# ziniuwan/maed

Measured on AMD Instinct MI355X. Metric: video-clips/sec (BxT frames) train step, higher is better.
Workload: dtype bf16

## Files before the change

### include/maed_hip.h

```cpp
#ifndef MAED_HIP_H
#define MAED_HIP_H

#include <stddef.h>
#include <stdint.h>

#ifdef __cplusplus
extern "C" {
#endif

typedef enum { MAED_F32 = 0, MAED_BF16 = 1,
               MAED_F32X3 = 2, MAED_F32X6 = 3,
               MAED_F32X1 = 4 } maed_dtype;

typedef enum {
    MAED_OK = 0,
    MAED_ERR_ARG = -1,
    MAED_ERR_SHAPE = -2,
    MAED_ERR_ALIGN = -3,
    MAED_ERR_LAUNCH = -4,
    MAED_ERR_UNSUPPORTED = -5
} maed_status;

typedef enum {
    MAED_EPI_STORE = 0,
    MAED_EPI_GELU = 1,
    MAED_EPI_RESID_F32 = 2,
    MAED_EPI_MUL_DGELU = 3,
    MAED_EPI_ATOMIC_F32 = 4,
    MAED_EPI_STORE_F32 = 5,
    MAED_EPI_TANH = 6,
    MAED_EPI_ADD = 7
} maed_epilogue;

typedef enum { MAED_IMPL_AUTO = 0, MAED_IMPL_VALU = 1, MAED_IMPL_MFMA = 2,
               MAED_IMPL_MFMA_GLDS1 = 3, MAED_IMPL_MFMA_GLDS2 = 4,
               MAED_IMPL_MFMA_LONG = 5,
               MAED_IMPL_MFMA_256 = 6,
               MAED_IMPL_X1 = 9,
               MAED_IMPL_MFMA_SK = 10,
               MAED_IMPL_X3 = 7, MAED_IMPL_X6 = 8
} maed_impl;

const char* maed_last_error(void);
int maed_version(void);

typedef enum {
    MAED_OPT_F32_MATMUL = 0,
    MAED_OPT_SIDE_STREAM = 1,
    MAED_OPT_TN_TARGET_WGS = 2,
    MAED_OPT_ABLATE = 3,
    MAED_OPT_GN_BWD_ONEPASS = 4,
    MAED_OPT_F32_BWD_X1 = 5,
    MAED_OPT_ST_FUSED = 6,
    MAED_OPT_CONV3X3_ROWS_WGS = 7,
    MAED_OPT_STEM_WGRAD_WGS = 8,
    MAED_OPT_LBS_FRAMES = 9,
    MAED_OPT_TN_DMA = 10,
    MAED_OPT_X3_PLANES = 11,
    MAED_OPT_X3_PLANES_LN = 12,
    MAED_OPT_SK = 13,
    MAED_OPT_SK_GRID = 14,
    MAED_OPT_TN_SK = 15,
    MAED_OPT_CONV3X3_NARROW_WGS = 16,
    MAED_OPT_CONV3X3_FRAME = 17,
    MAED_OPT_COUNT
} maed_option;
int maed_init(int device);
int maed_device_faults(void);
int maed_device_faults_clear(void);
int maed_set_option(int key, int value);
int maed_get_option(int key);

int maed_layernorm_fwd(const float* x, int64_t x_row_stride, const float* gamma, const float* beta,
                       void* y, int dtype, float* mean, float* rstd,
                       int64_t rows, int C, float eps, void* stream);
int maed_layernorm_bwd(const void* dy, int dtype, const float* x, int64_t x_row_stride,
                       const float* gamma, const float* mean, const float* rstd,
                       const float* dres_in, float* dx_out, void* dx_twin, float* dgamma, float* dbeta,
                       int64_t rows, int C, void* stream);

int maed_gemm_nt(const void* A, int64_t lda, const void* B, int64_t ldb,
                 int64_t M, int64_t N, int64_t K, int dtype, int epilogue,
                 const float* bias, void* out, int64_t ldo, void* out2,
                 const void* aux, int64_t ldaux, int splitk, int impl, void* stream);

int maed_gemm_nt_planes(const void* a_hi, const void* a_lo, int64_t lda, const void* b_hi, const void* b_lo, int64_t ldb, int64_t M, int64_t N, int64_t K,
                        int epilogue, const float* bias, void* out, int64_t ldo, void* out2_bf16, const void* aux, int64_t ldaux, void* out_hi, void* out_lo,
                        int variant, void* stream);
int maed_split_planes(const float* x, void* hi, void* lo, int64_t n, void* stream);

int maed_gemm_tn_wgrad(const void* Y, int64_t ldy, const void* X, int64_t ldx, int64_t M, int N, int K,
                       float* dW, int64_t ldw, float* dbias, int dtype, void* stream);

int maed_transpose_cast(const void* in, int in_dtype, int64_t ldi, int64_t M, int64_t N,
                        void* out_t, int64_t ldt, void* out_c, int64_t ldc, float* colsum,
                        int dtype, void* stream);

int maed_attn_spatial_fwd(const void* qkv, void* o, float* lse, int F, int P, int H, float scale,
                          int dtype, int impl, void* stream);
int maed_attn_spatial_bwd(const void* qkv, const void* o, const void* d_o, const float* lse,
                          void* dqkv, int accumulate, int F, int P, int H, float scale,
                          int dtype, int impl, void* stream);

int maed_attn_temporal_fwd(const void* qkv, void* o, float* lse, int F, int P, int H, int T,
                           float scale, int dtype, void* stream);
int maed_attn_temporal_bwd(const void* qkv, const void* o, const void* d_o, const float* lse,
                           void* dqkv, int accumulate, int F, int P, int H, int T, float scale,
                           int dtype, void* stream);

int maed_st_colmean(const void* x_s, const void* x_t, void* means, float* ws, int F, int P, int C, int dtype, void* stream);
int maed_st_mix_fwd(const void* x_s, const void* x_t, const float* logits, void* mix,
                    int F, int P, int C, int dtype, void* stream);
int maed_st_mix_bwd_reduce(const void* dmix, const void* x_s, const void* x_t, const float* logits,
                           void* dlogits, float* ws, int F, int P, int C, int dtype, void* stream);
int maed_st_mix_bwd_apply(const void* dmix, const float* logits, const void* dmeans, void* dx_s, void* dx_t,
                          int F, int P, int C, int dtype, void* stream);
int maed_st_fused_supported(int P, int C, int dtype);
int maed_st_fused_fwd(const void* x_s, const void* x_t, const void* w_ts, const float* b_ts, void* means, float* logits, void* mix,
                      uint32_t* sync, float* ex, int F, int P, int C, int dtype, void* stream);
int maed_st_fused_bwd(const void* dmix, const void* x_s, const void* x_t, const float* logits, const void* wt_ts, void* dlogits, void* dx_s,
                      void* dx_t, uint32_t* sync, float* ex, int F, int P, int C, int dtype, void* stream);


int maed_embed_add_fwd(const void* patch, int dtype, const float* cls, const float* pos, const float* temp,
                       float* tokens, int F, int P, int C, int T, void* stream);
int maed_embed_add_bwd(const float* dtokens, void* dpatch, int dtype, float* dpos, float* dtemp, int F, int P, int C, int T, void* stream);

int maed_dropout(const float* x, float* y, int64_t n, float p, uint64_t seed, void* stream);
typedef struct { float lr, bias_corr1, bias_corr2, reserved0; uint64_t seed; uint64_t reserved1; } maed_train_state;
int maed_dropout_dev(const float* x, float* y, int64_t n, float p, const maed_train_state* state, uint64_t call_id, void* stream);
int maed_tanh_bwd(const float* dy, const void* y, void* dx, int64_t n, int dtype, void* stream);

typedef struct {
    int F, P, C, H, T, hidden;
    int dtype;
    int impl;
    float eps;
} maed_block_dims;

typedef struct {
    const float *ln1_g, *ln1_b, *ln2_g, *ln2_b;
    const void *w_qkv, *w_ts, *w_proj, *w_fc1, *w_fc2;
    const float *b_qkv, *b_ts, *b_proj, *b_fc1, *b_fc2;
    const void *wt_qkv, *wt_ts, *wt_proj, *wt_fc1, *wt_fc2;
} maed_block_params;

typedef struct {
    float *ln1_g, *ln1_b, *ln2_g, *ln2_b;
    float *w_qkv, *w_ts, *w_proj, *w_fc1, *w_fc2;
    float *b_qkv, *b_ts, *b_proj, *b_fc1, *b_fc2;
} maed_block_grads;

size_t maed_ste_block_saved_bytes(const maed_block_dims* d);
size_t maed_ste_block_scratch_bytes(const maed_block_dims* d);
int maed_ste_block_fwd(const maed_block_dims* d, const maed_block_params* p, const float* x_in,
                       float* x_out, void* saved, void* stream);
size_t maed_ste_block_twin_work_bytes(const maed_block_dims* d);
int maed_ste_block_fwd_twin(const maed_block_dims* d, const maed_block_params* p, const float* x_in, float* x_out, void* saved_bf16, void* work_f32, int work_slot,
                            void* stream);
int maed_ste_block_twin_join(void* stream);
int maed_ste_block_infer(const maed_block_dims* d, const maed_block_params* p, const float* x_in,
                         float* x_out, void* work, void* stream);
int maed_ste_block_bwd(const maed_block_dims* d, const maed_block_params* p, const maed_block_grads* g,
                       const float* x_in, const float* dx_out, float* dx_in, void* saved, void* scratch,
                       const void* dx_out_twin, void* dx_in_twin, void* stream);

int maed_stream_fence(void* from_stream, void* to_stream);

int maed_prof_enable(int on);
int maed_prof_ntags(void);
int maed_prof_collect(double* ms_total_host, int* count_host);
int maed_prof_flops(double* flops_host);
int maed_prof_records(int tag, double* us_host, double* flops_host, double* bytes_host, int cap);

int maed_ktd_chain_fwd(const float* base, const float* w_anc, float* pose, int F, void* stream);

int maed_rot6d_pose_fwd(const float* pose6d, float* rotmat, float* angle_axis, int64_t n_joints, void* stream);

typedef struct {
    const float* v_template;
    const float* shapedirs;
    const float* posedirs;
    const float* J_template;
    const float* J_shapedirs;
    const float* lbs_weights;
    const int32_t* parents;
} maed_smpl_params;
int maed_smpl_lbs_fwd(const maed_smpl_params* sp, const float* betas, const float* rotmat,
                      float* verts, float* joints24, float* scratch_A, float* v_posed, int F, void* stream);
int maed_joint_regress_fwd(const float* Jreg, int J, const float* verts, float* out, int F, void* stream);
int maed_joint_regress_csr_fwd(const int32_t* rowptr, const int32_t* cols, const float* vals, int J, const float* verts, float* out, int F, void* stream);
int maed_smpl_joints_project_fwd(const float* joints24, const float* verts, const int64_t* extra_vertex_ids,
                                 const float* extra9, const int64_t* joint_map, const float* cam,
                                 const float* joints_override, int Jo, float* kp3d, float* kp2d, int F, void* stream);


int maed_smpl_joints_project_bwd(const float* kp3d, const float* cam, const int64_t* joint_map, const float* d_kp3d,
                                 const float* d_kp2d, const float* d_cam_in, int64_t cam_in_stride, float* d_joints24,
                                 float* d_extra21, float* d_extra9, float* d_cam, int F, void* stream);
int maed_smpl_skin_bwd(const maed_smpl_params* sp, const float* A, const float* v_posed, const float* d_verts,
                       const float* d_extra21, const int64_t* extra_vertex_ids, const float* d_extra9, const float* Jextra,
                       float* d_vposed, float* dA, int F, void* stream);
int maed_smpl_skin_bwd_sparse(const maed_smpl_params* sp, const float* A, const float* v_posed, const int32_t* active, int n_active,
                              const float* d_extra21, const int64_t* extra_vertex_ids, const float* d_extra9, const float* Jextra,
                              float* d_vposed_active, float* dA, int F, void* stream);
int maed_smpl_chain_bwd(const maed_smpl_params* sp, const float* betas, const float* rotmat, const float* dA,
                        const float* d_joints24, const float* dpf_dbeta, const float* d_rotmat_in, const float* d_betas_in,
                        int64_t betas_in_stride, float* d_rotmat, float* d_betas, int F, void* stream);
int maed_rot6d_pose_bwd(const float* pose6d, const float* d_rotmat, const float* d_aa, int64_t aa_stride,
                        float* d_pose6d, int64_t n_joints, void* stream);
int maed_ktd_chain_bwd(const float* pose, const float* w_anc, const float* d_pose, const float* d_shape, const float* d_cam,
                       float* d_out, int64_t ld_out, float* d_w_anc, float* d_b_feat, int F, void* stream);
#define MAED_KTD_W_ANC 3420
typedef struct { const float* w[26]; const float* b[26]; float* gw[26]; float* gb[26]; } maed_ktd_ptrs;
int maed_ktd_pack(const maed_ktd_ptrs* t, int hidden, float* w_feat, float* b_feat, float* w_anc, void* stream);
int maed_ktd_unpack_add(const maed_ktd_ptrs* t, int hidden, const float* d_w_feat, const float* d_b_feat, const float* d_w_anc, void* stream);

typedef struct { float w_kp2d, w_kp3d, w_pose, w_shape, w_norm; } maed_loss_weights;
int maed_loss_fwd_bwd(const float* pred_kp2d, const float* gt_kp2d, int M2, const float* pred_kp3d, const float* gt_kp3d,
                      const float* pred_theta, const float* gt_theta, const uint8_t* w_smpl, int M3,
                      const maed_loss_weights* w, float* losses, float* d_kp2d, float* d_kp3d, float* d_theta,
                      double* partials, void* stream);

int maed_loss_accl_fwd_bwd(const float* pred_kp3d, const float* gt_kp3d, int N, int T, float weight, double* loss, float* d_kp3d, void* stream);

typedef struct {
    const float* w;
    float* gw;
    const void* gout;
    int64_t dst_off;
    int64_t dst_t_off;
    int32_t O, I, KHW, fstart;
    int32_t gout_f32;
    int32_t pad_;
} maed_ws_conv;
int maed_weight_std_fwd(const void* conv_table, int n_convs, int n_filters, void* out, int dtype, float* stats, float eps, int transpose_tiles, void* stream);
int maed_weight_std_bwd(const void* conv_table, int n_convs, int n_filters, int dtype, const float* stats, float eps, void* stream);
int maed_groupnorm_fwd(const void* x, const void* residual, const float* gamma, const float* beta, void* y, double* sums,
                       uint8_t* relu_mask, int N, int HW, int C, float eps, int relu, int dtype, int sums_zeroed, void* stream);
int maed_groupnorm_fwd_twin(const void* x, const void* residual, const float* gamma, const float* beta, void* y, double* sums,
                            uint8_t* relu_mask, int N, int HW, int C, float eps, int relu, int sums_zeroed, void* twin_x, void* twin_y, void* stream);
#define MAED_GN_SYNC_WORDS 80
int maed_groupnorm_bwd(const void* x, const uint8_t* relu_mask, const void* dy, const double* sums, const float* gamma, const float* beta,
                       void* dx, void* dres, float* dgamma, float* dbeta, float* ab_scratch, int N, int HW, int C, float eps,
                       int relu, int dtype, int ab_zeroed, uint32_t* frame_sync, void* aux_stream, void* stream);
typedef struct { const float* ab; float* dgamma; float* dbeta; int N; int C; } maed_gn_affine_item;
int maed_gn_affine_grad_batch(const maed_gn_affine_item* items, int count, void* stream);

int maed_maxpool3s2_same_fwd(const void* x, void* y, uint8_t* idx, int N, int H, int W, int C, int dtype, void* stream);
int maed_maxpool3s2_same_bwd(const void* dy, const uint8_t* idx, void* dx, int N, int H, int W, int C, int dtype, void* stream);

int maed_stem_input(const float* x, void* y, int N, int C, int H, int W, int pad_top, int pad_bottom, int pad_left, int pad_right, int c_stride, int dtype,
                    void* stream);

int maed_conv3x3_wgrad_rows64_scratch_floats(int F, int H, int W, int Cin, int Cout);
int maed_conv3x3_wgrad_rows64(const void* dy, const void* x, float* dW, void* scratch, int F, int H, int W, int dtype, void* stream);

int maed_stem7x7s2_supported(int H, int W);
int maed_stem7x7s2_fwd(const void* xp, const void* w, void* wimg, void* y, double* gn_sums, int F, int H, int W, int dtype, void* stream);
int maed_stem7x7s2_wgrad_scratch_floats(int F, int H, int W);
int maed_stem7x7s2_wgrad(const void* dy, const void* xp, float* dW, void* scratch, int F, int H, int W, int dtype, void* stream);

int maed_subsample2_fwd(const void* x, void* y, int F, int H, int W, int C, int dtype, void* stream);
int maed_subsample2_bwd(const void* g, void* dx, int F, int H, int W, int C, int dtype, void* stream);

typedef struct { const float* src; void* dst_c; void* dst_t; int32_t rows, cols, tile0, tiles_n; } maed_wt_entry;
int maed_weight_refresh(const void* table, int n_entries, int n_tiles, int dtype, void* stream);

int maed_adam_step(float* p, const float* g, float* m, float* v, void* shadow_bf16, int64_t n,
                   float lr, float beta1, float beta2, float eps, float weight_decay,
                   float bias_corr1, float bias_corr2, float gscale, void* stream);
int maed_adam_step_dev(float* p, const float* g, float* m, float* v, void* shadow_bf16, int64_t n, const maed_train_state* state,
                       float beta1, float beta2, float eps, float weight_decay, float gscale, void* stream);

#define MAED_COMM_ID_BYTES 128
int maed_comm_load(const char* librccl_path);
int maed_comm_unique_id(void* id128);
int maed_comm_init(int rank, int world, const void* unique_id);
int maed_comm_allreduce_async(void* buf, size_t n, int dtype, void* compute_stream);
int maed_comm_wait(void* compute_stream);
int maed_comm_world(void);
int maed_comm_destroy(void);

int maed_conv3x3_fwd(const void* x, const void* w_taps, const void* zero_page, void* y, int F, int H, int W, int Cin, int Cout,
                     int stride, int pad_top, int pad_left, int Ho, int Wo, const void* add, int w_layout, int dtype, double* gn_sums,
                     void* stream);

int maed_conv1x1_fwd(const void* x, int64_t ldx, const void* w, int64_t ldw, int64_t M, int Cout, int Cin, void* y, int64_t ldy, int hw,
                     double* gn_sums, int dtype, void* stream);

int maed_conv3x3_s2_dgrad(const void* dy, const void* wt_image, const void* zero_page, void* dx, int F, int H, int W, int Cin, int Cout,
                          int pad_top, int pad_left, int Ho, int Wo, int dtype, void* stream);
int maed_conv3x3_s2_tables(void* tapmask, int* rowtab, int F, int H, int W, int pad_top, int pad_left, int Ho, int Wo, void* stream);
int maed_conv3x3_s2_wgrad(const void* dy, const void* x, const void* tapmask, const int* rowtab, const void* zero_page, float* dW, int F, int H, int W,
                          int Cin, int Cout, int Ho, int Wo, int dtype, void* stream);
int maed_conv3x3_tapmask(void* tapmask, int F, int H, int W, void* stream);
int maed_conv3x3_wgrad(const void* dy, const void* x, const void* tapmask, const void* zero_page, float* dW, int F, int H, int W, int Cin,
                       int Cout, int dtype, void* stream);

int maed_eval_pose_errors(const float* pred, const float* target, int N, int J, float* mpjpe, float* pa_mpjpe,
                          float* pred_centred, float* target_centred, void* stream);
int maed_similarity_transform(const float* S1, const float* S2, int N, int J, float* S1_hat, void* stream);
int maed_eval_accel(const float* joints, const float* joints_gt, int N, int J, float* out, void* stream);
int maed_eval_vertex_error(const float* pred_verts, const float* target_verts, int N, int V, float* out, void* stream);

size_t maed_clip_preprocess_workspace(int F, int H, int W);
int maed_clip_preprocess(const uint8_t* src, int64_t src_bytes, const int32_t* frame_i, const float* frame_minv, const int32_t* clip_i,
                         const float* clip_f, int F, int N, int H, int W, const float* norm_host, int has_contrast, int form, float* out,
                         void* workspace, size_t workspace_bytes, void* stream);

#ifdef __cplusplus
}
#endif
#endif
```

### maed_amd/_lib.py

```python
import ctypes as C
import os

HERE = os.path.dirname(os.path.abspath(__file__))
LIB_PATH = os.environ.get("MAED_HIP_LIB") or os.path.join(HERE, "libmaed_hip.so")

F32, BF16 = 0, 1
F32X3, F32X6, F32X1 = 2, 3, 4
EPI_STORE, EPI_GELU, EPI_RESID_F32, EPI_MUL_DGELU, EPI_ATOMIC_F32, EPI_STORE_F32, EPI_TANH, EPI_ADD = range(8)
IMPL_AUTO, IMPL_VALU, IMPL_MFMA = 0, 1, 2
IMPL_MFMA_256 = 6
IMPL_MFMA_LONG = 5
IMPL_MFMA_SK = 10
IMPL_X3, IMPL_X6, IMPL_X1 = 7, 8, 9
(OPT_F32_MATMUL, OPT_SIDE_STREAM, OPT_TN_TARGET_WGS, OPT_ABLATE, OPT_GN_BWD_ONEPASS, OPT_F32_BWD_X1, OPT_ST_FUSED, OPT_CONV3X3_ROWS_WGS, OPT_STEM_WGRAD_WGS,
 OPT_LBS_FRAMES, OPT_TN_DMA, OPT_X3_PLANES, OPT_X3_PLANES_LN, OPT_SK, OPT_SK_GRID, OPT_TN_SK, OPT_CONV3X3_NARROW_WGS, OPT_CONV3X3_FRAME) = range(18)

vp, i64, i32, f32 = C.c_void_p, C.c_int64, C.c_int, C.c_float


class GnAffineItem(C.Structure):
    _fields_ = [("ab", C.c_void_p), ("dgamma", C.c_void_p), ("dbeta", C.c_void_p), ("N", C.c_int), ("C", C.c_int)]


class BlockDims(C.Structure):
    _fields_ = [("F", i32), ("P", i32), ("C", i32), ("H", i32), ("T", i32), ("hidden", i32),
                ("dtype", i32), ("impl", i32), ("eps", f32)]


_PARAM_FIELDS = ["ln1_g", "ln1_b", "ln2_g", "ln2_b", "w_qkv", "w_ts", "w_proj", "w_fc1", "w_fc2",
                 "b_qkv", "b_ts", "b_proj", "b_fc1", "b_fc2", "wt_qkv", "wt_ts", "wt_proj", "wt_fc1", "wt_fc2"]
_GRAD_FIELDS = _PARAM_FIELDS[:14]


class BlockParams(C.Structure):
    _fields_ = [(n, vp) for n in _PARAM_FIELDS]


class BlockGrads(C.Structure):
    _fields_ = [(n, vp) for n in _GRAD_FIELDS]


class SmplParams(C.Structure):
    _fields_ = [(n, vp) for n in ["v_template", "shapedirs", "posedirs", "J_template", "J_shapedirs", "lbs_weights", "parents"]]


class KtdPtrs(C.Structure):
    _fields_ = [("w", vp * 26), ("b", vp * 26), ("gw", vp * 26), ("gb", vp * 26)]


class LossWeights(C.Structure):
    _fields_ = [(n, f32) for n in ["w_kp2d", "w_kp3d", "w_pose", "w_shape", "w_norm"]]


KTD_W_ANC = 3420

SIGNATURES = {
    "maed_last_error": (C.c_char_p, []),
    "maed_version": (i32, []),
    "maed_init": (i32, [i32]),
    "maed_device_faults": (i32, []),
    "maed_device_faults_clear": (i32, []),
    "maed_set_option": (i32, [i32, i32]),
    "maed_get_option": (i32, [i32]),
    "maed_layernorm_fwd": (i32, [vp, i64, vp, vp, vp, i32, vp, vp, i64, i32, f32, vp]),
    "maed_layernorm_bwd": (i32, [vp, i32, vp, i64, vp, vp, vp, vp, vp, vp, vp, vp, i64, i32, vp]),
    "maed_gemm_tn_wgrad": (i32, [vp, i64, vp, i64, i64, i32, i32, vp, i64, vp, i32, vp]),
    "maed_gemm_nt": (i32, [vp, i64, vp, i64, i64, i64, i64, i32, i32, vp, vp, i64, vp, vp, i64, i32, i32, vp]),
    "maed_transpose_cast": (i32, [vp, i32, i64, i64, i64, vp, i64, vp, i64, vp, i32, vp]),
    "maed_attn_spatial_fwd": (i32, [vp, vp, vp, i32, i32, i32, f32, i32, i32, vp]),
    "maed_attn_spatial_bwd": (i32, [vp, vp, vp, vp, vp, i32, i32, i32, i32, f32, i32, i32, vp]),
    "maed_attn_temporal_fwd": (i32, [vp, vp, vp, i32, i32, i32, i32, f32, i32, vp]),
    "maed_attn_temporal_bwd": (i32, [vp, vp, vp, vp, vp, i32, i32, i32, i32, i32, f32, i32, vp]),
    "maed_st_colmean": (i32, [vp, vp, vp, vp, i32, i32, i32, i32, vp]),
    "maed_st_mix_fwd": (i32, [vp, vp, vp, vp, i32, i32, i32, i32, vp]),
    "maed_st_mix_bwd_reduce": (i32, [vp, vp, vp, vp, vp, vp, i32, i32, i32, i32, vp]),
    "maed_st_mix_bwd_apply": (i32, [vp, vp, vp, vp, vp, i32, i32, i32, i32, vp]),
    "maed_st_fused_supported": (i32, [i32, i32, i32]),
    "maed_st_fused_fwd": (i32, [vp, vp, vp, vp, vp, vp, vp, vp, vp, i32, i32, i32, i32, vp]),
    "maed_st_fused_bwd": (i32, [vp, vp, vp, vp, vp, vp, vp, vp, vp, vp, i32, i32, i32, i32, vp]),
    "maed_embed_add_fwd": (i32, [vp, i32, vp, vp, vp, vp, i32, i32, i32, i32, vp]),
    "maed_embed_add_bwd": (i32, [vp, vp, i32, vp, vp, i32, i32, i32, i32, vp]),
    "maed_ste_block_saved_bytes": (C.c_size_t, [C.POINTER(BlockDims)]),
    "maed_ste_block_scratch_bytes": (C.c_size_t, [C.POINTER(BlockDims)]),
    "maed_gemm_nt_planes": (i32, [vp, vp, i64, vp, vp, i64, i64, i64, i64, i32, vp, vp, i64, vp, vp, i64, vp, vp, i32, vp]),
    "maed_split_planes": (i32, [vp, vp, vp, i64, vp]),
    "maed_ste_block_twin_work_bytes": (C.c_size_t, [C.POINTER(BlockDims)]),
    "maed_ste_block_fwd_twin": (i32, [C.POINTER(BlockDims), C.POINTER(BlockParams), vp, vp, vp, vp, i32, vp]),
    "maed_ste_block_twin_join": (i32, [vp]),
    "maed_ste_block_fwd": (i32, [C.POINTER(BlockDims), C.POINTER(BlockParams), vp, vp, vp, vp]),
    "maed_ste_block_infer": (i32, [C.POINTER(BlockDims), C.POINTER(BlockParams), vp, vp, vp, vp]),
    "maed_ste_block_bwd": (i32, [C.POINTER(BlockDims), C.POINTER(BlockParams), C.POINTER(BlockGrads), vp, vp, vp, vp, vp, vp, vp, vp]),
    "maed_loss_accl_fwd_bwd": (i32, [vp, vp, i32, i32, f32, vp, vp, vp]),
    "maed_dropout": (i32, [vp, vp, i64, f32, C.c_uint64, vp]),
    "maed_dropout_dev": (i32, [vp, vp, i64, f32, vp, C.c_uint64, vp]),
    "maed_tanh_bwd": (i32, [vp, vp, vp, i64, i32, vp]),
    "maed_stream_fence": (i32, [vp, vp]),
    "maed_prof_enable": (i32, [i32]),
    "maed_prof_ntags": (i32, []),
    "maed_prof_collect": (i32, [C.POINTER(C.c_double), C.POINTER(i32)]),
    "maed_prof_flops": (i32, [C.POINTER(C.c_double)]),
    "maed_prof_records": (i32, [i32, C.POINTER(C.c_double), C.POINTER(C.c_double), C.POINTER(C.c_double), i32]),
    "maed_ktd_chain_fwd": (i32, [vp, vp, vp, i32, vp]),
    "maed_rot6d_pose_fwd": (i32, [vp, vp, vp, i64, vp]),
    "maed_smpl_lbs_fwd": (i32, [C.POINTER(SmplParams), vp, vp, vp, vp, vp, vp, i32, vp]),
    "maed_joint_regress_fwd": (i32, [vp, i32, vp, vp, i32, vp]),
    "maed_joint_regress_csr_fwd": (i32, [vp, vp, vp, i32, vp, vp, i32, vp]),
    "maed_smpl_joints_project_fwd": (i32, [vp, vp, vp, vp, vp, vp, vp, i32, vp, vp, i32, vp]),
    "maed_smpl_joints_project_bwd": (i32, [vp, vp, vp, vp, vp, vp, i64, vp, vp, vp, vp, i32, vp]),
    "maed_smpl_skin_bwd": (i32, [C.POINTER(SmplParams), vp, vp, vp, vp, vp, vp, vp, vp, vp, i32, vp]),
    "maed_smpl_skin_bwd_sparse": (i32, [C.POINTER(SmplParams), vp, vp, vp, i32, vp, vp, vp, vp, vp, vp, i32, vp]),
    "maed_smpl_chain_bwd": (i32, [C.POINTER(SmplParams), vp, vp, vp, vp, vp, vp, vp, i64, vp, vp, i32, vp]),
    "maed_rot6d_pose_bwd": (i32, [vp, vp, vp, i64, vp, i64, vp]),
    "maed_ktd_chain_bwd": (i32, [vp, vp, vp, vp, vp, vp, i64, vp, vp, i32, vp]),
    "maed_ktd_pack": (i32, [C.POINTER(KtdPtrs), i32, vp, vp, vp, vp]),
    "maed_ktd_unpack_add": (i32, [C.POINTER(KtdPtrs), i32, vp, vp, vp, vp]),
    "maed_loss_fwd_bwd": (i32, [vp, vp, i32, vp, vp, vp, vp, vp, i32, C.POINTER(LossWeights), vp, vp, vp, vp, vp, vp]),
    "maed_weight_std_fwd": (i32, [vp, i32, i32, vp, i32, vp, f32, i32, vp]),
    "maed_weight_std_bwd": (i32, [vp, i32, i32, i32, vp, f32, vp]),
    "maed_groupnorm_fwd": (i32, [vp, vp, vp, vp, vp, vp, vp, i32, i32, i32, f32, i32, i32, i32, vp]),
    "maed_groupnorm_fwd_twin": (i32, [vp, vp, vp, vp, vp, vp, vp, i32, i32, i32, f32, i32, i32, vp, vp, vp]),
    "maed_groupnorm_bwd": (i32, [vp, vp, vp, vp, vp, vp, vp, vp, vp, vp, vp, i32, i32, i32, f32, i32, i32, i32, vp, vp, vp]),
    "maed_gn_affine_grad_batch": (i32, [vp, i32, vp]),
    "maed_comm_load": (i32, [C.c_char_p]),
    "maed_comm_unique_id": (i32, [vp]),
    "maed_comm_init": (i32, [i32, i32, vp]),
    "maed_comm_allreduce_async": (i32, [vp, C.c_size_t, i32, vp]),
    "maed_comm_wait": (i32, [vp]),
    "maed_comm_world": (i32, []),
    "maed_comm_destroy": (i32, []),
    "maed_conv3x3_fwd": (i32, [vp, vp, vp, vp, i32, i32, i32, i32, i32, i32, i32, i32, i32, i32, vp, i32, i32, vp, vp]),
    "maed_conv1x1_fwd": (i32, [vp, i64, vp, i64, i64, i32, i32, vp, i64, i32, vp, i32, vp]),
    "maed_conv3x3_tapmask": (i32, [vp, i32, i32, i32, vp]),
    "maed_conv3x3_s2_dgrad": (i32, [vp, vp, vp, vp, i32, i32, i32, i32, i32, i32, i32, i32, i32, i32, vp]),
    "maed_conv3x3_s2_tables": (i32, [vp, vp, i32, i32, i32, i32, i32, i32, i32, vp]),
    "maed_conv3x3_s2_wgrad": (i32, [vp, vp, vp, vp, vp, vp, i32, i32, i32, i32, i32, i32, i32, i32, vp]),
    "maed_conv3x3_wgrad": (i32, [vp, vp, vp, vp, vp, i32, i32, i32, i32, i32, i32, vp]),
    "maed_eval_pose_errors": (i32, [vp, vp, i32, i32, vp, vp, vp, vp, vp]),
    "maed_similarity_transform": (i32, [vp, vp, i32, i32, vp, vp]),
    "maed_eval_accel": (i32, [vp, vp, i32, i32, vp, vp]),
    "maed_eval_vertex_error": (i32, [vp, vp, i32, i32, vp, vp]),
    "maed_maxpool3s2_same_fwd": (i32, [vp, vp, vp, i32, i32, i32, i32, i32, vp]),
    "maed_maxpool3s2_same_bwd": (i32, [vp, vp, vp, i32, i32, i32, i32, i32, vp]),
    "maed_stem_input": (i32, [vp, vp, i32, i32, i32, i32, i32, i32, i32, i32, i32, i32, vp]),
    "maed_conv3x3_wgrad_rows64_scratch_floats": (i32, [i32, i32, i32, i32, i32]),
    "maed_conv3x3_wgrad_rows64": (i32, [vp, vp, vp, vp, i32, i32, i32, i32, vp]),
    "maed_stem7x7s2_supported": (i32, [i32, i32]),
    "maed_stem7x7s2_fwd": (i32, [vp, vp, vp, vp, vp, i32, i32, i32, i32, vp]),
    "maed_stem7x7s2_wgrad_scratch_floats": (i32, [i32, i32, i32]),
    "maed_stem7x7s2_wgrad": (i32, [vp, vp, vp, vp, i32, i32, i32, i32, vp]),
    "maed_subsample2_fwd": (i32, [vp, vp, i32, i32, i32, i32, i32, vp]),
    "maed_subsample2_bwd": (i32, [vp, vp, i32, i32, i32, i32, i32, vp]),
    "maed_weight_refresh": (i32, [vp, i32, i32, i32, vp]),
    "maed_adam_step": (i32, [vp, vp, vp, vp, vp, i64, f32, f32, f32, f32, f32, f32, f32, f32, vp]),
    "maed_adam_step_dev": (i32, [vp, vp, vp, vp, vp, i64, vp, f32, f32, f32, f32, f32, vp]),
    "maed_clip_preprocess_workspace": (C.c_size_t, [i32, i32, i32]),
    "maed_clip_preprocess": (i32, [vp, i64, vp, vp, vp, vp, i32, i32, i32, i32, C.POINTER(f32), i32, i32, vp, vp, C.c_size_t, vp]),
}

_lib = None
_init_pending = False


class MaedHipError(RuntimeError):
    pass


def lib():
    global _lib, _init_pending
    if _lib is None:
        if not os.path.exists(LIB_PATH):
            raise MaedHipError(f"{LIB_PATH} is missing: build it with `python -m maed_amd.build` "
                               "(hipcc --offload-arch=gfx950).  maed_amd has no non-HIP fallback.")
        handle = C.CDLL(LIB_PATH)
        for name, (res, args) in SIGNATURES.items():
            fn = getattr(handle, name)
            fn.restype, fn.argtypes = res, args
        _lib = handle
        apply_options(handle)
        _init_pending = True
    if _init_pending:
        import torch
        if torch.cuda.is_available() and torch.cuda.is_initialized():
            _init_pending = False
            check(_lib.maed_init(torch.cuda.current_device()), "maed_init")
    return _lib


_OPTIONS = {
    OPT_F32_MATMUL: {"exact": 0, "0": 0, "bf16x3": 1, "1": 1, "bf16x6": 2, "2": 2}[os.environ.get("MAED_F32_MATMUL", "exact")],
    OPT_SIDE_STREAM: int(os.environ.get("MAED_WGRAD_SIDE_STREAM", "1") == "1"),
    OPT_TN_TARGET_WGS: int(os.environ.get("MAED_TN_TARGET_WGS", "0")),
    OPT_ABLATE: int(os.environ.get("MAED_GEMM_ABLATE", "0")),
    OPT_F32_BWD_X1: int(os.environ.get("MAED_F32_BWD", "") == "bf16x1"),
    OPT_ST_FUSED: int(os.environ.get("MAED_ST_FUSED", "1")),
    OPT_GN_BWD_ONEPASS: int(os.environ.get("MAED_GN_BWD_ONEPASS", "1")),
    OPT_CONV3X3_ROWS_WGS: 0 if os.environ.get("MAED_CONV3X3_WGRAD_ROWS", "1") == "0" else int(os.environ.get("MAED_CONV3X3_ROWS_WGS", "256")),
    OPT_STEM_WGRAD_WGS: int(os.environ.get("MAED_STEM_WGS", "512")),
    OPT_LBS_FRAMES: int(os.environ.get("MAED_LBS_FB", "0")),
    OPT_TN_DMA: int(os.environ.get("MAED_TN_DMA", "1")),
    OPT_X3_PLANES: int(os.environ.get("MAED_X3_PLANES", "6")),
    OPT_SK: int(os.environ.get("MAED_SK", "1")),
    OPT_SK_GRID: int(os.environ.get("MAED_SK_GRID", "0")),
    OPT_CONV3X3_FRAME: int(os.environ.get("MAED_CONV3X3_FRAME", "1")),
    OPT_CONV3X3_NARROW_WGS: int(os.environ.get("MAED_CONV3X3_NARROW_WGS", "0")),
    OPT_TN_SK: int(os.environ.get("MAED_TN_SK", "1")),
    OPT_X3_PLANES_LN: int(os.environ.get("MAED_X3_PLANES_LN", "0")),
}


def apply_options(handle):
    for k, v in _OPTIONS.items():
        if handle.maed_set_option(k, v) != 0:
            raise MaedHipError(f"maed_set_option({k}, {v}) failed")


def set_option(key, value):
    _OPTIONS[key] = int(value)
    if _lib is not None:
        check(_lib.maed_set_option(key, int(value)), "set_option")


def get_option(key):
    return _OPTIONS[key]


def check(rc, what=""):
    if rc != 0:
        msg = lib().maed_last_error().decode("utf-8", "replace")
        raise MaedHipError(f"{what or 'libmaed_hip'} failed with status {rc}: {msg}")


def device_faults():
    return 0 if _lib is None else int(_lib.maed_device_faults())


def loaded_path():
    return LIB_PATH if _lib is not None else None
```

### maed_amd/csrc/backbone.hip

```cpp
#include "common.cuh"

struct WsConv {
    const float* w;
    float* gw;
    const void* gout;
    int64_t dst_off;
    int64_t dst_t_off;
    int32_t O, I, KHW, fstart;
    int32_t gout_f32, pad_;
};
#define WS_MAX_CONVS 64

__device__ __forceinline__ int ws_find_conv(const WsConv* __restrict__ tab, int n_convs, int fi) {
    int c = 0;
    for (int i = 1; i < n_convs; ++i) c = (fi >= tab[i].fstart) ? i : c;
    return c;
}

template <typename T>
__global__ __launch_bounds__(256) void ws_fwd_kernel(const WsConv* __restrict__ tab, int n_convs, int n_filters, T* __restrict__ out,
                                                     float* __restrict__ stats , float eps, int skip_transposed) {
    const int fi = blockIdx.x * 4 + (threadIdx.x >> 6), lane = threadIdx.x & 63;
    if (fi >= n_filters) return;
    const WsConv d = tab[ws_find_conv(tab, n_convs, fi)];
    const int K = d.I * d.KHW, o = fi - d.fstart;
    const float* src = d.w + (int64_t)o * K;
    float s = 0.f;
    for (int i = lane; i < K; i += 64) s += src[i];
    const float mean = wave_sum(s) / (float)K;
    float q = 0.f;
    for (int i = lane; i < K; i += 64) { const float c = src[i] - mean; q += c * c; }
    const float inv = 1.f / (sqrtf(wave_sum(q) / (float)K) + eps);
    if (lane == 0) { stats[2 * fi] = mean; stats[2 * fi + 1] = inv; }
    T* dst = out + d.dst_off + (int64_t)o * K;
    T* dst_t = (d.dst_t_off >= 0 && !skip_transposed) ? out + d.dst_t_off + o : nullptr;
    const int KHW = d.KHW, I = d.I;
    for (int ci = lane; ci < I; ci += 64) {
        const float* sp = src + (int64_t)ci * KHW;
        for (int r = 0; r < KHW; ++r) {
            const float v = (sp[r] - mean) * inv;
            stf(dst + (int64_t)r * I + ci, v);
            if (dst_t) stf(dst_t + ((int64_t)r * I + ci) * d.O, v);
        }
    }
}

template <typename T>
__global__ __launch_bounds__(256) void ws_transpose_kernel(const WsConv* __restrict__ tab, int n_convs, T* __restrict__ out) {
    __shared__ T tile[64][66];
    int t = blockIdx.x, c = 0, tk = 0;
    for (; c < n_convs; ++c) {
        const int K = tab[c].I * tab[c].KHW;
        tk = (K + 63) / 64;
        const int nt = tab[c].dst_t_off >= 0 ? ((tab[c].O + 63) / 64) * tk : 0;
        if (t < nt) break;
        t -= nt;
    }
    if (c >= n_convs) return;
    const WsConv d = tab[c];
    const int K = d.I * d.KHW, o0 = (t / tk) * 64, k0 = (t % tk) * 64;
    const T* src = out + d.dst_off;
    T* dst = out + d.dst_t_off;
    const int r = threadIdx.x >> 2, q = (threadIdx.x & 3) * 16;
    constexpr int VE = 16 / (int)sizeof(T);
    if (o0 + r < d.O) {
        const T* sp = src + (int64_t)(o0 + r) * K + k0 + q;
        if (k0 + q + 16 <= K && ((uintptr_t)sp & 15) == 0) {
#pragma unroll
            for (int v = 0; v < 16 / VE; ++v) { const uint4 w = reinterpret_cast<const uint4*>(sp)[v]; T e[VE]; memcpy(e, &w, 16);
#pragma unroll
                for (int j = 0; j < VE; ++j) tile[r][q + v * VE + j] = e[j]; }
        } else {
#pragma unroll
            for (int j = 0; j < 16; ++j) if (k0 + q + j < K) tile[r][q + j] = sp[j];
        }
    }
    __syncthreads();
    if (k0 + r < K) {
        T* dp = dst + (int64_t)(k0 + r) * d.O + o0 + q;
        if (o0 + q + 16 <= d.O && ((uintptr_t)dp & 15) == 0) {
#pragma unroll
            for (int v = 0; v < 16 / VE; ++v) { T e[VE];
#pragma unroll
                for (int j = 0; j < VE; ++j) e[j] = tile[q + v * VE + j][r];
                uint4 w; memcpy(&w, e, 16); reinterpret_cast<uint4*>(dp)[v] = w; }
        } else {
#pragma unroll
            for (int j = 0; j < 16; ++j) if (o0 + q + j < d.O) dp[j] = tile[q + j][r];
        }
    }
}

template <typename T>
__global__ __launch_bounds__(256) void ws_bwd_kernel(const WsConv* __restrict__ tab, int n_convs, int n_filters,
                                                     const float* __restrict__ stats, float eps) {
    const int fi = blockIdx.x * 4 + (threadIdx.x >> 6), lane = threadIdx.x & 63;
    if (fi >= n_filters) return;
    const WsConv d = tab[ws_find_conv(tab, n_convs, fi)];
    if (!d.gout || !d.gw) return;
    const int K = d.I * d.KHW, o = fi - d.fstart;
    const float* src = d.w + (int64_t)o * K;
    const T* g = (const T*)d.gout + (int64_t)o * K;
    const float* g32 = (const float*)d.gout + (int64_t)o * K;
    const bool f32 = d.gout_f32 != 0;
    const float mean = stats[2 * fi], inv = stats[2 * fi + 1];
    const int KHW = d.KHW, I = d.I;
    const float rk = 1.0f / (float)KHW;
    float sg = 0.f, sgw = 0.f;
    for (int i = lane; i < K; i += 64) {
        const int ci = KHW == 1 ? i : (int)(((float)i + 0.5f) * rk), r = i - ci * KHW;
        const float gi = f32 ? g32[(int64_t)r * I + ci] : ldf(g + (int64_t)r * I + ci);
        sg += gi; sgw += gi * (src[i] - mean);
    }
    sg = wave_sum(sg); sgw = wave_sum(sgw);
    const float sigma = 1.f / inv - eps;
    const float c2 = (sigma > 0.f) ? sgw * inv * inv / ((float)K * sigma) : 0.f;
    const float gm = sg / (float)K;
    float* dst = d.gw + (int64_t)o * K;
    for (int i = lane; i < K; i += 64) {
        const int ci = KHW == 1 ? i : (int)(((float)i + 0.5f) * rk), r = i - ci * KHW;
        const float gi = f32 ? g32[(int64_t)r * I + ci] : ldf(g + (int64_t)r * I + ci);
        dst[i] += inv * (gi - gm) - (src[i] - mean) * c2;
    }
}

extern "C" int maed_weight_std_fwd(const void* conv_table, int n_convs, int n_filters, void* out, int dtype, float* stats, float eps,
                                   int filters_aligned64, void* stream) {
    MAED_CHECK_ARG(conv_table && out && stats, MAED_ERR_ARG, "weight_std_fwd: null pointer");
    MAED_CHECK_ARG(n_convs > 0 && n_convs <= WS_MAX_CONVS, MAED_ERR_SHAPE, "weight_std_fwd: n_convs=%d out of range", n_convs);
    if (n_filters <= 0) return MAED_OK;
    const int t_tiles = filters_aligned64;
    MAED_DISPATCH_DTYPE(dtype, T, {
        hipLaunchKernelGGL((ws_fwd_kernel<T>), dim3((n_filters + 3) / 4), dim3(256), 0, (hipStream_t)stream, (const WsConv*)conv_table, n_convs, n_filters, (T*)out, stats, eps,
                           t_tiles > 0 ? 1 : 0);
        if (t_tiles > 0) hipLaunchKernelGGL((ws_transpose_kernel<T>), dim3(t_tiles), dim3(256), 0, (hipStream_t)stream, (const WsConv*)conv_table, n_convs, (T*)out);
    });
    MAED_CHECK_LAUNCH("weight_std_fwd");
    return MAED_OK;
}

extern "C" int maed_weight_std_bwd(const void* conv_table, int n_convs, int n_filters, int dtype, const float* stats, float eps, void* stream) {
    MAED_CHECK_ARG(conv_table && stats, MAED_ERR_ARG, "weight_std_bwd: null pointer");
    MAED_CHECK_ARG(n_convs > 0 && n_convs <= WS_MAX_CONVS, MAED_ERR_SHAPE, "weight_std_bwd: n_convs=%d out of range", n_convs);
    if (n_filters <= 0) return MAED_OK;
    MAED_DISPATCH_DTYPE(dtype, T, hipLaunchKernelGGL((ws_bwd_kernel<T>), dim3((n_filters + 3) / 4), dim3(256), 0, (hipStream_t)stream,
                                                      (const WsConv*)conv_table, n_convs, n_filters, stats, eps));
    MAED_CHECK_LAUNCH("weight_std_bwd");
    return MAED_OK;
}

#define GN_G 32

template <typename T>
__device__ __forceinline__ void gn_load8(const T* p, float (&v)[8]) { ld8(p, v); }

template <typename T>
__global__ __launch_bounds__(256) void gn_stats_kernel(const T* __restrict__ x, double* __restrict__ sums , int HW, int C,
                                                       int rows_per_wg) {
    __shared__ double ls[GN_G][2];
    const int n = blockIdx.y, cbn = C / 8, cb = threadIdx.x % cbn, rsub = threadIdx.x / cbn, rstep = 256 / cbn;
    if (threadIdx.x < GN_G * 2) (&ls[0][0])[threadIdx.x] = 0.0;
    __syncthreads();
    const int r0 = blockIdx.x * rows_per_wg;
    const int r1 = min(HW, r0 + rows_per_wg);
    float s[8], q[8];
#pragma unroll
    for (int j = 0; j < 8; ++j) { s[j] = 0.f; q[j] = 0.f; }
    const T* base = x + ((int64_t)n * HW) * C + cb * 8;
    for (int r = r0 + rsub; r < r1; r += rstep) {
        float v[8];
        gn_load8(base + (int64_t)r * C, v);
#pragma unroll
        for (int j = 0; j < 8; ++j) { s[j] += v[j]; q[j] = fmaf(v[j], v[j], q[j]); }
    }
    const int cpg = C / GN_G;
    if (cpg >= 8) {
        float ss = 0.f, qq = 0.f;
#pragma unroll
        for (int j = 0; j < 8; ++j) { ss += s[j]; qq += q[j]; }
        const int g = cb * 8 / cpg;
        atomicAdd(&ls[g][0], (double)ss); atomicAdd(&ls[g][1], (double)qq);
    } else {
        for (int j0 = 0; j0 < 8; j0 += cpg) {
            float ss = 0.f, qq = 0.f;
            for (int j = j0; j < j0 + cpg; ++j) { ss += s[j]; qq += q[j]; }
            const int g = (cb * 8 + j0) / cpg;
            atomicAdd(&ls[g][0], (double)ss); atomicAdd(&ls[g][1], (double)qq);
        }
    }
    __syncthreads();
    if (threadIdx.x < GN_G * 2) atomicAdd(sums + (int64_t)n * GN_G * 2 + threadIdx.x, (&ls[0][0])[threadIdx.x]);
}


template <typename T, bool RES, bool RELU>
__global__ __launch_bounds__(256) void gn_apply_kernel(const T* __restrict__ x, const T* __restrict__ res, const double* __restrict__ sums,
                                                       const float* __restrict__ gamma, const float* __restrict__ beta, T* __restrict__ y,
                                                       uint8_t* __restrict__ mask, int HW, int C, float eps, int rows_per_wg,
                                                       bf16* __restrict__ twin_x = nullptr, bf16* __restrict__ twin_y = nullptr) {
    __shared__ float lmu[GN_G], lrs[GN_G];
    const int n = blockIdx.y;
    if (threadIdx.x < GN_G) {
        const double cnt = (double)HW * (C / GN_G);
        const double m = sums[((int64_t)n * GN_G + threadIdx.x) * 2] / cnt;
        double var = sums[((int64_t)n * GN_G + threadIdx.x) * 2 + 1] / cnt - m * m;
        if (var < 0.0) var = 0.0;
        lmu[threadIdx.x] = (float)m; lrs[threadIdx.x] = (float)(1.0 / sqrt(var + (double)eps));
    }
    __syncthreads();
    const int cbn = C / 8, cb = threadIdx.x % cbn, rsub = threadIdx.x / cbn, rstep = 256 / cbn, cpg = C / GN_G;
    float a[8], b[8];
    {
        float gg[8], bb[8];
        ld8(gamma + cb * 8, gg); ld8(beta + cb * 8, bb);
#pragma unroll
        for (int j = 0; j < 8; ++j) {
            const int g = (cb * 8 + j) / cpg;
            a[j] = lrs[g] * gg[j]; b[j] = bb[j] - lmu[g] * a[j];
        }
    }
    const int r0 = blockIdx.x * rows_per_wg, r1 = min(HW, r0 + rows_per_wg);
    const int64_t base = ((int64_t)n * HW) * C + cb * 8;
    for (int r = r0 + rsub; r < r1; r += rstep) {
        float v[8], o[8];
        gn_load8(x + base + (int64_t)r * C, v);
        if (twin_x) st8_nt(twin_x + base + (int64_t)r * C, v);
#pragma unroll
        for (int j = 0; j < 8; ++j) o[j] = fmaf(v[j], a[j], b[j]);
        if (RES) { float rr[8]; gn_load8(res + base + (int64_t)r * C, rr);
#pragma unroll
            for (int j = 0; j < 8; ++j) o[j] += rr[j]; }
        if (RELU) {
            if (RES && mask) {
                uint32_t bits = 0;
#pragma unroll
                for (int j = 0; j < 8; ++j) bits |= (o[j] > 0.f ? 1u : 0u) << j;
                mask[((int64_t)n * HW + r) * cbn + cb] = (uint8_t)bits;
            }
#pragma unroll
            for (int j = 0; j < 8; ++j) o[j] = fmaxf(o[j], 0.f); }
        st8(y + base + (int64_t)r * C, o);
        if (twin_y) st8_nt(twin_y + base + (int64_t)r * C, o);
    }
}

template <typename T, bool RELU, bool YMASK>
__global__ __launch_bounds__(256) void gn_bwd_reduce_kernel(const T* __restrict__ x, const uint8_t* __restrict__ mask, const T* __restrict__ dy,
                                                            const double* __restrict__ sums, const float* __restrict__ gamma,
                                                            const float* __restrict__ beta, float* __restrict__ ab ,
                                                            float* __restrict__ dgamma, float* __restrict__ dbeta,
                                                            int HW, int C, float eps, int rows_per_wg, int defer_affine) {
    MAED_DYN_SHARED(float, lpart);
    __shared__ float lmu[GN_G], lrs[GN_G];
    const int n = blockIdx.y;
    if (threadIdx.x < GN_G) {
        const double cnt = (double)HW * (C / GN_G);
        const double m = sums[((int64_t)n * GN_G + threadIdx.x) * 2] / cnt;
        double var = sums[((int64_t)n * GN_G + threadIdx.x) * 2 + 1] / cnt - m * m;
        if (var < 0.0) var = 0.0;
        lmu[threadIdx.x] = (float)m; lrs[threadIdx.x] = (float)(1.0 / sqrt(var + (double)eps));
    }
    __syncthreads();
    const int cbn = C / 8, cb = threadIdx.x % cbn, rsub = threadIdx.x / cbn, rstep = 256 / cbn, cpg = C / GN_G;
    float mu[8], rs[8], sa[8], sb[8], ga[8], be[8];
    if (RELU && !YMASK) { ld8(gamma + cb * 8, ga); ld8(beta + cb * 8, be); }
#pragma unroll
    for (int j = 0; j < 8; ++j) { const int g = (cb * 8 + j) / cpg; mu[j] = lmu[g]; rs[j] = lrs[g]; sa[j] = 0.f; sb[j] = 0.f; }
    const int r0 = blockIdx.x * rows_per_wg, r1 = min(HW, r0 + rows_per_wg);
    const int64_t base = ((int64_t)n * HW) * C + cb * 8;
#define GN_RED_ROW(v_, d_, o_)                                                                                  \
    {                                                                                                           \
        _Pragma("unroll") for (int j = 0; j < 8; ++j) v_[j] = (v_[j] - mu[j]) * rs[j];               \
        if (RELU) {                                                                                             \
            if (YMASK) { _Pragma("unroll") for (int j = 0; j < 8; ++j) d_[j] = ((o_ >> j) & 1u) ? d_[j] : 0.f; }  \
            else { _Pragma("unroll") for (int j = 0; j < 8; ++j) d_[j] = fmaf(v_[j], ga[j], be[j]) > 0.f ? d_[j] : 0.f; } \
        }                                                                                                       \
        _Pragma("unroll") for (int j = 0; j < 8; ++j) { sa[j] += d_[j]; sb[j] = fmaf(d_[j], v_[j], sb[j]); }    \
    }
    int r = r0 + rsub;
    for (; r + 3 * rstep < r1; r += 4 * rstep) {
        float v0[8], v1[8], v2[8], v3[8], d0[8], d1[8], d2[8], d3[8];
        uint32_t o0 = 0, o1 = 0, o2 = 0, o3 = 0;
        const int64_t a0 = base + (int64_t)r * C, a1 = a0 + (int64_t)rstep * C, a2 = a1 + (int64_t)rstep * C, a3 = a2 + (int64_t)rstep * C;
        gn_load8(x + a0, v0); gn_load8(x + a1, v1); gn_load8(x + a2, v2); gn_load8(x + a3, v3);
        gn_load8(dy + a0, d0); gn_load8(dy + a1, d1); gn_load8(dy + a2, d2); gn_load8(dy + a3, d3);
        if (RELU && YMASK) {
            const int64_t m0 = ((int64_t)n * HW + r) * cbn + cb;
            o0 = mask[m0]; o1 = mask[m0 + (int64_t)rstep * cbn]; o2 = mask[m0 + 2 * (int64_t)rstep * cbn]; o3 = mask[m0 + 3 * (int64_t)rstep * cbn];
        }
        GN_RED_ROW(v0, d0, o0) GN_RED_ROW(v1, d1, o1) GN_RED_ROW(v2, d2, o2) GN_RED_ROW(v3, d3, o3)
    }
    for (; r < r1; r += rstep) {
        float v[8], d[8];
        uint32_t o = 0;
        gn_load8(x + base + (int64_t)r * C, v); gn_load8(dy + base + (int64_t)r * C, d);
        if (RELU && YMASK) o = mask[((int64_t)n * HW + r) * cbn + cb];
        GN_RED_ROW(v, d, o)
    }
#undef GN_RED_ROW
    float* mine = lpart + ((size_t)rsub * C + cb * 8) * 2;
#pragma unroll
    for (int j = 0; j < 8; ++j) { mine[2 * j] = sa[j]; mine[2 * j + 1] = sb[j]; }
    __syncthreads();
    for (int i = threadIdx.x; i < 2 * C; i += 256) {
        float t = 0.f;
        for (int k = 0; k < rstep; ++k) t += lpart[(size_t)k * 2 * C + i];
        atomicAdd(ab + (int64_t)n * C * 2 + i, t);
        if (!defer_affine) atomicAdd(((i & 1) ? dgamma : dbeta) + (i >> 1), t);
    }
}

__global__ __launch_bounds__(256) void gn_affine_grad_kernel(const float* __restrict__ ab, float* __restrict__ dgamma, float* __restrict__ dbeta, int N, int C) {
    colsum_add(ab, N, 2 * C, [=](int i) { return ((i & 1) ? dgamma : dbeta) + (i >> 1); });
}

#define GN_BATCH_MAX 64
struct GnAffineBatch {
    maed_gn_affine_item it[GN_BATCH_MAX];
    int first[GN_BATCH_MAX + 1];
    int count;
};
__global__ __launch_bounds__(256) void gn_affine_grad_batch_kernel(GnAffineBatch t) {
    __shared__ float fold[4][64];
    int i = 0;
    while (i + 1 < t.count && (int)blockIdx.x >= t.first[i + 1]) ++i;
    const maed_gn_affine_item it = t.it[i];
    const int cols = 2 * it.C, c = ((int)blockIdx.x - t.first[i]) * 64 + (threadIdx.x & 63), rl = threadIdx.x >> 6;
    float s = 0.f;
    if (c < cols)
        for (int r = rl; r < it.N; r += 4) s += it.ab[(int64_t)r * cols + c];
    fold[rl][threadIdx.x & 63] = s;
    __syncthreads();
    if (rl == 0 && c < cols) {
        atomicAdd(((c & 1) ? it.dgamma : it.dbeta) + (c >> 1), (fold[0][threadIdx.x] + fold[1][threadIdx.x]) + (fold[2][threadIdx.x] + fold[3][threadIdx.x]));
    }
}
extern "C" int maed_gn_affine_grad_batch(const maed_gn_affine_item* items, int count, void* stream) {
    MAED_CHECK_ARG(count >= 0 && (items || count == 0), MAED_ERR_ARG, "gn_affine_grad_batch: null table");
    for (int base = 0; base < count; base += GN_BATCH_MAX) {
        GnAffineBatch t;
        t.count = count - base < GN_BATCH_MAX ? count - base : GN_BATCH_MAX;
        int wg = 0;
        for (int i = 0; i < t.count; ++i) {
            const maed_gn_affine_item& it = items[base + i];
            MAED_CHECK_ARG(it.ab && it.dgamma && it.dbeta && it.N > 0 && it.C > 0, MAED_ERR_ARG, "gn_affine_grad_batch: item %d: null pointer or empty extent", base + i);
            t.it[i] = it; t.first[i] = wg;
            wg += (2 * it.C + 63) / 64;
        }
        t.first[t.count] = wg;
        hipLaunchKernelGGL(gn_affine_grad_batch_kernel, dim3((unsigned)wg), dim3(256), 0, (hipStream_t)stream, t);
    }
    MAED_CHECK_LAUNCH("gn_affine_grad_batch");
    return MAED_OK;
}

template <typename T, bool RES, bool RELU>
__global__ __launch_bounds__(256) void gn_bwd_apply_kernel(const T* __restrict__ x, const uint8_t* __restrict__ mask, const T* __restrict__ dy,
                                                           const double* __restrict__ sums, const float* __restrict__ ab,
                                                           const float* __restrict__ gamma, const float* __restrict__ beta,
                                                           T* __restrict__ dx, T* __restrict__ dres,
                                                           int HW, int C, float eps, int rows_per_wg) {
    __shared__ float lmu[GN_G], lrs[GN_G], lm1[GN_G], lm2[GN_G];
    const int n = blockIdx.y, cpg = C / GN_G;
    if (threadIdx.x < GN_G) {
        const double cnt = (double)HW * cpg;
        const double m = sums[((int64_t)n * GN_G + threadIdx.x) * 2] / cnt;
        double var = sums[((int64_t)n * GN_G + threadIdx.x) * 2 + 1] / cnt - m * m;
        if (var < 0.0) var = 0.0;
        lmu[threadIdx.x] = (float)m; lrs[threadIdx.x] = (float)(1.0 / sqrt(var + (double)eps));
        float m1 = 0.f, m2 = 0.f;
        for (int c = threadIdx.x * cpg; c < (threadIdx.x + 1) * cpg; ++c) {
            m1 = fmaf(gamma[c], ab[((int64_t)n * C + c) * 2], m1);
            m2 = fmaf(gamma[c], ab[((int64_t)n * C + c) * 2 + 1], m2);
        }
        lm1[threadIdx.x] = m1 / (float)cnt; lm2[threadIdx.x] = m2 / (float)cnt;
    }
    __syncthreads();
    const int cbn = C / 8, cb = threadIdx.x % cbn, rsub = threadIdx.x / cbn, rstep = 256 / cbn;
    float mu[8], rs[8], gg[8], be[8], m1[8], m2[8];
    ld8(gamma + cb * 8, gg); ld8(beta + cb * 8, be);
#pragma unroll
    for (int j = 0; j < 8; ++j) { const int g = (cb * 8 + j) / cpg; mu[j] = lmu[g]; rs[j] = lrs[g]; m1[j] = lm1[g]; m2[j] = lm2[g]; }
    const int r0 = blockIdx.x * rows_per_wg, r1 = min(HW, r0 + rows_per_wg);
    const int64_t base = ((int64_t)n * HW) * C + cb * 8;
    for (int r = r0 + rsub; r < r1; r += rstep) {
        float v[8], d[8], o[8];
        gn_load8(x + base + (int64_t)r * C, v); gn_load8(dy + base + (int64_t)r * C, d);
        if (RELU) {
            if (RES) { const uint32_t bits = mask[((int64_t)n * HW + r) * cbn + cb];
#pragma unroll
                for (int j = 0; j < 8; ++j) d[j] = ((bits >> j) & 1u) ? d[j] : 0.f;
            } else {
#pragma unroll
                for (int j = 0; j < 8; ++j) d[j] = fmaf((v[j] - mu[j]) * rs[j], gg[j], be[j]) > 0.f ? d[j] : 0.f;
            }
        }
        if (RES && dres) st8(dres + base + (int64_t)r * C, d);
#pragma unroll
        for (int j = 0; j < 8; ++j) o[j] = rs[j] * (gg[j] * d[j] - m1[j] - (v[j] - mu[j]) * rs[j] * m2[j]);
        st8(dx + base + (int64_t)r * C, o);
    }
}

#define GN1_NT 512
template <typename T> struct GnChunk;
template <> struct GnChunk<bf16> { uint4 v; };
template <> struct GnChunk<float> { float4 a, b; };
__device__ __forceinline__ void gn_chunk_ld(const bf16* p, GnChunk<bf16>& c) { c.v = *reinterpret_cast<const uint4*>(p); }
__device__ __forceinline__ void gn_chunk_ld(const float* p, GnChunk<float>& c) { c.a = *reinterpret_cast<const float4*>(p); c.b = *reinterpret_cast<const float4*>(p + 4); }
__device__ __forceinline__ void gn_chunk_st(bf16* p, const GnChunk<bf16>& c) { *reinterpret_cast<uint4*>(p) = c.v; }
__device__ __forceinline__ void gn_chunk_st(float* p, const GnChunk<float>& c) { *reinterpret_cast<float4*>(p) = c.a; *reinterpret_cast<float4*>(p + 4) = c.b; }
__device__ __forceinline__ void gn_chunk_zero(GnChunk<bf16>& c) { c.v = make_uint4(0u, 0u, 0u, 0u); }
__device__ __forceinline__ void gn_chunk_zero(GnChunk<float>& c) { c.a = make_float4(0.f, 0.f, 0.f, 0.f); c.b = c.a; }
__device__ __forceinline__ void gn_chunk_get(const GnChunk<bf16>& c, float (&o)[8]) {
    o[0] = __uint_as_float(c.v.x << 16); o[1] = __uint_as_float(c.v.x & 0xffff0000u); o[2] = __uint_as_float(c.v.y << 16); o[3] = __uint_as_float(c.v.y & 0xffff0000u);
    o[4] = __uint_as_float(c.v.z << 16); o[5] = __uint_as_float(c.v.z & 0xffff0000u); o[6] = __uint_as_float(c.v.w << 16); o[7] = __uint_as_float(c.v.w & 0xffff0000u);
}
__device__ __forceinline__ void gn_chunk_get(const GnChunk<float>& c, float (&o)[8]) {
    o[0] = c.a.x; o[1] = c.a.y; o[2] = c.a.z; o[3] = c.a.w; o[4] = c.b.x; o[5] = c.b.y; o[6] = c.b.z; o[7] = c.b.w;
}
__device__ __forceinline__ void gn_chunk_put(GnChunk<bf16>& c, const float (&o)[8]) {
    c.v = make_uint4(pack_bf2(o[0], o[1]), pack_bf2(o[2], o[3]), pack_bf2(o[4], o[5]), pack_bf2(o[6], o[7]));
}
__device__ __forceinline__ void gn_chunk_put(GnChunk<float>& c, const float (&o)[8]) {
    c.a = make_float4(o[0], o[1], o[2], o[3]); c.b = make_float4(o[4], o[5], o[6], o[7]);
}
#define GN1_SYNC_WORDS 80
template <typename T, bool RELU, bool YMASK, int GPC, int CH, int NT>
__global__ __launch_bounds__(NT, 4) void gn_bwd_onepass_kernel(const T* __restrict__ x, const uint8_t* __restrict__ mask, const T* __restrict__ dy,
                                                                   const double* __restrict__ sums, const float* __restrict__ gamma, const float* __restrict__ beta,
                                                                   float* ab , T* __restrict__ dx, T* __restrict__ dres,
                                                                   uint32_t* sync , int HW, int C, float eps, int S,
                                                                   int rows_per_wg, int phase, int skew, uint32_t* fault ) {
    MAED_DYN_SHARED(float, lpart);
    __shared__ float lmu[GN_G], lrs[GN_G], lgrp[GN_G * 2], lb[GN_G], lk[GN_G];
    __shared__ int lfail;
    const int n = blockIdx.y, tid = threadIdx.x, cpg = C / GN_G;
    if (tid < GN_G) {
        const double cnt = (double)HW * cpg;
        const double m = sums[((int64_t)n * GN_G + tid) * 2] / cnt;
        double var = sums[((int64_t)n * GN_G + tid) * 2 + 1] / cnt - m * m;
        if (var < 0.0) var = 0.0;
        lmu[tid] = (float)m; lrs[tid] = (float)(1.0 / sqrt(var + (double)eps));
    }
    if (tid < GN_G * 2) lgrp[tid] = 0.f;
    if (tid == 0) lfail = 0;
    __syncthreads();
    const int cbn = C / 8, cb = tid % cbn, rsub = tid / cbn, rstep = NT / cbn;
    constexpr int JS = 8 / GPC;
    const int g0 = cb * 8 / cpg;
    float mu[GPC], rs[GPC];
#pragma unroll
    for (int q = 0; q < GPC; ++q) { mu[q] = lmu[g0 + q]; rs[q] = lrs[g0 + q]; }
    const int r0 = blockIdx.x * rows_per_wg, r1 = min(HW, r0 + rows_per_wg);
    const int64_t base = ((int64_t)n * HW) * C + cb * 8;
    float* const gsum = (float*)(sync + (int64_t)n * GN1_SYNC_WORDS + 16);
#ifndef MAED_HOSTSIM
    if (skew > 0 && (n & 1) && (int)(blockIdx.y * gridDim.x + blockIdx.x) < 512)
        for (int i = 0; i < skew; ++i) __builtin_amdgcn_s_sleep(100);
#endif

    GnChunk<T> xr[CH], dr[CH];
    uint32_t mb[(CH + 3) / 4];
#pragma unroll
    for (int k = 0; k < (CH + 3) / 4; ++k) mb[k] = 0u;
#pragma unroll
    for (int k = 0; k < CH; ++k) {
        const int r = r0 + rsub + k * rstep;
        if (r < r1) {
            gn_chunk_ld(x + base + (int64_t)r * C, xr[k]);
            gn_chunk_ld(dy + base + (int64_t)r * C, dr[k]);
            if (RELU && YMASK) mb[k >> 2] |= (uint32_t)mask[((int64_t)n * HW + r) * cbn + cb] << (8 * (k & 3));
        } else { gn_chunk_zero(xr[k]); gn_chunk_zero(dr[k]); }
    }
    {
        float sa[8], sb[8], ga[8], be[8];
#pragma unroll
        for (int j = 0; j < 8; ++j) { sa[j] = 0.f; sb[j] = 0.f; ga[j] = 0.f; be[j] = 0.f; }
        if (RELU && !YMASK) { ld8(gamma + cb * 8, ga); ld8(beta + cb * 8, be); }
#pragma unroll
        for (int k = 0; k < CH; ++k) {
            if (r0 + rsub + k * rstep >= r1) continue;
            float v[8], d[8];
            gn_chunk_get(xr[k], v); gn_chunk_get(dr[k], d);
            const uint32_t bits = (mb[k >> 2] >> (8 * (k & 3))) & 0xffu;
#pragma unroll
            for (int j = 0; j < 8; ++j) {
                const float xh = (v[j] - mu[j / JS]) * rs[j / JS];
                if (RELU) d[j] = (YMASK ? ((bits >> j) & 1u) != 0u : fmaf(xh, ga[j], be[j]) > 0.f) ? d[j] : 0.f;
                sa[j] += d[j]; sb[j] = fmaf(d[j], xh, sb[j]);
            }
            if (RELU) gn_chunk_put(dr[k], d);
        }
        if (!(RELU && !YMASK)) ld8(gamma + cb * 8, ga);
        if (phase != 2) {
            float* mine = lpart + ((size_t)rsub * C + cb * 8) * 2;
#pragma unroll
            for (int j = 0; j < 8; ++j) { mine[2 * j] = sa[j]; mine[2 * j + 1] = sb[j]; }
#pragma unroll
            for (int q = 0; q < GPC; ++q) {
                float p1 = 0.f, p2 = 0.f;
#pragma unroll
                for (int j = q * JS; j < (q + 1) * JS; ++j) { p1 = fmaf(ga[j], sa[j], p1); p2 = fmaf(ga[j], sb[j], p2); }
                for (int m = cbn; m < 64; m <<= 1) { p1 += __shfl_xor(p1, m, 64); p2 += __shfl_xor(p2, m, 64); }
                if ((tid & 63) < cbn) { atomicAdd(&lgrp[(g0 + q) * 2], p1); atomicAdd(&lgrp[(g0 + q) * 2 + 1], p2); }
            }
        }
    }
    __syncthreads();
    if (phase != 2) {
        if (tid < GN_G * 2 && (S > 1 || phase == 1)) atomicAdd(gsum + tid, lgrp[tid]);
        if (phase == 0 && S > 1) {
            MAED_WAIT_VMCNT0();
            __syncthreads();
            if (tid == 0 && !maed_frame_arrive_and_wait(sync + (int64_t)n * GN1_SYNC_WORDS, (uint32_t)S)) { lfail = 1; maed_report_fault(fault); }
        }
        for (int i = tid; i < 2 * C; i += NT) {
            float t = 0.f;
            for (int k = 0; k < rstep; ++k) t += lpart[(size_t)k * 2 * C + i];
            atomicAdd(ab + (int64_t)n * C * 2 + i, t);
        }
        if (phase == 1) return;
        __syncthreads();
    }
    if (tid < GN_G * 2 && (S > 1 || phase == 2)) lgrp[tid] = maed_coherent_read(gsum + tid);
    __syncthreads();
    if (tid < GN_G) {
        const float cnt = (float)((double)HW * cpg);
        const float poison = lfail ? __uint_as_float(0x7fc00000u) : 0.f;
        lb[tid] = lrs[tid] * (lgrp[2 * tid] / cnt) + poison; lk[tid] = lrs[tid] * (lgrp[2 * tid + 1] / cnt);
    }
    __syncthreads();
    float A[8], B[GPC], K[GPC];
    {
        float gg[8];
        ld8(gamma + cb * 8, gg);
#pragma unroll
        for (int j = 0; j < 8; ++j) A[j] = rs[j / JS] * gg[j];
#pragma unroll
        for (int q = 0; q < GPC; ++q) { B[q] = lb[g0 + q]; K[q] = lk[g0 + q]; }
    }
#pragma unroll
    for (int k = 0; k < CH; ++k) {
        const int r = r0 + rsub + k * rstep;
        if (r >= r1) continue;
        float v[8], d[8], o[8];
        gn_chunk_get(xr[k], v); gn_chunk_get(dr[k], d);
        if (dres) gn_chunk_st(dres + base + (int64_t)r * C, dr[k]);
#pragma unroll
        for (int j = 0; j < 8; ++j) o[j] = fmaf(A[j], d[j], -fmaf((v[j] - mu[j / JS]) * rs[j / JS], K[j / JS], B[j / JS]));
        GnChunk<T> oc;
        gn_chunk_put(oc, o);
        gn_chunk_st(dx + base + (int64_t)r * C, oc);
    }
}

static int gn_check(int C, int HW, const char* who) {
    MAED_CHECK_ARG(C % GN_G == 0 && C % 8 == 0 && C / 8 <= 256 && 256 % (C / 8) == 0, MAED_ERR_SHAPE, "%s: C=%d unsupported (need C%%32==0, C/8 a power of two <= 256)", who, C);
    MAED_CHECK_ARG(HW > 0, MAED_ERR_SHAPE, "%s: HW=%d", who, HW);
    return MAED_OK;
}
static int gn_rows_per_wg(int N, int HW, int C, int target_wgs = 2048) {
    const int tile = 256 / (C / 8);
    int chunks = (target_wgs + N - 1) / N;
    int rows = (HW + chunks - 1) / chunks;
    rows = (rows + tile - 1) / tile * tile;
    return rows < tile ? tile : rows;
}

static int groupnorm_fwd(const void* x, const void* residual, const float* gamma, const float* beta, void* y, double* sums,
                         uint8_t* relu_mask, int N, int HW, int C, float eps, int relu, int dtype, int sums_zeroed, void* twin_x, void* twin_y, void* stream) {
    MAED_CHECK_ARG(x && gamma && beta && y && sums, MAED_ERR_ARG, "groupnorm_fwd: null pointer");
    MAED_PROPAGATE(gn_check(C, HW, "groupnorm_fwd"));
    if (N <= 0) return MAED_OK;
    hipStream_t s = (hipStream_t)stream;
    const int rows = gn_rows_per_wg(N, HW, C);
    dim3 grid((HW + rows - 1) / rows, N);
    if (!sums_zeroed) MAED_HIP(hipMemsetAsync(sums, 0, (size_t)N * GN_G * 2 * sizeof(double), s), "groupnorm_fwd: memset");
    MAED_DISPATCH_DTYPE(dtype, T, {
        if (sums_zeroed != 2)
            hipLaunchKernelGGL((gn_stats_kernel<T>), grid, dim3(256), 0, s, (const T*)x, sums, HW, C, rows);
        if (residual && relu) hipLaunchKernelGGL((gn_apply_kernel<T, true, true>), grid, dim3(256), 0, s, (const T*)x, (const T*)residual, sums, gamma, beta, (T*)y, relu_mask, HW, C, eps, rows, (bf16*)twin_x, (bf16*)twin_y);
        else if (residual) hipLaunchKernelGGL((gn_apply_kernel<T, true, false>), grid, dim3(256), 0, s, (const T*)x, (const T*)residual, sums, gamma, beta, (T*)y, relu_mask, HW, C, eps, rows, (bf16*)twin_x, (bf16*)twin_y);
        else if (relu) hipLaunchKernelGGL((gn_apply_kernel<T, false, true>), grid, dim3(256), 0, s, (const T*)x, (const T*)nullptr, sums, gamma, beta, (T*)y, relu_mask, HW, C, eps, rows, (bf16*)twin_x, (bf16*)twin_y);
        else hipLaunchKernelGGL((gn_apply_kernel<T, false, false>), grid, dim3(256), 0, s, (const T*)x, (const T*)nullptr, sums, gamma, beta, (T*)y, relu_mask, HW, C, eps, rows, (bf16*)twin_x, (bf16*)twin_y);
    });
    MAED_CHECK_LAUNCH("groupnorm_fwd");
    return MAED_OK;
}

extern "C" int maed_groupnorm_fwd(const void* x, const void* residual, const float* gamma, const float* beta, void* y, double* sums,
                                  uint8_t* relu_mask, int N, int HW, int C, float eps, int relu, int dtype, int sums_zeroed, void* stream) {
    return groupnorm_fwd(x, residual, gamma, beta, y, sums, relu_mask, N, HW, C, eps, relu, dtype, sums_zeroed, nullptr, nullptr, stream);
}
extern "C" int maed_groupnorm_fwd_twin(const void* x, const void* residual, const float* gamma, const float* beta, void* y, double* sums,
                                       uint8_t* relu_mask, int N, int HW, int C, float eps, int relu, int sums_zeroed, void* twin_x, void* twin_y, void* stream) {
    MAED_CHECK_ARG(is_aligned(twin_x, 16) && is_aligned(twin_y, 16), MAED_ERR_ALIGN, "groupnorm_fwd_twin: 16-B alignment");
    return groupnorm_fwd(x, residual, gamma, beta, y, sums, relu_mask, N, HW, C, eps, relu, MAED_F32, sums_zeroed, twin_x, twin_y, stream);
}

extern "C" int maed_groupnorm_bwd(const void* x, const uint8_t* relu_mask, const void* dy, const double* sums, const float* gamma, const float* beta,
                                  void* dx, void* dres, float* dgamma, float* dbeta, float* ab_scratch, int N, int HW, int C, float eps,
                                  int relu, int dtype, int ab_zeroed, uint32_t* frame_sync, void* aux_stream, void* stream) {
    MAED_CHECK_ARG(x && dy && sums && gamma && beta && dx && ab_scratch, MAED_ERR_ARG, "groupnorm_bwd: null pointer");
    MAED_CHECK_ARG((dgamma != nullptr) == (dbeta != nullptr), MAED_ERR_ARG, "groupnorm_bwd: dgamma and dbeta go together (both NULL: the caller folds ab_scratch with maed_gn_affine_grad_batch)");
    MAED_CHECK_ARG(!(relu && dres) || relu_mask, MAED_ERR_ARG, "groupnorm_bwd: the forward's relu_mask is needed when a residual was added before the ReLU");
    MAED_PROPAGATE(gn_check(C, HW, "groupnorm_bwd"));
    if (N <= 0) return MAED_OK;
    hipStream_t s = (hipStream_t)stream;
    const int rows = gn_rows_per_wg(N, HW, C);
    dim3 grid((HW + rows - 1) / rows, N);
    const int rrows = gn_rows_per_wg(N, HW, C, 768);
    dim3 rgrid((HW + rrows - 1) / rrows, N);
    if (!ab_zeroed) MAED_HIP(hipMemsetAsync(ab_scratch, 0, (size_t)N * C * 2 * sizeof(float), s), "groupnorm_bwd: memset");
    const size_t lds = (size_t)(256 / (C / 8)) * 2 * C * sizeof(float);
    constexpr int defer = 1;
    const bool ymask = relu && relu_mask;
    const int cpg = C / GN_G, cbn1 = C / 8, ch1 = dtype == MAED_BF16 ? ((relu && !ymask) ? 7 : 8) : 4;
    int S1 = 0, rows1 = 0;
    const int nt1 = maed_opt(MAED_OPT_GN_BWD_ONEPASS) == 2 ? 256 : GN1_NT;
    uint32_t* const fault1 = maed_fault_word();
    bool onepass = frame_sync && maed_opt(MAED_OPT_GN_BWD_ONEPASS) && cpg >= 2 && cbn1 <= nt1 && !maed_fault_seen("groupnorm_bwd");
    if (onepass) {
        const int rstep = nt1 / cbn1, cap = ch1 * rstep;
        S1 = (HW + cap - 1) / cap;
        rows1 = (((HW + S1 - 1) / S1) + rstep - 1) / rstep * rstep;
        onepass = S1 <= 64;
    }
#define GN_RED(RELU_, YM_) hipLaunchKernelGGL((gn_bwd_reduce_kernel<T, RELU_, YM_>), rgrid, dim3(256), lds, s, (const T*)x, relu_mask, (const T*)dy, \
        sums, gamma, beta, ab_scratch, dgamma, dbeta, HW, C, eps, rrows, defer)
#define GN_APP(RES_, RELU_) hipLaunchKernelGGL((gn_bwd_apply_kernel<T, RES_, RELU_>), grid, dim3(256), 0, s, (const T*)x, relu_mask, (const T*)dy, \
        sums, ab_scratch, gamma, beta, (T*)dx, (T*)dres, HW, C, eps, rows)
#define GN_ONE4(RELU_, YM_, GPC_, CH_, PH_, NT_) hipLaunchKernelGGL((gn_bwd_onepass_kernel<T, RELU_, YM_, GPC_, CH_, NT_>), dim3(S1, N), dim3(NT_), lds1, s, (const T*)x, relu_mask, \
        (const T*)dy, sums, gamma, beta, ab_scratch, (T*)dx, (T*)dres, frame_sync, HW, C, eps, (maed_opt(MAED_OPT_GN_BWD_ONEPASS) == 3 ? 1 : S1), rows1, PH_, skew1, fault1)
#define GN_ONE3(RELU_, YM_, GPC_, CH_, PH_) do { if (nt1 == 256) GN_ONE4(RELU_, YM_, GPC_, CH_, PH_, 256); else GN_ONE4(RELU_, YM_, GPC_, CH_, PH_, GN1_NT); } while (0)
#define GN_ONE2(RELU_, YM_, CH_, PH_) do { if (cpg >= 8) GN_ONE3(RELU_, YM_, 1, CH_, PH_); else if (cpg == 4) GN_ONE3(RELU_, YM_, 2, CH_, PH_); else GN_ONE3(RELU_, YM_, 4, CH_, PH_); } while (0)
#define GN_ONE(PH_) do { constexpr int CH_ = sizeof(T) == 2 ? 8 : 4, CHM_ = sizeof(T) == 2 ? 7 : 4; \
        if (!relu) GN_ONE2(false, false, CH_, PH_); else if (ymask) GN_ONE2(true, true, CH_, PH_); else GN_ONE2(true, false, CHM_, PH_); } while (0)
    const size_t lds1 = (size_t)(nt1 / cbn1) * 2 * C * sizeof(float);
    const int opt1 = maed_opt(MAED_OPT_GN_BWD_ONEPASS);
    const int skew1 = (int64_t)S1 * N >= 1536 ? (opt1 >= 10 ? opt1 - 10 : 2) : 0;
    MAED_DISPATCH_DTYPE(dtype, T, {
        if (onepass) {
#ifdef MAED_HOSTSIM
            GN_ONE(1); GN_ONE(2);
#else
            GN_ONE(0);
#endif
        } else if (!relu) GN_RED(false, false); else if (ymask) GN_RED(true, true); else GN_RED(true, false);
        if (defer && dgamma) {
            hipStream_t sa = s;
            if (aux_stream) {
                MAED_PROPAGATE(maed_stream_fence(s, aux_stream));
                sa = (hipStream_t)aux_stream;
            }
            hipLaunchKernelGGL(gn_affine_grad_kernel, dim3((2 * C + 63) / 64, (N + 63) / 64), dim3(256), 0, sa, ab_scratch, dgamma, dbeta, N, C);
        }
        if (onepass) { }
        else if (ymask) GN_APP(true, true); else if (dres) GN_APP(true, false); else if (relu) GN_APP(false, true); else GN_APP(false, false);
    });
#undef GN_RED
#undef GN_APP
#undef GN_ONE
#undef GN_ONE2
#undef GN_ONE3
#undef GN_ONE4
    MAED_CHECK_LAUNCH("groupnorm_bwd");
    return MAED_OK;
}

template <typename T>
__global__ __launch_bounds__(256) void maxpool3s2_fwd_kernel(const T* __restrict__ x, T* __restrict__ y, uint8_t* __restrict__ idx, int N, int H, int W,
                                                             int C, int Ho, int Wo, int top, int left) {
    const int64_t i = (int64_t)blockIdx.x * 256 + threadIdx.x;
    const int cb = C / 8;
    if (i >= (int64_t)N * Ho * Wo * cb) return;
    const int c8 = (int)(i % cb) * 8;
    const int64_t pix = i / cb;
    const int wo = (int)(pix % Wo), ho = (int)((pix / Wo) % Ho), n = (int)(pix / ((int64_t)Wo * Ho));
    float m[8]; int am[8];
#pragma unroll
    for (int j = 0; j < 8; ++j) { m[j] = -INFINITY; am[j] = 0; }
    bool first = true;
    for (int kh = 0; kh < 3; ++kh) {
        const int h = 2 * ho - top + kh;
        if (h < 0 || h >= H) continue;
        for (int kw = 0; kw < 3; ++kw) {
            const int w = 2 * wo - left + kw;
            if (w < 0 || w >= W) continue;
            float v[8];
            ld8(x + (((int64_t)n * H + h) * W + w) * C + c8, v);
#pragma unroll
            for (int j = 0; j < 8; ++j)
                if (first || v[j] > m[j] || v[j] != v[j]) { m[j] = v[j]; am[j] = kh * 3 + kw; }
            first = false;
        }
    }
    st8(y + i * 8, m);
    uint32_t lo = 0, hi = 0;
#pragma unroll
    for (int j = 0; j < 4; ++j) { lo |= (uint32_t)am[j] << (8 * j); hi |= (uint32_t)am[4 + j] << (8 * j); }
    *reinterpret_cast<uint2*>(idx + i * 8) = make_uint2(lo, hi);
}

template <typename T>
__global__ __launch_bounds__(256) void maxpool3s2_bwd_kernel(const T* __restrict__ dy, const uint8_t* __restrict__ idx, T* __restrict__ dx, int N, int H,
                                                             int W, int C, int Ho, int Wo, int top, int left) {
    const int64_t i = (int64_t)blockIdx.x * 256 + threadIdx.x;
    const int cb = C / 8, Hb = (H + top + 1) >> 1, Wb = (W + left + 1) >> 1;
    if (i >= (int64_t)N * Hb * Wb * cb) return;
    const int c8 = (int)(i % cb) * 8;
    const int64_t blk = i / cb;
    const int l = (int)(blk % Wb), k = (int)((blk / Wb) % Hb), n = (int)(blk / ((int64_t)Wb * Hb));
    float g[2][2][8];
#pragma unroll
    for (int a = 0; a < 2; ++a)
#pragma unroll
        for (int b = 0; b < 2; ++b)
#pragma unroll
            for (int j = 0; j < 8; ++j) g[a][b][j] = 0.f;
#pragma unroll
    for (int wh = 0; wh < 2; ++wh) {
        const int ho = k - 1 + wh;
        if (ho < 0 || ho >= Ho) continue;
#pragma unroll
        for (int ww = 0; ww < 2; ++ww) {
            const int wo = l - 1 + ww;
            if (wo < 0 || wo >= Wo) continue;
            const int64_t o = ((((int64_t)n * Ho + ho) * Wo + wo) * C + c8);
            const uint2 a = *reinterpret_cast<const uint2*>(idx + o);
            float d[8];
            ld8(dy + o, d);
#pragma unroll
            for (int dh = 0; dh < 2; ++dh) {
                const int kh = 2 * (1 - wh) + dh;
                if (kh > 2) continue;
#pragma unroll
                for (int dw = 0; dw < 2; ++dw) {
                    const int kw = 2 * (1 - ww) + dw;
                    if (kw > 2) continue;
                    const uint32_t tap = (uint32_t)(kh * 3 + kw);
#pragma unroll
                    for (int j = 0; j < 4; ++j) {
                        if (((a.x >> (8 * j)) & 0xffu) == tap) g[dh][dw][j] += d[j];
                        if (((a.y >> (8 * j)) & 0xffu) == tap) g[dh][dw][4 + j] += d[4 + j];
                    }
                }
            }
        }
    }
#pragma unroll
    for (int dh = 0; dh < 2; ++dh) {
        const int h = 2 * k - top + dh;
        if (h < 0 || h >= H) continue;
#pragma unroll
        for (int dw = 0; dw < 2; ++dw) {
            const int w = 2 * l - left + dw;
            if (w < 0 || w >= W) continue;
            st8(dx + (((int64_t)n * H + h) * W + w) * C + c8, g[dh][dw]);
        }
    }
}

static void maxpool_geom(int H, int W, int& Ho, int& Wo, int& top, int& left) {
    Ho = (H + 1) / 2; Wo = (W + 1) / 2;
    const int ph = (Ho - 1) * 2 + 3 - H, pw = (Wo - 1) * 2 + 3 - W;
    top = (ph > 0 ? ph : 0) / 2; left = (pw > 0 ? pw : 0) / 2;
}

extern "C" int maed_maxpool3s2_same_fwd(const void* x, void* y, uint8_t* idx, int N, int H, int W, int C, int dtype, void* stream) {
    MAED_CHECK_ARG(x && y && idx, MAED_ERR_ARG, "maxpool3s2_same_fwd: null pointer");
    MAED_CHECK_ARG(N >= 0 && H > 0 && W > 0 && C > 0 && C % 8 == 0, MAED_ERR_SHAPE, "maxpool3s2_same_fwd: C=%d must be a multiple of 8", C);
    int Ho, Wo, top, left;
    maxpool_geom(H, W, Ho, Wo, top, left);
    const int64_t n = (int64_t)N * Ho * Wo * (C / 8);
    if (n == 0) return MAED_OK;
    MAED_DISPATCH_DTYPE(dtype, T, hipLaunchKernelGGL((maxpool3s2_fwd_kernel<T>), dim3((unsigned)((n + 255) / 256)), dim3(256), 0, (hipStream_t)stream,
                                                      (const T*)x, (T*)y, idx, N, H, W, C, Ho, Wo, top, left));
    MAED_CHECK_LAUNCH("maxpool3s2_same_fwd");
    return MAED_OK;
}

extern "C" int maed_maxpool3s2_same_bwd(const void* dy, const uint8_t* idx, void* dx, int N, int H, int W, int C, int dtype, void* stream) {
    MAED_CHECK_ARG(dy && idx && dx, MAED_ERR_ARG, "maxpool3s2_same_bwd: null pointer");
    MAED_CHECK_ARG(N >= 0 && H > 0 && W > 0 && C > 0 && C % 8 == 0, MAED_ERR_SHAPE, "maxpool3s2_same_bwd: C=%d must be a multiple of 8", C);
    int Ho, Wo, top, left;
    maxpool_geom(H, W, Ho, Wo, top, left);
    const int64_t n = (int64_t)N * ((H + top + 1) / 2) * ((W + left + 1) / 2) * (C / 8);
    if (n == 0) return MAED_OK;
    MAED_DISPATCH_DTYPE(dtype, T, hipLaunchKernelGGL((maxpool3s2_bwd_kernel<T>), dim3((unsigned)((n + 255) / 256)), dim3(256), 0, (hipStream_t)stream,
                                                      (const T*)dy, idx, (T*)dx, N, H, W, C, Ho, Wo, top, left));
    MAED_CHECK_LAUNCH("maxpool3s2_same_bwd");
    return MAED_OK;
}

template <typename T>
__global__ __launch_bounds__(256) void stem_input_kernel(const float* __restrict__ x, T* __restrict__ y, int64_t n, int C, int CS, int H, int W, int Hp, int Wp, int top, int left) {
    const int64_t i = (int64_t)blockIdx.x * 256 + threadIdx.x;
    if (i >= n) return;
    const int xp = (int)(i % Wp), yp = (int)((i / Wp) % Hp);
    const int64_t f = i / ((int64_t)Wp * Hp);
    const int xx = xp - left, yy = yp - top;
    const bool in = (unsigned)xx < (unsigned)W && (unsigned)yy < (unsigned)H;
    if (CS == 4) {
        float v[4];
#pragma unroll
        for (int c = 0; c < 4; ++c) v[c] = (in && c < C) ? x[((f * C + c) * H + yy) * (int64_t)W + xx] : 0.f;
        st4(y + i * 4, v);
        return;
    }
    for (int c = 0; c < CS; ++c) stf(y + i * CS + c, (in && c < C) ? x[((f * C + c) * H + yy) * (int64_t)W + xx] : 0.f);
}

extern "C" int maed_stem_input(const float* x, void* y, int N, int C, int H, int W, int pad_top, int pad_bottom, int pad_left, int pad_right, int c_stride, int dtype,
                               void* stream) {
    MAED_CHECK_ARG(x && y, MAED_ERR_ARG, "stem_input: null pointer");
    MAED_CHECK_ARG(N >= 0 && C > 0 && C <= c_stride && c_stride <= 4 && H > 0 && W > 0 && pad_top >= 0 && pad_bottom >= 0 && pad_left >= 0 && pad_right >= 0, MAED_ERR_SHAPE,
                   "stem_input: bad extents (C <= c_stride <= 4)");
    MAED_CHECK_ARG(c_stride != 4 || is_aligned(y, 16), MAED_ERR_ALIGN, "stem_input: y must be 16-B aligned");
    const int Hp = H + pad_top + pad_bottom, Wp = W + pad_left + pad_right;
    const int64_t n = (int64_t)N * Hp * Wp;
    if (n == 0) return MAED_OK;
    MAED_DISPATCH_DTYPE(dtype, T, hipLaunchKernelGGL((stem_input_kernel<T>), dim3((unsigned)((n + 255) / 256)), dim3(256), 0, (hipStream_t)stream, x, (T*)y, n, C, c_stride, H,
                                                      W, Hp, Wp, pad_top, pad_left));
    MAED_CHECK_LAUNCH("stem_input");
    return MAED_OK;
}

template <typename T>
__global__ __launch_bounds__(256) void subsample2_fwd_kernel(const T* __restrict__ x, T* __restrict__ y, int64_t n, int H, int W, int C, int Ho, int Wo) {
    const int64_t i = (int64_t)blockIdx.x * 256 + threadIdx.x;
    if (i >= n) return;
    const int cb = C / 8, c8 = (int)(i % cb) * 8;
    const int64_t pix = i / cb;
    const int ox = (int)(pix % Wo), oy = (int)((pix / Wo) % Ho);
    const int64_t f = pix / ((int64_t)Wo * Ho);
    float v[8];
    ld8(x + ((f * H + 2 * oy) * W + 2 * ox) * C + c8, v);
    st8(y + i * 8, v);
}

template <typename T>
__global__ __launch_bounds__(256) void subsample2_bwd_kernel(const T* __restrict__ g, T* __restrict__ dx, int64_t n, int H, int W, int C, int Ho, int Wo) {
    const int64_t i = (int64_t)blockIdx.x * 256 + threadIdx.x;
    if (i >= n) return;
    const int cb = C / 8, c8 = (int)(i % cb) * 8;
    const int64_t pix = i / cb;
    const int ix = (int)(pix % W), iy = (int)((pix / W) % H);
    const int64_t f = pix / ((int64_t)W * H);
    float v[8] = {0.f, 0.f, 0.f, 0.f, 0.f, 0.f, 0.f, 0.f};
    if (!((ix | iy) & 1)) ld8(g + ((f * Ho + (iy >> 1)) * Wo + (ix >> 1)) * C + c8, v);
    st8(dx + i * 8, v);
}

extern "C" int maed_subsample2_fwd(const void* x, void* y, int F, int H, int W, int C, int dtype, void* stream) {
    MAED_CHECK_ARG(x && y, MAED_ERR_ARG, "subsample2_fwd: null pointer");
    MAED_CHECK_ARG(F >= 0 && H > 0 && W > 0 && C > 0 && C % 8 == 0, MAED_ERR_SHAPE, "subsample2_fwd: C=%d must be a multiple of 8", C);
    const int Ho = (H + 1) / 2, Wo = (W + 1) / 2;
    const int64_t n = (int64_t)F * Ho * Wo * (C / 8);
    if (n == 0) return MAED_OK;
    MAED_DISPATCH_DTYPE(dtype, T, hipLaunchKernelGGL((subsample2_fwd_kernel<T>), dim3((unsigned)((n + 255) / 256)), dim3(256), 0, (hipStream_t)stream,
                                                      (const T*)x, (T*)y, n, H, W, C, Ho, Wo));
    MAED_CHECK_LAUNCH("subsample2_fwd");
    return MAED_OK;
}

extern "C" int maed_subsample2_bwd(const void* g, void* dx, int F, int H, int W, int C, int dtype, void* stream) {
    MAED_CHECK_ARG(g && dx, MAED_ERR_ARG, "subsample2_bwd: null pointer");
    MAED_CHECK_ARG(F >= 0 && H > 0 && W > 0 && C > 0 && C % 8 == 0, MAED_ERR_SHAPE, "subsample2_bwd: C=%d must be a multiple of 8", C);
    const int Ho = (H + 1) / 2, Wo = (W + 1) / 2;
    const int64_t n = (int64_t)F * H * W * (C / 8);
    if (n == 0) return MAED_OK;
    MAED_DISPATCH_DTYPE(dtype, T, hipLaunchKernelGGL((subsample2_bwd_kernel<T>), dim3((unsigned)((n + 255) / 256)), dim3(256), 0, (hipStream_t)stream,
                                                      (const T*)g, (T*)dx, n, H, W, C, Ho, Wo));
    MAED_CHECK_LAUNCH("subsample2_bwd");
    return MAED_OK;
}
```

### maed_amd/csrc/options.hip

```cpp
#include "common.cuh"
#include "gemm_x3.h"
#include <atomic>
#include <string.h>

static std::atomic<int> g_opt[MAED_OPT_COUNT] = {
    {0},
    {1},
    {0},
    {0},
    {1},
    {0},
    {1},
    {256},
    {512},
    {0},
    {1},
    {6},
    {0},
    {1},
    {0},
    {1},
    {0},
    {1},
};

extern "C" int maed_init(int device) {
#ifndef MAED_HOSTSIM
    hipDeviceProp_t prop;
    if (hipGetDeviceProperties(&prop, device) != hipSuccess) { (void)hipGetLastError(); maed_set_error("init: no HIP device %d", device); return MAED_ERR_ARG; }
    if (!strstr(prop.gcnArchName, "gfx950")) {
        maed_set_error("init: device %d is %s; libmaed_hip is built for gfx950 (MI355X) only", device, prop.gcnArchName);
        return MAED_ERR_UNSUPPORTED;
    }
#else
    (void)device;
#endif
    (void)maed_fault_word();
#ifndef MAED_HOSTSIM
    if (maed_init_runtime() != MAED_OK) { maed_set_error("init: could not create the library's side streams / event rings"); return MAED_ERR_LAUNCH; }
#endif
    return MAED_OK;
}

static std::atomic<uint32_t*> g_fault{nullptr};
static std::atomic<int> g_fault_told{0};
uint32_t* maed_fault_word(void) {
    uint32_t* w = g_fault.load(std::memory_order_acquire);
    if (w) return w;
#ifdef MAED_HOSTSIM
    uint32_t* n = (uint32_t*)calloc(16, sizeof(uint32_t));
#else
    uint32_t* n = nullptr;
    if (hipHostMalloc((void**)&n, 64, hipHostMallocMapped | hipHostMallocCoherent) != hipSuccess || !n) { (void)hipGetLastError(); return nullptr; }
    memset(n, 0, 64);
#endif
    uint32_t* expected = nullptr;
    if (!g_fault.compare_exchange_strong(expected, n, std::memory_order_acq_rel)) {
#ifdef MAED_HOSTSIM
        free(n);
#else
        (void)hipHostFree(n);
#endif
        return expected;
    }
    return n;
}
bool maed_fault_seen(const char* who) {
    uint32_t* w = g_fault.load(std::memory_order_acquire);
    if (!w || *(volatile uint32_t*)w == 0) return false;
    if (!g_fault_told.exchange(1))
        maed_set_error("%s: %u frame-barrier timeout(s) on this device (workgroups of a frame were not co-resident: shared GPU / preemption); the affected results were "
                       "NaN-poisoned, the one-pass GroupNorm backward and the fused attentive addition now run as their multi-launch forms", who, *(volatile uint32_t*)w);
    return true;
}
extern "C" int maed_device_faults(void) {
    uint32_t* w = g_fault.load(std::memory_order_acquire);
    const int n = w ? (int)*(volatile uint32_t*)w : 0;
    if (n > 0)
        maed_set_error("%d frame-barrier timeout(s) on this device (workgroups of a frame were not co-resident: shared GPU / preemption); the affected results were "
                       "NaN-poisoned, the one-pass GroupNorm backward and the fused attentive addition run as their multi-launch forms from the next call on", n);
    return n;
}
extern "C" int maed_device_faults_clear(void) { uint32_t* w = g_fault.load(std::memory_order_acquire); if (w) *(volatile uint32_t*)w = 0; g_fault_told.store(0); return MAED_OK; }

extern "C" int maed_set_option(int key, int value) {
    MAED_CHECK_ARG(key >= 0 && key < MAED_OPT_COUNT, MAED_ERR_ARG, "set_option: unknown option %d", key);
    if (key == MAED_OPT_F32_MATMUL) MAED_CHECK_ARG(value >= 0 && value <= 2, MAED_ERR_ARG, "set_option: MAED_OPT_F32_MATMUL takes 0 (exact), 1 (bf16x3) or 2 (bf16x6)");
    if (key == MAED_OPT_TN_TARGET_WGS) MAED_CHECK_ARG(value == 0 || value >= 64, MAED_ERR_ARG, "set_option: MAED_OPT_TN_TARGET_WGS must be 0 (heuristic) or >= 64");
    if (key == MAED_OPT_CONV3X3_ROWS_WGS || key == MAED_OPT_STEM_WGRAD_WGS) MAED_CHECK_ARG(value >= 0 && value <= 65535, MAED_ERR_ARG, "set_option: workgroup count out of range");
    if (key == MAED_OPT_LBS_FRAMES) MAED_CHECK_ARG(value == 0 || value == 4 || value == 8 || value == 16, MAED_ERR_ARG, "set_option: MAED_OPT_LBS_FRAMES takes 0 (auto), 4, 8 or 16");
    if (key == MAED_OPT_X3_PLANES) MAED_CHECK_ARG(value == 0 || (value >= 2 && value <= 7 && value != 3), MAED_ERR_ARG, "set_option: MAED_OPT_X3_PLANES takes 0 (fp32 operands) or a kernel variant 2, 4, 5, 6, 7");
    if (key == MAED_OPT_SK) MAED_CHECK_ARG(value >= 0 && value <= 3, MAED_ERR_ARG, "set_option: MAED_OPT_SK takes 0 (off), 1 (heuristic), 2 (no K cuts) or 3 (always)");
    if (key == MAED_OPT_TN_SK) MAED_CHECK_ARG(value == 0 || value == 1, MAED_ERR_ARG, "set_option: MAED_OPT_TN_SK takes 0 or 1");
    if (key == MAED_OPT_SK_GRID) MAED_CHECK_ARG(value >= 0 && value <= 512, MAED_ERR_ARG, "set_option: MAED_OPT_SK_GRID takes 0 (one workgroup per CU) or a workgroup count <= 512");
    g_opt[key].store(value, std::memory_order_relaxed);
    return MAED_OK;
}

extern "C" int maed_get_option(int key) {
    if (key < 0 || key >= MAED_OPT_COUNT) { maed_set_error("get_option: unknown option %d", key); return MAED_ERR_ARG; }
    return g_opt[key].load(std::memory_order_relaxed);
}

int maed_opt(int key) { return g_opt[key].load(std::memory_order_relaxed); }

int maed_x3_planes(void) {
    const int v = maed_opt(MAED_OPT_F32_MATMUL);
    return v == 1 ? 2 : v == 2 ? 3 : 0;
}
```

### maed_amd/ops.py

```python
import ctypes as C
import math
import os
import threading
import weakref

import numpy as _np

import torch

from . import _lib as L
from ._lib import BF16, F32, check

WEIGHT_EPOCH = 0


def bump_weight_epoch():
    global WEIGHT_EPOCH
    WEIGHT_EPOCH += 1


def on_library_device(t):
    return t.is_cuda or (SIM_MODULE_PATHS and L._lib is not None and L._lib.maed_version() < 0)


SIM_MODULE_PATHS = True


_F32_MODES = {"exact": 0, "highest": 0, "bf16x3": 1, "high": 1, "bf16x6": 2}


def set_float32_matmul_precision(mode):
    L.set_option(L.OPT_F32_MATMUL, _F32_MODES[mode])


def get_float32_matmul_precision():
    return ("exact", "bf16x3", "bf16x6")[L.get_option(L.OPT_F32_MATMUL)]


def f32_split():
    return L.get_option(L.OPT_F32_MATMUL) != 0


def lib_matmul_dtype(dtype, prec=None):
    return dtype == torch.bfloat16 or (dtype == torch.float32 and (f32_split() or prec in ("bf16x3", "bf16x6", "bf16x1")))


def bwd_prec(prec):
    if L.get_option(L.OPT_F32_BWD_X1):
        return "bf16x1"
    return "bf16x3" if prec == "bf16x6" else prec


_BWD_TWIN = [os.environ.get("MAED_F32_BWD", "") == "bf16"]


def set_float32_backward_precision(mode):
    assert mode in (None, "same", "bf16x1", "bf16"), mode
    L.set_option(L.OPT_F32_BWD_X1, int(mode in ("bf16x1", "bf16")))
    _BWD_TWIN[0] = mode == "bf16"


def get_float32_backward_precision():
    return "bf16" if _BWD_TWIN[0] else "bf16x1" if L.get_option(L.OPT_F32_BWD_X1) else "same"


_SHADOW = {}
TWIN_FORWARDS = [0]


def shadow_put(t16, t32):
    _SHADOW[t16.data_ptr()] = (t16, t32)
    return t16


def shadow_of(t):
    if not _SHADOW or t is None or t.dtype != torch.bfloat16:
        return None
    e = _SHADOW.get(t.data_ptr())
    return e[1] if e is not None and e[0].numel() == t.numel() else None


def shadow_clear():
    assert not (_UNFILLED and _SHADOW) or all(k in _SHADOW for k in _UNFILLED), "an unfilled twin lost its shadow"
    for k in list(_UNFILLED):
        e = _SHADOW.get(k)
        if e is not None:
            e[0].copy_(e[1])
    _UNFILLED.clear()
    _SHADOW.clear()


def shadow_keep_only(t16):
    e = _SHADOW.get(t16.data_ptr()) if t16 is not None else None
    for k in list(_UNFILLED):
        if k in _SHADOW:
            _SHADOW[k][0].copy_(_SHADOW[k][1])
    _UNFILLED.clear()
    _SHADOW.clear()
    if e is not None:
        _SHADOW[t16.data_ptr()] = e


def twin_of(y32):
    return shadow_put(y32.to(torch.bfloat16), y32)


_UNFILLED = set()


def twin_later(y32):
    y16 = torch.empty_like(y32, dtype=torch.bfloat16)
    _UNFILLED.add(y16.data_ptr())
    return shadow_put(y16, y32)


def twin_fill(t16):
    if t16 is not None and t16.data_ptr() in _UNFILLED:
        _UNFILLED.discard(t16.data_ptr())
        t16.copy_(shadow_of(t16))


def bwd_twin():
    return _BWD_TWIN[0] and f32_split()


def mm_code(dtype, prec=None):
    if dtype == torch.float32 and prec in ("bf16x3", "bf16x6", "bf16x1"):
        return {"bf16x3": L.F32X3, "bf16x6": L.F32X6, "bf16x1": L.F32X1}[prec]
    return dt_code(dtype)


def dt_code(dtype):
    if dtype == torch.float32:
        return F32
    if dtype == torch.bfloat16:
        return BF16
    raise TypeError(f"maed_amd: unsupported compute dtype {dtype}")


_TLS = threading.local()


def _stream():
    s = getattr(_TLS, "stream", None)
    if s is not None:
        return s
    return torch._C._cuda_getCurrentRawStream(torch._C._cuda_getDevice())


_SIDE_ON = None
_SIDE = {}


def _side_on():
    return (L.get_option(L.OPT_SIDE_STREAM) == 1) if _SIDE_ON is None else _SIDE_ON


def _join_at_end_of_backward(device, st):
    if st[1]:
        return
    try:
        torch.autograd.Variable._execution_engine.queue_callback(lambda: side_stream_join(device))
    except RuntimeError:
        pass


def side_stream_run(fn, *tensors):
    t0 = tensors[0]
    if not (t0.is_cuda and _side_on()):
        return fn()
    st = _SIDE.get(t0.device)
    if st is None:
        st = _SIDE[t0.device] = [torch.cuda.Stream(device=t0.device), False]
    side = st[0]
    raw = side.cuda_stream
    check(L.lib().maed_stream_fence(_stream(), raw), "stream_fence")
    prev = getattr(_TLS, "stream", None)
    _TLS.stream = raw
    try:
        out = fn()
    finally:
        _TLS.stream = prev
    _keep_until_join(t0.device, st, tensors)
    _join_at_end_of_backward(t0.device, st)
    st[1] = True
    return out


def side_stream_handle(device, *tensors):
    if not (device.type == "cuda" and _side_on()):
        return None
    st = _SIDE.get(device)
    if st is None:
        st = _SIDE[device] = [torch.cuda.Stream(device=device), False]
    _keep_until_join(device, st, tensors)
    _join_at_end_of_backward(device, st)
    st[1] = True
    return st[0].cuda_stream


def _keep_until_join(device, st, tensors):
    keep = _KEEP.setdefault(device, [])
    keep.extend(tensors)
    if len(keep) > 4096:
        side_stream_join(device)


_KEEP = {}


def _keep_alive_on_stream(t):
    if getattr(_TLS, "stream", None) is not None:
        _KEEP.setdefault(t.device, []).append(t)


def side_stream_join(device):
    st = _SIDE.get(device)
    if st is not None and st[1]:
        torch.cuda.current_stream(device).wait_stream(st[0])
        st[1] = False
    keep = _KEEP.get(device)
    if keep:
        keep.clear()


def _p(t):
    if t is None:
        return None
    if not t.is_cuda:
        raise L.MaedHipError("maed_amd kernels need CUDA/HIP tensors (no CPU path)")
    return t.data_ptr()


def _c(t):
    return t if t.is_contiguous() else t.contiguous()


_TABLES = {}
_CAPTURE_KEEP = None


def _upload_table(tab, dev):
    host = torch.from_numpy(tab.view(_np.uint8))
    if dev.type != "cuda":
        return host.clone()
    key = (dev, host.numpy().tobytes())
    capturing = torch.cuda.is_current_stream_capturing()
    hit = _TABLES.get(key)
    if hit is not None:
        if capturing and _CAPTURE_KEEP is not None:
            _CAPTURE_KEEP.append(hit)
        return hit
    if capturing:
        raise RuntimeError("maed_amd: a pointer table changed between the eager warm-up steps and the capture (a row points at a per-step temporary)")
    pinned = host.pin_memory()
    out = pinned.to(dev, non_blocking=True)
    if len(_TABLES) >= 64:
        _TABLES.pop(next(iter(_TABLES)))
    _TABLES[key] = out
    return out


def layernorm_fwd(x, gamma, beta, out_dtype, eps=1e-6, row_stride=None, rows=None):
    C_ = x.shape[-1]
    if rows is None:
        x = _c(x)
        rows = x.numel() // C_
        row_stride = C_
    y = torch.empty(rows, C_, dtype=out_dtype, device=x.device)
    mean = torch.empty(rows, dtype=torch.float32, device=x.device)
    rstd = torch.empty_like(mean)
    check(L.lib().maed_layernorm_fwd(_p(x), row_stride, _p(gamma), _p(beta), _p(y), dt_code(out_dtype), _p(mean), _p(rstd),
                                     rows, C_, eps, _stream()), "layernorm_fwd")
    return y, mean, rstd


def layernorm_bwd(dy, x, gamma, mean, rstd, dres=None, dgamma=None, dbeta=None, want_twin=False):
    C_ = x.shape[-1]
    x, dy = _c(x), _c(dy)
    rows = x.numel() // C_
    dx = torch.empty(rows, C_, dtype=torch.float32, device=x.device)
    twin = torch.empty(rows, C_, dtype=dy.dtype, device=x.device) if want_twin else None
    dgamma = torch.zeros(C_, dtype=torch.float32, device=x.device) if dgamma is None else dgamma
    dbeta = torch.zeros(C_, dtype=torch.float32, device=x.device) if dbeta is None else dbeta
    check(L.lib().maed_layernorm_bwd(_p(dy), dt_code(dy.dtype), _p(x), C_, _p(gamma), _p(mean), _p(rstd), _p(dres), _p(dx), _p(twin),
                                     _p(dgamma), _p(dbeta), rows, C_, _stream()), "layernorm_bwd")
    return (dx, dgamma, dbeta, twin) if want_twin else (dx, dgamma, dbeta)


def gemm_tn_wgrad(Y, X, dW=None, dbias=None, prec=None):
    M, N = Y.shape
    K = X.shape[1]
    dW = torch.zeros(N, K, dtype=torch.float32, device=Y.device) if dW is None else dW
    check(L.lib().maed_gemm_tn_wgrad(_p(Y), Y.stride(0), _p(X), X.stride(0), M, N, K, _p(dW), dW.stride(0), _p(dbias), mm_code(Y.dtype, prec), _stream()),
          "gemm_tn_wgrad")
    return dW


def gemm_nt(A, B, epilogue=L.EPI_STORE, bias=None, out=None, out2=None, aux=None, splitk=1, impl=L.IMPL_AUTO, M=None, K=None, prec=None):
    assert A.dim() == 2 and B.dim() == 2 and A.dtype == B.dtype
    M = A.shape[0] if M is None else M
    K = A.shape[1] if K is None else K
    N = B.shape[0]
    assert A.stride(1) == 1 and B.stride(1) == 1
    if out is None:
        odt = torch.float32 if epilogue in (L.EPI_RESID_F32, L.EPI_ATOMIC_F32, L.EPI_STORE_F32) else A.dtype
        out = (torch.zeros if epilogue == L.EPI_ATOMIC_F32 else torch.empty)(M, N, dtype=odt, device=A.device)
    if epilogue == L.EPI_GELU and out2 is None:
        out2 = torch.empty_like(out)
    check(L.lib().maed_gemm_nt(_p(A), A.stride(0), _p(B), B.stride(0), M, N, K, mm_code(A.dtype, prec), epilogue, _p(bias),
                               _p(out), out.stride(0), _p(out2), _p(aux), aux.stride(0) if aux is not None else 0,
                               splitk, impl, _stream()), "gemm_nt")
    return (out, out2) if epilogue == L.EPI_GELU else out


def split_planes(x):
    x = _c(x)
    assert x.dtype == torch.float32 and x.numel() % 8 == 0
    hi, lo = torch.empty_like(x, dtype=torch.bfloat16), torch.empty_like(x, dtype=torch.bfloat16)
    check(L.lib().maed_split_planes(_p(x), _p(hi), _p(lo), x.numel(), _stream()), "split_planes")
    return hi, lo


def gemm_nt_planes(A, B, epilogue=L.EPI_STORE, bias=None, aux=None, want_f32=True, want_planes=False, want_pre=False, variant=0):
    (Ah, Al), (Bh, Bl) = A, B
    assert Ah.dtype == Al.dtype == Bh.dtype == Bl.dtype == torch.bfloat16 and Ah.shape == Al.shape and Bh.shape == Bl.shape
    assert Ah.stride() == Al.stride() and Bh.stride() == Bl.stride() and Ah.stride(1) == 1 and Bh.stride(1) == 1
    M, K = Ah.shape
    N = Bh.shape[0]
    dev = Ah.device
    out = torch.empty(M, N, dtype=torch.float32, device=dev) if want_f32 else None
    oh = torch.empty(M, N, dtype=torch.bfloat16, device=dev) if want_planes else None
    ol = torch.empty(M, N, dtype=torch.bfloat16, device=dev) if want_planes else None
    pre = torch.empty(M, N, dtype=torch.bfloat16, device=dev) if (want_pre and epilogue == L.EPI_GELU) else None
    check(L.lib().maed_gemm_nt_planes(_p(Ah), _p(Al), Ah.stride(0), _p(Bh), _p(Bl), Bh.stride(0), M, N, K, epilogue, _p(bias), _p(out), N, _p(pre), _p(aux),
                                      aux.stride(0) if aux is not None else 0, _p(oh), _p(ol), variant, _stream()), "gemm_nt_planes")
    return out, ((oh, ol) if want_planes else None), pre


def transpose_cast(x, out_dtype, want_t=True, want_c=False, colsum=None, pad_to=64):
    assert x.dim() == 2 and x.stride(1) == 1
    M, N = x.shape
    Mp = (M + pad_to - 1) // pad_to * pad_to
    out_t = torch.empty(N, Mp, dtype=out_dtype, device=x.device) if want_t else None
    out_c = torch.empty(M, N, dtype=out_dtype, device=x.device) if want_c else None
    check(L.lib().maed_transpose_cast(_p(x), dt_code(x.dtype), x.stride(0), M, N, _p(out_t), Mp, _p(out_c), N, _p(colsum),
                                      dt_code(out_dtype), _stream()), "transpose_cast")
    return out_t, out_c


def attn_spatial_fwd(qkv, H, impl=L.IMPL_AUTO):
    F_, P, C3 = qkv.shape
    C_ = C3 // 3
    qkv = _c(qkv)
    o = torch.empty(F_, P, C_, dtype=qkv.dtype, device=qkv.device)
    lse = torch.empty(F_, H, P, dtype=torch.float32, device=qkv.device)
    check(L.lib().maed_attn_spatial_fwd(_p(qkv), _p(o), _p(lse), F_, P, H, 1.0 / math.sqrt(C_ // H), dt_code(qkv.dtype), impl, _stream()),
          "attn_spatial_fwd")
    return o, lse


def attn_spatial_bwd(qkv, o, d_o, lse, H, dqkv=None, accumulate=False, impl=L.IMPL_AUTO):
    F_, P, C3 = qkv.shape
    dqkv = torch.empty_like(qkv) if dqkv is None else dqkv
    check(L.lib().maed_attn_spatial_bwd(_p(_c(qkv)), _p(_c(o)), _p(_c(d_o)), _p(lse), _p(dqkv), int(accumulate), F_, P, H,
                                        1.0 / math.sqrt(C3 // 3 // H), dt_code(qkv.dtype), impl, _stream()), "attn_spatial_bwd")
    return dqkv


def attn_temporal_fwd(qkv, H, T, prec=None):
    F_, P, C3 = qkv.shape
    C_ = C3 // 3
    qkv = _c(qkv)
    o = torch.empty(F_, P, C_, dtype=qkv.dtype, device=qkv.device)
    lse = torch.empty(F_, H, P, dtype=torch.float32, device=qkv.device)
    check(L.lib().maed_attn_temporal_fwd(_p(qkv), _p(o), _p(lse), F_, P, H, T, 1.0 / math.sqrt(C_ // H), mm_code(qkv.dtype, prec), _stream()),
          "attn_temporal_fwd")
    return o, lse


def attn_temporal_bwd(qkv, o, d_o, lse, H, T, dqkv=None, accumulate=False, prec=None):
    F_, P, C3 = qkv.shape
    dqkv = torch.empty_like(qkv) if dqkv is None else dqkv
    check(L.lib().maed_attn_temporal_bwd(_p(_c(qkv)), _p(_c(o)), _p(_c(d_o)), _p(lse), _p(dqkv), int(accumulate), F_, P, H, T,
                                         1.0 / math.sqrt(C3 // 3 // H), mm_code(qkv.dtype, prec), _stream()), "attn_temporal_bwd")
    return dqkv


def st_colmean(x_s, x_t):
    F_, P, C_ = x_s.shape
    means = torch.empty(F_, 2 * C_, dtype=x_s.dtype, device=x_s.device)
    ws = torch.empty(F_, 2 * C_, dtype=torch.float32, device=x_s.device)
    check(L.lib().maed_st_colmean(_p(_c(x_s)), _p(_c(x_t)), _p(means), _p(ws), F_, P, C_, dt_code(x_s.dtype), _stream()), "st_colmean")
    return means


def st_mix_fwd(x_s, x_t, logits):
    F_, P, C_ = x_s.shape
    mix = torch.empty_like(x_s)
    check(L.lib().maed_st_mix_fwd(_p(_c(x_s)), _p(_c(x_t)), _p(_c(logits)), _p(mix), F_, P, C_, dt_code(x_s.dtype), _stream()), "st_mix_fwd")
    return mix


def st_mix_bwd(dmix, x_s, x_t, logits, dmeans_fn):
    F_, P, C_ = x_s.shape
    dlogits = torch.empty(F_, 2 * C_, dtype=x_s.dtype, device=x_s.device)
    ws = torch.empty(F_, 2 * C_, dtype=torch.float32, device=x_s.device)
    check(L.lib().maed_st_mix_bwd_reduce(_p(_c(dmix)), _p(_c(x_s)), _p(_c(x_t)), _p(logits), _p(dlogits), _p(ws), F_, P, C_,
                                         dt_code(x_s.dtype), _stream()), "st_mix_bwd_reduce")
    dmeans = dmeans_fn(dlogits)
    dx_s, dx_t = torch.empty_like(x_s), torch.empty_like(x_t)
    check(L.lib().maed_st_mix_bwd_apply(_p(_c(dmix)), _p(logits), _p(_c(dmeans)), _p(dx_s), _p(dx_t), F_, P, C_, dt_code(x_s.dtype), _stream()),
          "st_mix_bwd_apply")
    return dx_s, dx_t, dlogits


def adam_step(p, g, m, v, shadow, lr, beta1, beta2, eps, wd, step, gscale=1.0):
    bc1 = 1.0 - beta1 ** step
    bc2 = 1.0 - beta2 ** step
    check(L.lib().maed_adam_step(_p(p), _p(g), _p(m), _p(v), _p(shadow), p.numel(), lr, beta1, beta2, eps, wd, bc1, bc2, gscale, _stream()),
          "adam_step")


def adam_step_dev(p, g, m, v, shadow, state, beta1, beta2, eps, wd, gscale=1.0):
    check(L.lib().maed_adam_step_dev(_p(p), _p(g), _p(m), _p(v), _p(shadow), p.numel(), _p(state), beta1, beta2, eps, wd, gscale, _stream()), "adam_step_dev")


class DeviceTrainState:

    def __init__(self, device):
        self.dev = torch.zeros(32, dtype=torch.uint8, device=device)
        self._host = _np.zeros(32, dtype=_np.uint8)
        self.calls = 0

    def set_hyper(self, lr, bias_corr1, bias_corr2):
        self._host[:12].view(_np.float32)[:] = (lr, bias_corr1, bias_corr2)

    def begin_step(self, seed=None):
        self.calls = 0
        if seed is None:
            seed = int(torch.randint(0, 2 ** 62, (1,), dtype=torch.int64).item())
        self._host[16:24].view(_np.uint64)[0] = seed

    def upload(self):
        src = torch.from_numpy(self._host.copy())
        self.dev.copy_(src.pin_memory() if self.dev.is_cuda else src, non_blocking=True)

    def next_call_id(self):
        self.calls += 1
        return self.calls


DEVICE_STATE = None


_WT_DTYPE = _np.dtype([("src", "u8"), ("dst_c", "u8"), ("dst_t", "u8"), ("rows", "i4"), ("cols", "i4"), ("tile0", "i4"), ("tiles_n", "i4")])


class WeightCache:

    _registry = weakref.WeakSet()

    def __init__(self):
        self._key = None
        self._val = None
        self._images = None
        self._weights = None
        self._dtype = None
        WeightCache._registry.add(self)

    @staticmethod
    def _make_key(weights, dtype):
        return (WEIGHT_EPOCH, dtype, tuple((w.data_ptr(), w._version, tuple(w.shape)) for w in weights))

    def get(self, weights, dtype):
        if self._make_key(weights, dtype) != self._key:
            self._weights, self._dtype = list(weights), dtype
            WeightCache._registry.add(self)
            WeightCache._refresh_group(self)
        return self._val

    @classmethod
    def _refresh_group(cls, me):
        dev, dtype = me._weights[0].device, me._dtype
        group = [c for c in cls._registry if c._weights is not None and c._dtype == dtype and c._weights[0].device == dev]
        rows, keep = [], []
        tile0 = 0
        with torch.no_grad():
            for c in group:
                ok = c._images is not None and len(c._images) == len(c._weights) and all(
                    im[1].shape == (w.shape[1], w.shape[0]) and im[1].dtype == dtype and im[1].device == dev for im, w in zip(c._images, c._weights))
                if not ok:
                    c._images = [(None if dtype == torch.float32 else torch.empty(w.shape, dtype=dtype, device=dev),
                                  torch.empty(w.shape[1], w.shape[0], dtype=dtype, device=dev)) for w in c._weights]
                val = []
                for w, (wc, wt) in zip(c._weights, c._images):
                    src = _c(w.detach())
                    keep.append(src)
                    R, Cn = src.shape
                    tn = (Cn + 63) // 64
                    rows.append((_p(src), 0 if wc is None else _p(wc), _p(wt), R, Cn, tile0, tn))
                    tile0 += ((R + 63) // 64) * tn
                    val.append((src if dtype == torch.float32 else wc, wt))
                c._val = val
        for lo in range(0, len(rows), 256):
            chunk = rows[lo:lo + 256]
            base = chunk[0][5]
            tab = _np.array([r[:5] + (r[5] - base, r[6]) for r in chunk], dtype=_WT_DTYPE)
            ntiles = (chunk[-1][5] - base) + ((chunk[-1][3] + 63) // 64) * chunk[-1][6]
            tab_dev = _upload_table(tab, dev)
            check(L.lib().maed_weight_refresh(_p(tab_dev), len(chunk), ntiles, dt_code(dtype), _stream()), "weight_refresh")
        for c in group:
            c._key = cls._make_key(c._weights, dtype)


_SCRATCH = {}


def _aligned_bytes(nbytes, device, align=256):
    buf = torch.empty(nbytes + align, dtype=torch.uint8, device=device)
    off = (-buf.data_ptr()) % align
    return buf[off:off + nbytes]


def twin_join():
    check(L.lib().maed_ste_block_twin_join(_stream()), "ste_block_twin_join")


def _scratch(nbytes, device, tag=None):
    key = (device.index, _stream(), tag)
    buf = _SCRATCH.get(key)
    if buf is None or buf.numel() < nbytes:
        if buf is not None and isinstance(tag, tuple) and tag and tag[0] == "twin":
            twin_join()
        buf = _aligned_bytes(nbytes, device)
        _SCRATCH[key] = buf
    return buf


class LinearFn(torch.autograd.Function):

    @staticmethod
    def forward(ctx, x, weight, bias, cache, direct_w=None, direct_b=None):
        (wc, wt), = cache.get([weight], x.dtype)
        ctx.save_for_backward(x, weight, bias)
        ctx.wt = wt
        ctx.direct = None
        if direct_w is not None and LinearFn._grad_at_apply and any(ctx.needs_input_grad[1:3]):
            ctx.direct = (direct_w, direct_b)
            direct_grad_begin(direct_w, direct_b)
        x32 = shadow_of(x)
        if x32 is not None:
            return gemm_nt(_c(x32), _c(weight.detach()), L.EPI_STORE, bias=bias)
        return gemm_nt(_c(x), wc, L.EPI_STORE, bias=bias)

    @staticmethod
    def backward(ctx, dy):
        x, weight, bias = ctx.saved_tensors
        dy = _c(dy if dy.dtype == x.dtype else dy.to(x.dtype))
        if lib_matmul_dtype(dy.dtype) and weight.shape[0] % 8 == 0 and weight.shape[1] % 8 == 0:
            if ctx.direct is not None:
                gw, gb = direct_grad_slot(ctx.direct[0]), direct_grad_slot(ctx.direct[1])
                if gw is not None and (bias is None or gb is not None):
                    gemm_tn_wgrad(dy, x, dW=gw.view(weight.shape), dbias=gb)
                    dx = gemm_nt(dy, ctx.wt, L.EPI_STORE) if ctx.needs_input_grad[0] else None
                    direct_grad_done(*ctx.direct)
                    return dx, None, None, None, None, None
                direct_grad_cancel(*ctx.direct)
            db = torch.zeros_like(bias) if bias is not None else None
            dW = gemm_tn_wgrad(dy, x, dbias=db)
            dx = gemm_nt(dy, ctx.wt, L.EPI_STORE) if ctx.needs_input_grad[0] else None
            return dx, dW, db, None, None, None
        if ctx.direct is not None:
            direct_grad_cancel(*ctx.direct)
        db = torch.zeros_like(bias) if bias is not None else None
        dyt, _ = transpose_cast(dy, dy.dtype, colsum=db)
        xt, _ = transpose_cast(x, x.dtype)
        tiles = max(1, (weight.shape[0] // 128) * (weight.shape[1] // 128))
        dW = gemm_nt(dyt, xt, L.EPI_ATOMIC_F32, splitk=max(1, min(dyt.shape[1] // 256, 1024 // tiles)))
        dx = gemm_nt(dy, ctx.wt, L.EPI_STORE) if ctx.needs_input_grad[0] else None
        return dx, dW, db, None, None, None

    _grad_at_apply = True

    @classmethod
    def apply(cls, *args):
        LinearFn._grad_at_apply = torch.is_grad_enabled()
        return super().apply(*args)


class EmbedAddFn(torch.autograd.Function):

    @staticmethod
    def forward(ctx, patch, cls, pos, temp, T):
        F_, Pm1, C_ = patch.shape
        tok = torch.empty(F_, Pm1 + 1, C_, dtype=torch.float32, device=patch.device)
        check(L.lib().maed_embed_add_fwd(_p(_c(patch)), dt_code(patch.dtype), _p(_c(cls)), _p(_c(pos)), _p(_c(temp)), _p(tok),
                                         F_, Pm1 + 1, C_, T, _stream()), "embed_add_fwd")
        ctx.T, ctx.pdtype = T, patch.dtype
        ctx.temp_shape = temp.shape
        return tok

    @staticmethod
    def backward(ctx, dtok):
        dtok = _c(dtok)
        F_, P, C_ = dtok.shape
        dpatch = torch.empty(F_, P - 1, C_, dtype=ctx.pdtype, device=dtok.device)
        dpos = torch.zeros(1, P, C_, dtype=torch.float32, device=dtok.device)
        dtemp = torch.zeros(ctx.temp_shape, dtype=torch.float32, device=dtok.device)
        check(L.lib().maed_embed_add_bwd(_p(dtok), _p(dpatch), dt_code(ctx.pdtype), _p(dpos), _p(dtemp), F_, P, C_, ctx.T, _stream()), "embed_add_bwd")
        dcls = dpos[:, :1].clone()
        return dpatch, dcls, dpos, dtemp, None



_TWIN = [None, None, None]
TWIN_HITS = [0, 0]
_TWIN_WARNED = [False]


DIRECT_GRADS = os.environ.get("MAED_DIRECT_GRADS", "1") == "1"


def direct_grad_slot(p):
    if not DIRECT_GRADS or p is None or not p.is_leaf:
        return None
    g = p.grad
    if g is None or g.dtype != torch.float32 or g.shape != p.shape or g.device != p.device or not g.is_contiguous():
        return None
    return g


def direct_grad_begin(*params):
    for p in params:
        if p is not None:
            p._maed_direct = getattr(p, "_maed_direct", 0) + 1


def direct_grad_cancel(*params):
    for p in params:
        if p is not None:
            p._maed_direct = max(getattr(p, "_maed_direct", 1) - 1, 0)


def direct_grad_done(*params):
    for p in params:
        if p is None:
            continue
        n = getattr(p, "_maed_direct", 1) - 1
        p._maed_direct = max(n, 0)
        hook = getattr(p, "_maed_ready", None)
        if n <= 0 and hook is not None:
            hook(p)


class ReportingFn(torch.autograd.Function):
    _grad_mode_at_apply = True

    @classmethod
    def apply(cls, *args):
        ReportingFn._grad_mode_at_apply = torch.is_grad_enabled()
        return super().apply(*args)

    @staticmethod
    def will_run_backward(ctx):
        return ReportingFn._grad_mode_at_apply and any(ctx.needs_input_grad)


class STEBlockFn(ReportingFn):

    @staticmethod
    def forward(ctx, x, block, dims, H, T, *params):
        lib = L.lib()
        x = _c(x)
        d = L.BlockDims(*dims)
        y = torch.empty_like(x)
        twin = block.compute_dtype == torch.float32 and bwd_twin() and ReportingFn.will_run_backward(ctx) and dims[7] != L.IMPL_VALU and dims[2] % 8 == 0 and dims[5] % 8 == 0
        if twin:
            dims = dims[:6] + (BF16,) + dims[7:]
            d16 = L.BlockDims(*dims)
            pr = block._c_params_masters()
            saved = _aligned_bytes(lib.maed_ste_block_saved_bytes(C.byref(d16)), x.device)
            slot = getattr(block, "_chain_index", 0) & 1
            work = _scratch(lib.maed_ste_block_twin_work_bytes(C.byref(d)), x.device, tag=("twin", slot))
            check(lib.maed_ste_block_fwd_twin(C.byref(d), C.byref(pr), _p(x), _p(y), _p(saved), _p(work), slot, _stream()), "ste_block_fwd_twin")
            TWIN_FORWARDS[0] += 1
        else:
            pr = block._c_params(block.compute_dtype)
            saved = _aligned_bytes(lib.maed_ste_block_saved_bytes(C.byref(d)), x.device)
            entry = lib.maed_ste_block_fwd if ReportingFn.will_run_backward(ctx) else lib.maed_ste_block_infer
            check(entry(C.byref(d), C.byref(pr), _p(x), _p(y), _p(saved), _stream()), "ste_block_fwd")
        ctx.block, ctx.dims, ctx.bdt = block, dims, (torch.bfloat16 if twin else block.compute_dtype)
        ctx.save_for_backward(x, saved)
        _TWIN[0], _TWIN[1], _TWIN[2] = None, None, None
        if ReportingFn.will_run_backward(ctx):
            block._pending_backwards += 1
        return y

    @staticmethod
    def backward(ctx, dy):
        lib = L.lib()
        x, saved = ctx.saved_tensors
        block = ctx.block
        d = L.BlockDims(*ctx.dims)
        cdt = ctx.bdt
        pr = block._c_params(cdt, backward=True)
        gr = block._c_grads()
        dy = _c(dy)
        dx = torch.empty_like(dy)
        scratch = _scratch(lib.maed_ste_block_scratch_bytes(C.byref(d)), dy.device)
        tw_in = None
        if cdt != torch.float32:
            ref, cand, producer = _TWIN
            mine = getattr(block, "_chain_index", None)
            if ref is not None and ref() is dy and cand.shape == dy.shape and cand.dtype == cdt:
                tw_in = cand
            elif ref is not None and producer is not None and mine is not None and producer == mine + 1 and not _TWIN_WARNED[0]:
                _TWIN_WARNED[0] = True
                import warnings
                warnings.warn("maed_amd: the residual-gradient hand-off between consecutive STE blocks was bypassed (the gradient tensor arriving at a block is not "
                              "the one the next block returned); falling back to one extra cast pass per block", RuntimeWarning, stacklevel=2)
            TWIN_HITS[0 if tw_in is not None else 1] += 1
        _TWIN[0], _TWIN[1], _TWIN[2] = None, None, None
        tw_out = torch.empty(dy.shape, dtype=cdt, device=dy.device) if cdt != torch.float32 else None
        check(lib.maed_ste_block_bwd(C.byref(d), C.byref(pr), C.byref(gr), _p(x), _p(dy), _p(dx), _p(saved), _p(scratch),
                                     _p(tw_in), _p(tw_out), _stream()), "ste_block_bwd")
        if tw_out is not None:
            _TWIN[0], _TWIN[1], _TWIN[2] = weakref.ref(dx), tw_out, getattr(block, "_chain_index", None)
        block._pending_backwards -= 1
        if block._pending_backwards == 0 and block.grads_ready is not None:
            block.grads_ready(block)
        return (dx, None, None, None, None) + (None,) * (len(ctx.needs_input_grad) - 5)



_WS_DTYPE = _np.dtype([("w", "u8"), ("gw", "u8"), ("gout", "u8"), ("dst_off", "i8"), ("dst_t_off", "i8"), ("O", "i4"), ("I", "i4"), ("KHW", "i4"),
                       ("fstart", "i4"), ("gout_f32", "i4"), ("pad_", "i4")])


def _ws_table(weights, grads=None, gouts=None, transposed=None, gout_f32=None):
    tab = _np.zeros(len(weights), dtype=_WS_DTYPE)
    off = fstart = 0
    for i, w in enumerate(weights):
        O, I, kh, kw = w.shape
        tab[i] = (w.data_ptr(), 0 if grads is None else grads[i], 0 if gouts is None else gouts[i], off, -1, O, I, kh * kw, fstart,
                  0 if gout_f32 is None else int(gout_f32[i]), 0)
        off += w.numel()
        fstart += O
    total = off
    t_offs = {}
    for i in sorted(transposed or ()):
        tab[i]["dst_t_off"] = total
        t_offs[i] = total
        total += weights[i].numel()
    return tab, off, fstart, total, t_offs


class WeightStdFn(ReportingFn):

    @staticmethod
    def forward(ctx, owner, dtype, eps, *weights):
        weights = [_c(w) for w in weights]
        direct = getattr(owner, "_direct_convs", None)
        gemm = set((direct if direct is not None else getattr(owner, "_gemm_convs", ())) or ()) if lib_matmul_dtype(dtype, getattr(owner, "f32_matmul", None)) else set()
        tab, _, nf, total, t_offs = _ws_table(weights, transposed=gemm)
        dev = weights[0].device
        out = torch.empty(total, dtype=dtype, device=dev)
        stats = torch.empty(nf * 2, dtype=torch.float32, device=dev)
        tab_dev = _upload_table(tab, dev)
        t_tiles = sum(-(-weights[i].shape[0] // 64) * -(-(weights[i].numel() // weights[i].shape[0]) // 64) for i in t_offs) if os.environ.get("MAED_WS_TILED", "1") == "1" else 0
        check(L.lib().maed_weight_std_fwd(_p(tab_dev), len(weights), nf, _p(out), dt_code(dtype), _p(stats), eps, t_tiles, _stream()), "weight_std_fwd")
        ctx.owner, ctx.dtype, ctx.eps, ctx.stats, ctx.nf = owner, dtype, eps, stats, nf
        ctx.weights = weights
        ctx.set_materialize_grads(False)
        if ReportingFn.will_run_backward(ctx):
            owner._pending_backwards += 1
        views, off = [], 0
        for w in weights:
            O, I, kh, kw = w.shape
            views.append(out[off:off + w.numel()].view(O, kh, kw, I).permute(0, 3, 1, 2))
            off += w.numel()
        owner._w_std_t = {i: out[o:o + weights[i].numel()].view(-1, weights[i].shape[0]) for i, o in t_offs.items()}
        owner._dw_arena, owner._dw_slices = None, {}
        if gemm and ReportingFn.will_run_backward(ctx):
            n = sum(weights[i].numel() for i in gemm)
            keep = getattr(owner, "_dw_arena_persist", None)
            if owner._pending_backwards == 1 and keep is not None and keep.numel() == n and keep.device == dev:
                owner._dw_arena = keep.zero_()
            else:
                owner._dw_arena = torch.zeros(n, dtype=torch.float32, device=dev)
                if owner._pending_backwards == 1:
                    owner._dw_arena_persist = owner._dw_arena
            o = 0
            for i in sorted(gemm):
                owner._dw_slices[i] = owner._dw_arena[o:o + weights[i].numel()].view(weights[i].shape[0], -1)
                o += weights[i].numel()
        ctx.dw_slices = owner._dw_slices
        return tuple(views)

    @staticmethod
    def backward(ctx, *gouts):
        dev = ctx.weights[0].device
        gn_affine_flush(dev)
        st = _SIDE.get(dev) if (_side_on() and getattr(ctx.owner, "_ws_on_side", False)) else None
        if st is None or not st[1]:
            side_stream_join(dev)
            return WeightStdFn._backward_body(ctx, gouts)
        side = st[0]
        side.wait_stream(torch.cuda.current_stream(dev))
        _keep_until_join(dev, st, [g for g in gouts if g is not None])
        with torch.cuda.stream(side):
            return WeightStdFn._backward_body(ctx, gouts)

    @staticmethod
    def _backward_body(ctx, gouts):
        weights, owner = ctx.weights, ctx.owner
        params = owner.conv_weights()
        keep, gptr, optr, f32 = [], [], [], []
        for i, (w, p, g) in enumerate(zip(weights, params, gouts)):
            direct = ctx.dw_slices.get(i)
            if g is None and direct is None:
                gptr.append(0); optr.append(0); f32.append(0)
                continue
            if p.grad is None:
                p.grad = torch.zeros_like(p)
            if direct is not None:
                gptr.append(p.grad.data_ptr()); optr.append(direct.data_ptr()); f32.append(1)
                continue
            g = g.to(ctx.dtype)
            g = g.contiguous(memory_format=torch.channels_last) if w.shape[2] * w.shape[3] > 1 else g.contiguous()
            keep.append(g)
            gptr.append(p.grad.data_ptr()); optr.append(g.data_ptr()); f32.append(0)
        tab, _, nf, _, _ = _ws_table(weights, gptr, optr, gout_f32=f32)
        tab_dev = _upload_table(tab, weights[0].device)
        check(L.lib().maed_weight_std_bwd(_p(tab_dev), len(weights), nf, dt_code(ctx.dtype), _p(ctx.stats), ctx.eps, _stream()), "weight_std_bwd")
        owner._pending_backwards -= 1
        if owner._pending_backwards == 0 and owner.grads_ready is not None:
            owner.grads_ready(owner)
        return (None, None, None) + (None,) * len(weights)


LAZY_RES = {}


GN_SYNC_WORDS = 80
GN_DEFER_AFFINE = os.environ.get("MAED_GN_DEFER_AFFINE", "1") == "1"
_GN_DEFERRED = {}


def gn_affine_defer(device, ab, dgamma, dbeta, N, C_):
    pend = _GN_DEFERRED.setdefault(device, [])
    if not pend:
        try:
            torch.autograd.Variable._execution_engine.queue_callback(lambda: gn_affine_flush(device))
        except RuntimeError:
            pass
    pend.append((ab, dgamma, dbeta, N, C_))


def gn_affine_flush(device):
    pend = _GN_DEFERRED.get(device)
    if not pend:
        return
    items = (L.GnAffineItem * len(pend))()
    for i, (ab, dg, db, N, C_) in enumerate(pend):
        items[i].ab, items[i].dgamma, items[i].dbeta, items[i].N, items[i].C = _p(ab), _p(dg), _p(db), N, C_
    check(L.lib().maed_gn_affine_grad_batch(C.cast(items, C.c_void_p), len(pend), _stream()), "gn_affine_grad_batch")
    pend.clear()


class GroupNormFn(torch.autograd.Function):

    @staticmethod
    def forward(ctx, x, residual, gamma, beta, eps, relu, direct, sums=None, ab=None, stats_ready=False, lazy_res=False, sync=None):
        N, C_, H, W = x.shape
        x32 = shadow_of(x)
        r32 = shadow_of(residual) if x32 is not None else None
        if x32 is not None and not x.is_contiguous(memory_format=torch.channels_last):
            twin_fill(x)
        assert x32 is None or residual is None or r32 is not None, "GroupNormFn: the residual of a shadowed input has no shadow"
        x = x.contiguous(memory_format=torch.channels_last)
        if residual is not None:
            residual = residual.contiguous(memory_format=torch.channels_last).to(x.dtype)
        xin, rin = (x, residual) if x32 is None else (x32.contiguous(memory_format=torch.channels_last), r32)
        y = torch.empty_like(xin, memory_format=torch.channels_last)
        zeroed = sums is not None
        if sums is None:
            sums = torch.empty(N, 32, 2, dtype=torch.float64, device=x.device)
        ctx.has_res = residual is not None
        need_mask = relu and ctx.has_res and (x.requires_grad or residual.requires_grad or gamma.requires_grad)
        mask = torch.empty(N * H * W * (C_ // 8), dtype=torch.uint8, device=x.device) if need_mask else None
        if x32 is not None:
            fill_x = x.data_ptr() in _UNFILLED
            y16 = torch.empty_like(y, dtype=torch.bfloat16)
            twin_fill(residual)
            check(L.lib().maed_groupnorm_fwd_twin(_p(xin), _p(rin), _p(gamma), _p(beta), _p(y), _p(sums), _p(mask), N, H * W, C_, eps, int(relu),
                                                  2 if (stats_ready and zeroed) else int(zeroed), _p(x) if fill_x else None, _p(y16), _stream()), "groupnorm_fwd_twin")
            _UNFILLED.discard(x.data_ptr())
            y = shadow_put(y16, y)
        else:
            check(L.lib().maed_groupnorm_fwd(_p(xin), _p(rin), _p(gamma), _p(beta), _p(y), _p(sums), _p(mask), N, H * W, C_, eps, int(relu),
                                             dt_code(xin.dtype), 2 if (stats_ready and zeroed) else int(zeroed), _stream()), "groupnorm_fwd")
        ctx.ab = ab
        ctx.sync = sync if ab is not None else None
        ctx.save_for_backward(x, mask, sums)
        ctx.eps, ctx.relu, ctx.direct = eps, relu, direct
        ctx.lazy_res = bool(lazy_res) and need_mask
        ctx.gamma, ctx.beta = gamma, beta
        return y

    @staticmethod
    def backward(ctx, dy):
        x, mask, sums = ctx.saved_tensors
        gamma, beta = ctx.gamma, ctx.beta
        N, C_, H, W = x.shape
        dy = dy.contiguous(memory_format=torch.channels_last)
        dx = torch.empty_like(x, memory_format=torch.channels_last)
        dres = torch.empty_like(x, memory_format=torch.channels_last) if (ctx.has_res and not ctx.lazy_res) else None
        if ctx.direct:
            if gamma.grad is None:
                gamma.grad = torch.zeros_like(gamma)
            if beta.grad is None:
                beta.grad = torch.zeros_like(beta)
            dgamma, dbeta = gamma.grad, beta.grad
        else:
            dgamma = torch.zeros(C_, dtype=torch.float32, device=x.device)
            dbeta = torch.zeros(C_, dtype=torch.float32, device=x.device)
        ab, ab_zeroed, sync = ctx.ab, ctx.ab is not None, ctx.sync
        ctx.ab = ctx.sync = None
        if ab is None:
            ab = torch.empty(N, C_, 2, dtype=torch.float32, device=x.device)
        if sync is None:
            sync = torch.zeros(N * GN_SYNC_WORDS, dtype=torch.int32, device=x.device)
        defer = ctx.direct and ab_zeroed and GN_DEFER_AFFINE
        aux = side_stream_handle(x.device, ab) if (ctx.direct and not defer) else None
        check(L.lib().maed_groupnorm_bwd(_p(x), _p(mask), _p(dy), _p(sums), _p(gamma), _p(beta), _p(dx), _p(dres), None if defer else _p(dgamma),
                                         None if defer else _p(dbeta), _p(ab), N, H * W, C_, ctx.eps, int(ctx.relu), dt_code(x.dtype), int(ab_zeroed), _p(sync), aux,
                                         _stream()), "groupnorm_bwd")
        if defer:
            gn_affine_defer(x.device, ab, dgamma, dbeta, N, C_)
        if ctx.lazy_res:
            for k in [k for k, (r, _) in LAZY_RES.items() if r() is None]:
                del LAZY_RES[k]
            LAZY_RES[dy.data_ptr()] = (weakref.ref(dy), mask)
            dres = dy
        if ctx.direct:
            return dx, dres, None, None, None, None, None, None, None, None, None, None
        return dx, dres, dgamma, dbeta, None, None, None, None, None, None, None, None


def stem_input(x, dtype, k, s, own=False):
    N, C_, H, W = x.shape
    ph = max((math.ceil(H / s) - 1) * s + k - H, 0)
    pw = max((math.ceil(W / s) - 1) * s + k - W, 0)
    cs, extra = (4, 1) if own else (C_, 0)
    y = torch.empty(N, H + ph, W + pw + extra, cs, dtype=dtype, device=x.device)
    check(L.lib().maed_stem_input(_p(x), _p(y), N, C_, H, W, ph // 2, ph - ph // 2, pw // 2, pw - pw // 2 + extra, cs, dt_code(dtype), _stream()), "stem_input")
    return y.permute(0, 3, 1, 2)


def stem7x7s2_supported(H, W, F_=1):
    H, W, F_ = int(H), int(W), int(F_)
    if F_ < 1 or F_ * (H + 5) * (W + 6) * 8 >= 1 << 31 or F_ * (H // 2) * (W // 2) * 128 >= 1 << 32:
        return False
    return bool(L.lib().maed_stem7x7s2_supported(H, W))


class StemConvFn(torch.autograd.Function):

    @staticmethod
    def forward(ctx, xp, w, dw, sums, hw):
        H, W = hw
        F_ = xp.shape[0]
        assert xp.shape[1] == 4 and xp.shape[2] == H + 5 and xp.shape[3] == W + 6 and xp.dtype == torch.bfloat16 and w.shape[0] == 64 and w.shape[2:] == (7, 7), (xp.shape, w.shape)
        wc = w.permute(0, 2, 3, 1)
        assert wc.is_contiguous() and wc.shape[3] == 3, "stem: the standardised weight must be the channels_last (64, 7, 7, 3) image"
        ctx.save_for_backward(xp)
        ctx.dw, ctx.hw = dw, hw
        x32 = shadow_of(xp)
        if x32 is not None:
            assert sums is None, "stem: the GroupNorm behind a shadowed stem computes its own statistics"
            w32 = shadow_of(w)
            return twin_later(torch.nn.functional.conv2d(x32, w32, None, 2, 0).contiguous(memory_format=torch.channels_last))
        y = torch.empty((F_, 64, H // 2, W // 2), dtype=xp.dtype, device=xp.device, memory_format=torch.channels_last)
        wimg = torch.empty(64 * 224, dtype=xp.dtype, device=xp.device)
        check(L.lib().maed_stem7x7s2_fwd(_p(xp), _p(wc), _p(wimg), _p(y), _p(sums), F_, H, W, dt_code(xp.dtype), _stream()), "stem7x7s2_fwd")
        return y

    @staticmethod
    def backward(ctx, dy):
        (xp,) = ctx.saved_tensors
        H, W = ctx.hw
        dy = dy.contiguous(memory_format=torch.channels_last)
        assert ctx.dw is not None, "stem: no fp32 weight-gradient slice (WeightStdFn hands it out when the backward will run)"
        dw = ctx.dw
        scratch = torch.empty(L.lib().maed_stem7x7s2_wgrad_scratch_floats(xp.shape[0], H, W), dtype=torch.float32, device=dy.device)
        side_stream_run(lambda: check(L.lib().maed_stem7x7s2_wgrad(_p(dy), _p(xp), _p(dw), _p(scratch), xp.shape[0], H, W, dt_code(dy.dtype), _stream()), "stem7x7s2_wgrad"),
                        dy, xp, dw, scratch)
        return None, None, None, None, None


class MaxPool3s2SameFn(torch.autograd.Function):

    @staticmethod
    def forward(ctx, x):
        N, C_, H, W = x.shape
        x32 = shadow_of(x)
        x = (x if x32 is None else x32).contiguous(memory_format=torch.channels_last)
        Ho, Wo = (H + 1) // 2, (W + 1) // 2
        y = torch.empty((N, C_, Ho, Wo), dtype=x.dtype, device=x.device, memory_format=torch.channels_last)
        idx = torch.empty(N * Ho * Wo * C_, dtype=torch.uint8, device=x.device)
        check(L.lib().maed_maxpool3s2_same_fwd(_p(x), _p(y), _p(idx), N, H, W, C_, dt_code(x.dtype), _stream()), "maxpool3s2_same_fwd")
        ctx.save_for_backward(idx)
        ctx.geom = (N, C_, H, W)
        return y if x32 is None else twin_of(y)

    @staticmethod
    def backward(ctx, dy):
        idx, = ctx.saved_tensors
        N, C_, H, W = ctx.geom
        dy = dy.contiguous(memory_format=torch.channels_last)
        dx = torch.empty((N, C_, H, W), dtype=dy.dtype, device=dy.device, memory_format=torch.channels_last)
        check(L.lib().maed_maxpool3s2_same_bwd(_p(dy), _p(idx), _p(dx), N, H, W, C_, dt_code(dy.dtype), _stream()), "maxpool3s2_same_bwd")
        return dx


class Conv1x1Fn(torch.autograd.Function):

    @staticmethod
    def forward(ctx, x, w, wt, dw, fork=False, gn_sums=None, stride=1, lazy_short=False, prec=None):
        N, I, H, W = x.shape
        x32, w32 = shadow_of(x), shadow_of(w)
        assert (x32 is None) == (w32 is None), "Conv1x1Fn: activation and weight must both (or neither) have fp32 shadows"
        x = x.contiguous(memory_format=torch.channels_last)
        O = w.shape[0]
        Ho, Wo = ((H + 1) // 2, (W + 1) // 2) if stride == 2 else (H, W)

        def rows_of(t):
            if stride == 2:
                assert not fork
                A_ = torch.empty(N * Ho * Wo, I, dtype=t.dtype, device=t.device)
                check(L.lib().maed_subsample2_fwd(_p(t), _p(A_), N, H, W, I, dt_code(t.dtype), _stream()), "subsample2_fwd")
                return A_
            assert stride == 1
            return t.permute(0, 2, 3, 1).reshape(N * H * W, I)

        def product(A_, w_):
            w2 = w_.reshape(O, I)
            w2 = w2 if w2.is_contiguous() else w2.contiguous()
            if gn_sums is not None:
                y_ = torch.empty(N * Ho * Wo, O, dtype=A_.dtype, device=A_.device)
                check(L.lib().maed_conv1x1_fwd(_p(A_), A_.stride(0), _p(w2), w2.stride(0), N * Ho * Wo, O, I, _p(y_), O, Ho * Wo, _p(gn_sums), mm_code(A_.dtype, prec),
                                               _stream()), "conv1x1_fwd")
                return y_
            return gemm_nt(A_, w2, L.EPI_STORE, prec=prec)

        A = rows_of(x)
        if x32 is not None:
            y32 = product(rows_of(x32.contiguous(memory_format=torch.channels_last)), w32).view(N, Ho, Wo, O).permute(0, 3, 1, 2)
            y = twin_later(y32)
        else:
            y = product(A, w).view(N, Ho, Wo, O).permute(0, 3, 1, 2)
        ctx.save_for_backward(A, wt)
        ctx.dw, ctx.geom, ctx.stride, ctx.prec = dw, (N, I, H, W, O, Ho, Wo), stride, prec
        ctx.lazy_short = bool(lazy_short) and fork
        ctx.set_materialize_grads(False)
        if not fork:
            return y
        xa = x.view_as(x)
        if x32 is not None:
            shadow_put(xa, x32)
        return y, xa

    @staticmethod
    def backward(ctx, dy, g_short=None):
        A, wt = ctx.saved_tensors
        N, I, H, W, O, Ho, Wo = ctx.geom
        dx = None
        mask = None
        if ctx.lazy_short and g_short is not None:
            ent = LAZY_RES.pop(g_short.data_ptr(), None)
            if ent is None or ent[0]() is not g_short:
                raise RuntimeError("Conv1x1Fn: the shortcut gradient was announced as lazily masked (GroupNormFn lazy_res) but arrived as another tensor -- "
                                   "the residual must feed exactly one GroupNorm")
            mask = ent[1]
        if dy is None:
            if mask is not None:
                raise RuntimeError("Conv1x1Fn: lazily masked shortcut gradient without a gradient for the convolution itself")
            return g_short, None, None, None, None, None, None, None, None
        Y = dy.contiguous(memory_format=torch.channels_last).permute(0, 2, 3, 1).reshape(N * Ho * Wo, O)
        if ctx.needs_input_grad[0]:
            if g_short is not None:
                G = g_short.contiguous(memory_format=torch.channels_last).to(Y.dtype).permute(0, 2, 3, 1).reshape(N * H * W, I)
                dx = gemm_nt(Y, wt, L.EPI_ADD, aux=G, out2=mask, prec=bwd_prec(ctx.prec))
            else:
                dx = gemm_nt(Y, wt, L.EPI_STORE, prec=bwd_prec(ctx.prec))
            if ctx.stride == 2:
                g, dx = dx, torch.empty(N * H * W, I, dtype=dx.dtype, device=dx.device)
                check(L.lib().maed_subsample2_bwd(_p(g), _p(dx), N, H, W, I, dt_code(dx.dtype), _stream()), "subsample2_bwd")
            dx = dx.view(N, H, W, I).permute(0, 3, 1, 2)
        if ctx.dw is not None:
            dw, prec = ctx.dw, ctx.prec
            side_stream_run(lambda: gemm_tn_wgrad(Y, A, dW=dw, prec=bwd_prec(prec)), Y, A, dw)
        if mask is not None and dx is None:
            raise RuntimeError("Conv1x1Fn: lazily masked shortcut gradient but no input gradient requested")
        return dx, None, None, None, None, None, None, None, None




_ZERO_PAGE = {}


def _zero_page(device):
    key = str(device)
    if key not in _ZERO_PAGE:
        _ZERO_PAGE[key] = _aligned_bytes(256, device).zero_()
    return _ZERO_PAGE[key]


def conv3x3(x, w_taps, stride=1, add=None, w_layout=0, gn_sums=None, prec=None):
    N, I, H, W = x.shape
    x = x.contiguous(memory_format=torch.channels_last)
    O = w_taps.numel() // (9 * I)
    Ho, Wo = -(-H // stride), -(-W // stride)
    ph, pw = max((Ho - 1) * stride + 3 - H, 0), max((Wo - 1) * stride + 3 - W, 0)
    y = torch.empty(N, O, Ho, Wo, dtype=x.dtype, device=x.device, memory_format=torch.channels_last)
    if add is not None:
        add = add.contiguous(memory_format=torch.channels_last)
    check(L.lib().maed_conv3x3_fwd(_p(x), _p(w_taps), _p(_zero_page(x.device)), _p(y), N, H, W, I, O, stride, ph // 2, pw // 2, Ho, Wo, _p(add),
                                   w_layout, mm_code(x.dtype, prec), _p(gn_sums), _stream()), "conv3x3_fwd")
    return y


def conv3x3_s2_dgrad(dy, wt, H, W, pad_top, pad_left):
    N, O, Ho, Wo = dy.shape
    I = wt.numel() // (9 * O)
    dy = dy.contiguous(memory_format=torch.channels_last)
    dx = torch.empty(N, I, H, W, dtype=dy.dtype, device=dy.device, memory_format=torch.channels_last)
    check(L.lib().maed_conv3x3_s2_dgrad(_p(dy), _p(wt), _p(_zero_page(dy.device)), _p(dx), N, H, W, I, O, pad_top, pad_left, Ho, Wo, dt_code(dy.dtype), _stream()),
          "conv3x3_s2_dgrad")
    return dx


_TAPMASKS = {}


def _tapmask(N, H, W, device):
    key = (N, H, W, str(device))
    if key not in _TAPMASKS:
        n = (N * H * W + 63) // 64 * 64
        m = _aligned_bytes(2 * n, device)
        check(L.lib().maed_conv3x3_tapmask(_p(m), N, H, W, _stream()), "conv3x3_tapmask")
        _TAPMASKS[key] = m
    return _TAPMASKS[key]


def conv3x3_wgrad(dy, x, out=None, prec=None):
    N, I, H, W = x.shape
    O = dy.shape[1]
    dW = torch.zeros(O, 3, 3, I, dtype=torch.float32, device=x.device) if out is None else out
    if x.dtype == torch.bfloat16:
        nb = L.lib().maed_conv3x3_wgrad_rows64_scratch_floats(N, H, W, I, O)
        if nb > 0:
            scratch = torch.empty(nb, dtype=torch.float32, device=x.device)
            check(L.lib().maed_conv3x3_wgrad_rows64(_p(dy), _p(x), _p(dW), _p(scratch), N, H, W, dt_code(x.dtype), _stream()), "conv3x3_wgrad_rows64")
            _keep_alive_on_stream(scratch)
            return dW
    check(L.lib().maed_conv3x3_wgrad(_p(dy), _p(x), _p(_tapmask(N, H, W, x.device)), _p(_zero_page(x.device)), _p(dW), N, H, W, I, O,
                                     mm_code(x.dtype, prec), _stream()), "conv3x3_wgrad")
    return dW


_S2_TABLES = {}


def conv3x3_s2_wgrad(dy, x, pad_top, pad_left, out=None):
    N, I, H, W = x.shape
    O, Ho, Wo = dy.shape[1:]
    key = (N, H, W, Ho, Wo, pad_top, pad_left, str(x.device))
    if key not in _S2_TABLES:
        n = (N * Ho * Wo + 63) // 64 * 64
        mask, rows = _aligned_bytes(2 * n, x.device), _aligned_bytes(4 * n, x.device)
        check(L.lib().maed_conv3x3_s2_tables(_p(mask), _p(rows), N, H, W, pad_top, pad_left, Ho, Wo, _stream()), "conv3x3_s2_tables")
        _S2_TABLES[key] = (mask, rows)
    mask, rows = _S2_TABLES[key]
    dW = torch.zeros(O, 3, 3, I, dtype=torch.float32, device=x.device) if out is None else out
    check(L.lib().maed_conv3x3_s2_wgrad(_p(dy), _p(x), _p(mask), _p(rows), _p(_zero_page(x.device)), _p(dW), N, H, W, I, O, Ho, Wo, dt_code(x.dtype), _stream()),
          "conv3x3_s2_wgrad")
    return dW


class Conv3x3Fn(torch.autograd.Function):

    @staticmethod
    def forward(ctx, x, w, stride, wt=None, dw=None, gn_sums=None, prec=None):
        x32, w32 = shadow_of(x), shadow_of(w)
        assert (x32 is None) == (w32 is None), "Conv3x3Fn: activation and weight must both (or neither) have fp32 shadows"
        x = x.contiguous(memory_format=torch.channels_last)
        ctx.save_for_backward(x, w)
        ctx.stride, ctx.wt, ctx.dw, ctx.prec = stride, wt, dw, prec
        w_taps = (w if w32 is None else w32).permute(0, 2, 3, 1)
        w_taps = w_taps if w_taps.is_contiguous() else w_taps.contiguous()
        if x32 is not None:
            return twin_later(conv3x3(x32, w_taps, stride, gn_sums=gn_sums, prec=prec))
        return conv3x3(x, w_taps, stride, gn_sums=gn_sums, prec=prec)

    @staticmethod
    def backward(ctx, dy):
        x, w = ctx.saved_tensors
        s, wt, dw_slice, prec = ctx.stride, ctx.wt, ctx.dw, ctx.prec
        dy = dy.contiguous(memory_format=torch.channels_last)
        N, I, H, W = x.shape
        O = w.shape[0]
        Ho, Wo = dy.shape[-2:]
        ph, pw = max((Ho - 1) * s + 3 - H, 0), max((Wo - 1) * s + 3 - W, 0)
        need_x = ctx.needs_input_grad[0]
        need_w = ctx.needs_input_grad[1] or dw_slice is not None
        dx = dw = None
        own_dx = need_x and s == 1 and O % 64 == 0
        own_dx_s2 = need_x and s == 2 and wt is not None and O % 64 == 0 and I % 8 == 0 and dy.dtype == torch.bfloat16 and min(H, W) > 1
        if own_dx_s2:
            dx = conv3x3_s2_dgrad(dy, wt, H, W, ph // 2, pw // 2)
            own_dx = True
        elif own_dx:
            if wt is not None:
                dx = conv3x3(dy, wt, 1, w_layout=1, prec=bwd_prec(prec))
            else:
                dx = conv3x3(dy, w.flip(2, 3).permute(1, 2, 3, 0).contiguous(), 1, prec=bwd_prec(prec))
        own_dw = need_w and s == 1 and ((N * H * W) % 64 == 0 or x.dtype == torch.float32) and I % 8 == 0 and O % 8 == 0
        own_dw_s2 = (need_w and s == 2 and dw_slice is not None and x.dtype == torch.bfloat16 and (N * Ho * Wo) % 64 == 0 and I % 8 == 0 and O % 8 == 0
                     and N * H * W < 1 << 31)
        if own_dw_s2:
            side_stream_run(lambda: conv3x3_s2_wgrad(dy, x, ph // 2, pw // 2, out=dw_slice), dy, x, dw_slice)
            need_w = False
        elif own_dw:
            if dw_slice is not None:
                side_stream_run(lambda: conv3x3_wgrad(dy, x, out=dw_slice, prec=bwd_prec(prec)), dy, x, dw_slice)
            else:
                dw = conv3x3_wgrad(dy, x, prec=bwd_prec(prec)).permute(0, 3, 1, 2)
            need_w = False
        if need_w or (need_x and not own_dx):
            sym = ph % 2 == 0 and pw % 2 == 0
            xin = x if sym else torch.nn.functional.pad(x, [pw // 2, pw - pw // 2, ph // 2, ph - ph // 2])
            pad = (ph // 2, pw // 2) if sym else (0, 0)
            gx, gw, _ = torch.ops.aten.convolution_backward(dy, xin, w, None, (s, s), pad, (1, 1), False, (0, 0), 1,
                                                            (need_x and not own_dx, need_w, False))
            if need_w:
                if dw_slice is not None:
                    dw_slice.view(O, 3, 3, I).add_(gw.permute(0, 2, 3, 1))
                else:
                    dw = gw
            if need_x and not own_dx:
                dx = gx if sym else gx[:, :, ph // 2:ph // 2 + H, pw // 2:pw // 2 + W]
        return dx, dw, None, None, None, None, None


PRE_FORM_AUTO, PRE_FORM_DIRECT, PRE_FORM_LDS, PRE_FORM_TWO = range(4)


def clip_preprocess_workspace(F, H, W):
    return int(L.lib().maed_clip_preprocess_workspace(F, H, W))


def clip_preprocess(blob, offsets, src_bytes, F, N, H, W, mean, std, has_contrast, out, form=PRE_FORM_AUTO):
    base = _p(blob)
    _p(out)
    if out.dtype != torch.float32 or not out.is_contiguous() or out.numel() != F * 3 * H * W:
        raise L.MaedHipError(f"clip_preprocess: out must be contiguous fp32 with {F * 3 * H * W} elements")
    if blob.dtype != torch.uint8 or offsets[4] + src_bytes > blob.numel():
        raise L.MaedHipError("clip_preprocess: the packed buffer is shorter than its tables say")
    need = clip_preprocess_workspace(F, H, W) if (form == PRE_FORM_TWO or (form == PRE_FORM_AUTO and has_contrast)) else 0
    ws = _scratch(need, out.device, tag="clip_preprocess") if need else None
    norm = (C.c_float * 6)(*[float(v) for v in mean], *[float(v) for v in std])
    fi, fm, ci, cf, px = (base + o for o in offsets)
    check(L.lib().maed_clip_preprocess(px, src_bytes, fi, fm, ci, cf, F, N, H, W, norm, int(bool(has_contrast)), form, _p(out), _p(ws), need, _stream()),
          "clip_preprocess")
    return out
```

### maed_amd/resnetv2.py

```python
import math
import os
from collections import OrderedDict

import torch
import torch.nn as nn
import torch.nn.functional as F

from . import ops


_OWN_CONV3X3 = os.environ.get("MAED_CONV3X3", "own") == "own"


_WS_PER_STAGE_ENV = os.environ.get("MAED_WS_PER_STAGE", "auto")

_LAZY_RES_GRAD = os.environ.get("MAED_GN_LAZY_DRES", "1") == "1"

_FUSE_GN_STATS = os.environ.get("MAED_GN_FUSE_STATS", "1") == "1"


def _ws_per_stage():
    if _WS_PER_STAGE is not None:
        return _WS_PER_STAGE
    import torch.distributed as dist
    return dist.is_available() and dist.is_initialized() and dist.get_world_size() > 1


_WS_PER_STAGE = None if _WS_PER_STAGE_ENV == "auto" else _WS_PER_STAGE_ENV == "1"


class _WsGroup:

    def __init__(self, parent, conv_idx, norms):
        self.parent, self.conv_idx, self.norms = parent, list(conv_idx), list(norms)
        self._pending_backwards = 0
        self._ws_on_side = False
        self._w_std_t, self._dw_slices, self._dw_arena = {}, {}, None

    @property
    def f32_matmul(self):
        return self.parent.f32_matmul

    def conv_weights(self):
        return [self.parent._convs[i].weight for i in self.conv_idx]

    def fused_parameters(self):
        return self.conv_weights() + [t for m in self.norms for t in (m.weight, m.bias)]

    @property
    def _direct_convs(self):
        pos = {ci: k for k, ci in enumerate(self.conv_idx)}
        return [pos[i] for i in self.parent._direct_convs if i in pos]

    @property
    def grads_ready(self):
        cb = self.parent.grads_ready
        return None if cb is None else (lambda _owner: cb(self))


def _same_pad(x, k, s, value=0.0):
    ih, iw = x.shape[-2:]
    ph = max((math.ceil(ih / s) - 1) * s + k - ih, 0)
    pw = max((math.ceil(iw / s) - 1) * s + k - iw, 0)
    if ph > 0 or pw > 0:
        x = F.pad(x, [pw // 2, pw - pw // 2, ph // 2, ph - ph // 2], value=value)
    return x


class StdConv2dSame(nn.Conv2d):

    def __init__(self, in_channel, out_channels, kernel_size, stride=1, dilation=1, groups=1, bias=False, eps=1e-5):
        super().__init__(in_channel, out_channels, kernel_size, stride=stride, padding=0, dilation=dilation, groups=groups, bias=bias)
        self.eps = eps

    def get_weight(self):
        std, mean = torch.std_mean(self.weight, dim=[1, 2, 3], keepdim=True, unbiased=False)
        return (self.weight - mean) / (std + self.eps)

    _w_std = None
    _w_t = None
    _dw = None
    _prec = None
    _prepadded = False
    _gn_behind = None
    _stem_hw = None

    @staticmethod
    def _gn_sums_for(gn, x_shape, out_channels, stride):
        if gn is None or not _FUSE_GN_STATS or gn._sums_buf is None or gn.num_groups != 32:
            return None
        cpg = out_channels // 32
        hw = (-(-x_shape[-2] // stride)) * (-(-x_shape[-1] // stride))
        if out_channels % 32 or cpg < 2 or cpg & (cpg - 1) or hw < 128 or x_shape[0] * x_shape[1] * x_shape[2] * x_shape[3] * 2 >= 1 << 32:
            return None
        gn._stats_ready = True
        return gn._sums_buf

    def forward(self, x, fork=False, gn=None, lazy_short=False):
        w = self._w_std
        if w is not None and self._w_t is not None and self.kernel_size == (1, 1):
            return ops.Conv1x1Fn.apply(x, w, self._w_t, self._dw, fork, self._gn_sums_for(gn, x.shape, self.out_channels, self.stride[0]), self.stride[0], lazy_short,
                                       self._prec)
        assert not fork
        if (w is not None and _OWN_CONV3X3 and self.kernel_size == (3, 3) and ops.on_library_device(x) and ops.lib_matmul_dtype(x.dtype, self._prec)
                and self.in_channels % 64 == 0 and self.out_channels % 8 == 0 and self.dilation == (1, 1) and self.groups == 1):
            return ops.Conv3x3Fn.apply(x, w, self.stride[0], self._w_t, self._dw, self._gn_sums_for(gn, x.shape, self.out_channels, self.stride[0]), self._prec)
        if w is None:
            w = self.get_weight().to(x.dtype)
            if ops.on_library_device(x):
                w = w.contiguous(memory_format=torch.channels_last)
        if self._prepadded == "own":
            gn = self._gn_behind[0] if self._gn_behind else None
            sums = None
            if ops.shadow_of(x) is None and gn is not None and _FUSE_GN_STATS and gn._sums_buf is not None and gn.num_groups == 32 and self.out_channels == 64:
                gn._stats_ready, sums = True, gn._sums_buf
            return ops.StemConvFn.apply(x, w, self._dw, sums, self._stem_hw)
        if self._prepadded:
            return F.conv2d(x, w, None, self.stride, 0, self.dilation, self.groups)
        k, s = self.kernel_size[0], self.stride[0]
        ih, iw = x.shape[-2:]
        ph = max((math.ceil(ih / s) - 1) * s + k - ih, 0)
        pw = max((math.ceil(iw / s) - 1) * s + k - iw, 0)
        if ph % 2 == 0 and pw % 2 == 0:
            return F.conv2d(x, w, None, self.stride, (ph // 2, pw // 2), self.dilation, self.groups)
        x = F.pad(x, [pw // 2, pw - pw // 2, ph // 2, ph - ph // 2])
        return F.conv2d(x, w, None, self.stride, 0, self.dilation, self.groups)


class GroupNormAct(nn.GroupNorm):

    _direct_grad = False
    _sums_buf = None
    _ab_buf = None
    _sync_buf = None
    _stats_ready = False

    def __init__(self, num_channels, num_groups=32, eps=1e-5, affine=True, apply_act=True):
        super().__init__(num_groups, num_channels, eps=eps, affine=affine)
        self.apply_act = apply_act

    def forward(self, x, residual=None, relu=None, lazy_res=False):
        relu = self.apply_act if relu is None else relu
        if ops.on_library_device(x) and self.num_groups == 32:
            ready, self._stats_ready = self._stats_ready and self._sums_buf is not None, False
            return ops.GroupNormFn.apply(x, residual, self.weight, self.bias, self.eps, relu, self._direct_grad, self._sums_buf, self._ab_buf, ready, lazy_res,
                                         self._sync_buf)
        x = F.group_norm(x, self.num_groups, self.weight.to(x.dtype), self.bias.to(x.dtype), self.eps)
        if residual is not None:
            x = x + residual
        return F.relu(x) if relu else x


class MaxPool2dSame(nn.Module):

    def __init__(self, kernel_size=3, stride=2):
        super().__init__()
        self.kernel_size, self.stride = kernel_size, stride

    def forward(self, x):
        if ops.on_library_device(x) and self.kernel_size == 3 and self.stride == 2 and x.shape[1] % 8 == 0 and x.dtype in (torch.float32, torch.bfloat16):
            return ops.MaxPool3s2SameFn.apply(x)
        return F.max_pool2d(_same_pad(x, self.kernel_size, self.stride, value=-float("inf")), self.kernel_size, self.stride, 0)


class DownsampleConv(nn.Module):

    def __init__(self, in_chs, out_chs, stride=1):
        super().__init__()
        self.conv = StdConv2dSame(in_chs, out_chs, 1, stride=stride)
        self.norm = GroupNormAct(out_chs, apply_act=False)

    def forward(self, x):
        return self.norm(self.conv(x, gn=self.norm))


class Bottleneck(nn.Module):

    def __init__(self, in_chs, out_chs, stride=1, downsample=False):
        super().__init__()
        mid = out_chs // 4
        self.downsample = DownsampleConv(in_chs, out_chs, stride) if downsample else None
        self.conv1 = StdConv2dSame(in_chs, mid, 1)
        self.norm1 = GroupNormAct(mid)
        self.conv2 = StdConv2dSame(mid, mid, 3, stride=stride)
        self.norm2 = GroupNormAct(mid)
        self.conv3 = StdConv2dSame(mid, out_chs, 1)
        self.norm3 = GroupNormAct(out_chs, apply_act=False)
        self.drop_path = nn.Identity()

    def forward(self, x):
        if self.conv1._w_t is not None and torch.is_grad_enabled() and x.requires_grad:
            lazy = self.downsample is None and _LAZY_RES_GRAD
            y, xa = self.conv1(x, fork=True, gn=self.norm1, lazy_short=lazy)
            shortcut = xa if self.downsample is None else self.downsample(xa)
            x = self.norm1(y)
            x = self.norm2(self.conv2(x, gn=self.norm2))
            return self.norm3(self.conv3(x, gn=self.norm3), residual=shortcut, relu=True, lazy_res=lazy)
        else:
            shortcut = x if self.downsample is None else self.downsample(x)
            x = self.norm1(self.conv1(x, gn=self.norm1))
        x = self.norm2(self.conv2(x, gn=self.norm2))
        return self.norm3(self.conv3(x, gn=self.norm3), residual=shortcut, relu=True)


class ResNetStage(nn.Module):

    def __init__(self, in_chs, out_chs, stride, depth):
        super().__init__()
        blocks = OrderedDict()
        for b in range(depth):
            blocks[str(b)] = Bottleneck(in_chs if b == 0 else out_chs, out_chs, stride=stride if b == 0 else 1, downsample=(b == 0))
        self.blocks = nn.Sequential(blocks)

    def forward(self, x):
        return self.blocks(x)


def _slots(module, **values):
    module.__dict__.update(values)


class ResNetV2(nn.Module):

    def __init__(self, layers=(3, 4, 9), channels=(256, 512, 1024), in_chans=3, stem_chs=64, compute_dtype=torch.float32, f32_matmul=None, **_):
        super().__init__()
        self.compute_dtype = compute_dtype
        assert f32_matmul in (None, "bf16x3", "bf16x6"), f32_matmul
        self.f32_matmul = f32_matmul
        self.stem = nn.Sequential(OrderedDict([
            ("conv", StdConv2dSame(in_chans, stem_chs, 7, stride=2)),
            ("norm", GroupNormAct(stem_chs)),
            ("pool", MaxPool2dSame(3, 2)),
        ]))
        stages = OrderedDict()
        prev = stem_chs
        for i, (d, c) in enumerate(zip(layers, channels)):
            stages[str(i)] = ResNetStage(prev, c, stride=1 if i == 0 else 2, depth=d)
            prev = c
        self.stages = nn.Sequential(stages)
        self.num_features = prev
        self.norm = nn.Identity()
        self.head = nn.Identity()
        for m in self.modules():
            if isinstance(m, nn.Conv2d):
                nn.init.kaiming_normal_(m.weight, mode="fan_out", nonlinearity="relu")
        self._convs = [m for m in self.modules() if isinstance(m, StdConv2dSame)]
        self._norms = [m for m in self.modules() if isinstance(m, GroupNormAct)]
        for m in self._norms:
            m._direct_grad = True
        strides = ((1, 1), (2, 2)) if os.environ.get("MAED_CONV1X1_S2", "1") == "1" else ((1, 1),)
        self._gemm_convs = [i for i, c in enumerate(self._convs) if c.kernel_size == (1, 1) and c.stride in strides
                            and c.in_channels % 64 == 0 and c.out_channels % 64 == 0]
        if os.environ.get("MAED_GEMM_CONVS", "1") == "0":
            self._gemm_convs = []
        s3 = ((1, 1), (2, 2)) if os.environ.get("MAED_CONV3X3_S2", "1") == "1" else ((1, 1),)
        self._own3x3 = [i for i, c in enumerate(self._convs) if _OWN_CONV3X3 and c.kernel_size == (3, 3) and c.stride in s3
                        and c.in_channels % 64 == 0 and c.out_channels % 64 == 0]
        self.stem.conv._gn_behind = (self.stem.norm,)
        self._own_stem_now = []
        self._w_std_t, self._dw_slices, self._dw_arena = {}, {}, None
        self._pending_backwards = 0
        self._grad_forward_seen = False
        self.grads_ready = None
        conv_pos = {id(c): i for i, c in enumerate(self._convs)}
        parts = [[self.stem, self.stages[0]]] + [[st] for st in list(self.stages)[1:]]
        self._ws_groups = [_WsGroup(self, [conv_pos[id(m)] for part in ps for m in part.modules() if isinstance(m, StdConv2dSame)],
                                    [m for part in ps for m in part.modules() if isinstance(m, GroupNormAct)]) for ps in parts]

    def conv_weights(self):
        return [c.weight for c in self._convs]

    @property
    def _direct_convs(self):
        return list(self._gemm_convs) + list(self._own3x3) + list(self._own_stem_now)

    def fused_parameters(self):
        return self.conv_weights() + [t for m in self._norms for t in (m.weight, m.bias)]

    def forward_features(self, x):
        if not ops.on_library_device(x):
            return self.stages(self.stem(x))
        try:
            y = self._forward_features_library(x)
            ops.shadow_keep_only(y)
            return y
        except BaseException:
            ops.shadow_clear()
            raise
        finally:
            _slots(self.stem.conv, _prepadded=False, _stem_hw=None)
            self._own_stem_now = []
            for c in self._convs:
                _slots(c, _w_std=None, _w_t=None, _dw=None, _prec=None)
            for m in self._norms:
                _slots(m, _sums_buf=None, _ab_buf=None, _sync_buf=None)

    def _forward_features_library(self, x):
        stem = self.stem.conv
        cdt = self.compute_dtype
        stem_fused = (x.dtype == torch.float32 and x.is_contiguous() and x.shape[1] <= 4 and not x.requires_grad and os.environ.get("MAED_STEM_INPUT", "1") == "1"
                      and stem.dilation == (1, 1) and stem.kernel_size[0] == stem.kernel_size[1])
        own_ok = (os.environ.get("MAED_STEM_OWN", "1") == "1" and stem.kernel_size == (7, 7) and stem.stride == (2, 2)
                  and stem.in_channels <= 3 and stem.out_channels == 64 and stem.groups == 1 and ops.stem7x7s2_supported(x.shape[2], x.shape[3], x.shape[0]))
        twin = (cdt == torch.float32 and ops.bwd_twin() and torch.is_grad_enabled() and stem_fused and own_ok
                and len(set(self._gemm_convs) | set(self._own3x3) | {0}) == len(self._convs) and any(p.requires_grad for p in self.fused_parameters()))
        ops.shadow_clear()
        if twin:
            cdt = torch.bfloat16
            ops.TWIN_FORWARDS[0] += 1
        if stem_fused:
            own = cdt == torch.bfloat16 and own_ok
            self._own_stem_now = [0] if own else []
            _slots(stem, _prepadded="own" if own else True, _stem_hw=(x.shape[2], x.shape[3]))
            x32p = ops.stem_input(x, torch.float32, stem.kernel_size[0], stem.stride[0], own=False) if twin else None
            x = ops.stem_input(x, cdt, stem.kernel_size[0], stem.stride[0], own=own)
            if twin:
                ops.shadow_put(x, x32p)
        else:
            x = x.to(dtype=cdt, memory_format=torch.channels_last)
        ws = None if _ws_per_stage() else self._standardise(self, cdt, twin)
        N = x.shape[0]
        sums = torch.zeros(len(self._norms), N, 32, 2, dtype=torch.float64, device=x.device)
        ab = None
        if torch.is_grad_enabled() and any(p.requires_grad for p in self.fused_parameters()):
            self._grad_forward_seen = True
        if torch.is_grad_enabled() and any(p.requires_grad for p in (self._norms[0].weight, self._convs[0].weight)):
            ab = torch.zeros(N * 2 * sum(m.num_channels for m in self._norms) + N * ops.GN_SYNC_WORDS * len(self._norms), dtype=torch.float32, device=x.device)
        if ws is not None:
            for i, (c, w) in enumerate(zip(self._convs, ws)):
                _slots(c, _w_std=w, _w_t=self._w_std_t.get(i), _dw=self._dw_slices.get(i), _prec=self.f32_matmul)
        off = 0
        for i, m in enumerate(self._norms):
            _slots(m, _sums_buf=sums[i])
            if ab is not None:
                n = N * 2 * m.num_channels
                _slots(m, _ab_buf=ab[off:off + n].view(N, m.num_channels, 2), _sync_buf=ab[off + n:off + n + N * ops.GN_SYNC_WORDS])
                off += n + N * ops.GN_SYNC_WORDS
        if ws is not None:
            return self.stages(self.stem(x))
        for gi, g in enumerate(self._ws_groups):
            wg = self._standardise(g, cdt, twin)
            for k, (ci, w) in enumerate(zip(g.conv_idx, wg)):
                c = self._convs[ci]
                _slots(c, _w_std=w, _w_t=g._w_std_t.get(k), _dw=g._dw_slices.get(k), _prec=self.f32_matmul)
            x = self.stages[0](self.stem(x)) if gi == 0 else self.stages[gi](x)
        runs = [g for g in self._ws_groups if g._pending_backwards > 0]
        for k, g in enumerate(self._ws_groups):
            g._ws_on_side = bool(runs) and g is not runs[0] and g in runs
        return x

    def _standardise(self, owner, cdt, twin):
        eps = self._convs[0].eps
        ws = ops.WeightStdFn.apply(owner, cdt, eps, *owner.conv_weights())
        if twin:
            import types
            with torch.no_grad():
                ws32 = ops.WeightStdFn.apply(types.SimpleNamespace(_direct_convs=[], f32_matmul=self.f32_matmul, _pending_backwards=0), torch.float32, eps,
                                             *[w.detach() for w in owner.conv_weights()])
            for w16, w32 in zip(ws, ws32):
                ops.shadow_put(w16, w32)
        return ws

    def forward(self, x, seqlen=8):
        return self.forward_features(x)
```

Before: 418.4.

## Fuse stem GroupNorm+ReLU apply into maxpool forward and pooled backward gather

Adds a fused kernel that applies the stem GroupNorm affine and ReLU while computing the 3x3 stride-2 max pool, so the full-resolution normalized activation is never written to memory. The backward GroupNorm kernels gain a POOL mode that gathers the pooled gradient through the argmax indices on the fly, which removes the separate maxpool backward pass and its full-size dx buffer. This costs recomputing the normalization per pooling window and scattered index-based gathers inside the GN reduce and apply kernels. It is enabled by default through a new option.

```diff
diff --git a/include/maed_hip.h b/include/maed_hip.h
--- a/include/maed_hip.h
+++ b/include/maed_hip.h
@@ -63,6 +63,7 @@
     MAED_OPT_TN_SK = 15,
     MAED_OPT_CONV3X3_NARROW_WGS = 16,
     MAED_OPT_CONV3X3_FRAME = 17,
+    MAED_OPT_GN_FUSE_APPLY = 18,
     MAED_OPT_COUNT
 } maed_option;
 int maed_init(int device);
@@ -249,6 +250,11 @@
 
 int maed_maxpool3s2_same_fwd(const void* x, void* y, uint8_t* idx, int N, int H, int W, int C, int dtype, void* stream);
 int maed_maxpool3s2_same_bwd(const void* dy, const uint8_t* idx, void* dx, int N, int H, int W, int C, int dtype, void* stream);
+int maed_maxpool3s2_same_gn_fwd(const void* x, const double* sums, const float* gamma, const float* beta, void* y, uint8_t* idx, int N, int H, int W, int C,
+                                float eps, int dtype, void* stream);
+int maed_groupnorm_bwd_pooled(const void* x, const void* pooled_dy, const uint8_t* pool_idx, const double* sums, const float* gamma, const float* beta,
+                              void* dx, float* dgamma, float* dbeta, float* ab_scratch, int N, int H, int W, int C, float eps, int dtype, int ab_zeroed,
+                              uint32_t* frame_sync, void* aux_stream, void* stream);
 
 int maed_stem_input(const float* x, void* y, int N, int C, int H, int W, int pad_top, int pad_bottom, int pad_left, int pad_right, int c_stride, int dtype,
                     void* stream);
diff --git a/maed_amd/_lib.py b/maed_amd/_lib.py
--- a/maed_amd/_lib.py
+++ b/maed_amd/_lib.py
@@ -13,7 +13,7 @@
 IMPL_MFMA_SK = 10
 IMPL_X3, IMPL_X6, IMPL_X1 = 7, 8, 9
 (OPT_F32_MATMUL, OPT_SIDE_STREAM, OPT_TN_TARGET_WGS, OPT_ABLATE, OPT_GN_BWD_ONEPASS, OPT_F32_BWD_X1, OPT_ST_FUSED, OPT_CONV3X3_ROWS_WGS, OPT_STEM_WGRAD_WGS,
- OPT_LBS_FRAMES, OPT_TN_DMA, OPT_X3_PLANES, OPT_X3_PLANES_LN, OPT_SK, OPT_SK_GRID, OPT_TN_SK, OPT_CONV3X3_NARROW_WGS, OPT_CONV3X3_FRAME) = range(18)
+ OPT_LBS_FRAMES, OPT_TN_DMA, OPT_X3_PLANES, OPT_X3_PLANES_LN, OPT_SK, OPT_SK_GRID, OPT_TN_SK, OPT_CONV3X3_NARROW_WGS, OPT_CONV3X3_FRAME, OPT_GN_FUSE_APPLY) = range(19)
 
 vp, i64, i32, f32 = C.c_void_p, C.c_int64, C.c_int, C.c_float
 
@@ -141,6 +141,8 @@
     "maed_eval_vertex_error": (i32, [vp, vp, i32, i32, vp, vp]),
     "maed_maxpool3s2_same_fwd": (i32, [vp, vp, vp, i32, i32, i32, i32, i32, vp]),
     "maed_maxpool3s2_same_bwd": (i32, [vp, vp, vp, i32, i32, i32, i32, i32, vp]),
+    "maed_maxpool3s2_same_gn_fwd": (i32, [vp, vp, vp, vp, vp, vp, i32, i32, i32, i32, f32, i32, vp]),
+    "maed_groupnorm_bwd_pooled": (i32, [vp, vp, vp, vp, vp, vp, vp, vp, vp, vp, i32, i32, i32, i32, f32, i32, i32, vp, vp, vp]),
     "maed_stem_input": (i32, [vp, vp, i32, i32, i32, i32, i32, i32, i32, i32, i32, i32, vp]),
     "maed_conv3x3_wgrad_rows64_scratch_floats": (i32, [i32, i32, i32, i32, i32]),
     "maed_conv3x3_wgrad_rows64": (i32, [vp, vp, vp, vp, i32, i32, i32, i32, vp]),
@@ -204,6 +206,7 @@
     OPT_CONV3X3_FRAME: int(os.environ.get("MAED_CONV3X3_FRAME", "1")),
     OPT_CONV3X3_NARROW_WGS: int(os.environ.get("MAED_CONV3X3_NARROW_WGS", "0")),
     OPT_TN_SK: int(os.environ.get("MAED_TN_SK", "1")),
+    OPT_GN_FUSE_APPLY: int(os.environ.get("MAED_GN_FUSE_APPLY", "1")),
     OPT_X3_PLANES_LN: int(os.environ.get("MAED_X3_PLANES_LN", "0")),
 }
 
diff --git a/maed_amd/csrc/backbone.hip b/maed_amd/csrc/backbone.hip
--- a/maed_amd/csrc/backbone.hip
+++ b/maed_amd/csrc/backbone.hip
@@ -244,12 +244,48 @@
     }
 }
 
-template <typename T, bool RELU, bool YMASK>
+struct GnPool { const void* dy; const uint8_t* idx; int W, Ho, Wo, top, left; };
+template <typename T>
+__device__ __forceinline__ void gn_pool_gather8(const GnPool& p, int n, int r, int C, int c8, float (&g)[8]) {
+    const int h = r / p.W, w = r - h * p.W;
+    const int hp = h + p.top, wp = w + p.left, k = hp >> 1, dh = hp & 1, l = wp >> 1, dw = wp & 1;
+#pragma unroll
+    for (int j = 0; j < 8; ++j) g[j] = 0.f;
+#pragma unroll
+    for (int wh = 0; wh < 2; ++wh) {
+        const int ho = k - 1 + wh, kh = 2 * (1 - wh) + dh;
+        if (kh > 2 || ho < 0 || ho >= p.Ho) continue;
+#pragma unroll
+        for (int ww = 0; ww < 2; ++ww) {
+            const int wo = l - 1 + ww, kw = 2 * (1 - ww) + dw;
+            if (kw > 2 || wo < 0 || wo >= p.Wo) continue;
+            const int64_t o = ((((int64_t)n * p.Ho + ho) * p.Wo + wo) * C + c8);
+            const uint2 a = *reinterpret_cast<const uint2*>(p.idx + o);
+            float d[8];
+            ld8((const T*)p.dy + o, d);
+            const uint32_t tap = (uint32_t)(kh * 3 + kw);
+#pragma unroll
+            for (int j = 0; j < 4; ++j) {
+                if (((a.x >> (8 * j)) & 0xffu) == tap) g[j] += d[j];
+                if (((a.y >> (8 * j)) & 0xffu) == tap) g[4 + j] += d[4 + j];
+            }
+        }
+    }
+#pragma unroll
+    for (int j = 0; j < 8; ++j) g[j] = round_to<T>(g[j]);
+}
+template <typename T, bool POOL>
+__device__ __forceinline__ void gn_dy_load8(const T* dy, const GnPool& pool, int n, int r, int HW, int C, int c8, float (&d)[8]) {
+    if (POOL) gn_pool_gather8<T>(pool, n, r, C, c8, d);
+    else gn_load8(dy + ((int64_t)n * HW + r) * C + c8, d);
+}
+
+template <typename T, bool RELU, bool YMASK, bool POOL = false>
 __global__ __launch_bounds__(256) void gn_bwd_reduce_kernel(const T* __restrict__ x, const uint8_t* __restrict__ mask, const T* __restrict__ dy,
                                                             const double* __restrict__ sums, const float* __restrict__ gamma,
                                                             const float* __restrict__ beta, float* __restrict__ ab ,
                                                             float* __restrict__ dgamma, float* __restrict__ dbeta,
-                                                            int HW, int C, float eps, int rows_per_wg, int defer_affine) {
+                                                            int HW, int C, float eps, int rows_per_wg, int defer_affine, GnPool pool) {
     MAED_DYN_SHARED(float, lpart);
     __shared__ float lmu[GN_G], lrs[GN_G];
     const int n = blockIdx.y;
@@ -283,7 +319,8 @@
         uint32_t o0 = 0, o1 = 0, o2 = 0, o3 = 0;
         const int64_t a0 = base + (int64_t)r * C, a1 = a0 + (int64_t)rstep * C, a2 = a1 + (int64_t)rstep * C, a3 = a2 + (int64_t)rstep * C;
         gn_load8(x + a0, v0); gn_load8(x + a1, v1); gn_load8(x + a2, v2); gn_load8(x + a3, v3);
-        gn_load8(dy + a0, d0); gn_load8(dy + a1, d1); gn_load8(dy + a2, d2); gn_load8(dy + a3, d3);
+        gn_dy_load8<T, POOL>(dy, pool, n, r, HW, C, cb * 8, d0); gn_dy_load8<T, POOL>(dy, pool, n, r + rstep, HW, C, cb * 8, d1);
+        gn_dy_load8<T, POOL>(dy, pool, n, r + 2 * rstep, HW, C, cb * 8, d2); gn_dy_load8<T, POOL>(dy, pool, n, r + 3 * rstep, HW, C, cb * 8, d3);
         if (RELU && YMASK) {
             const int64_t m0 = ((int64_t)n * HW + r) * cbn + cb;
             o0 = mask[m0]; o1 = mask[m0 + (int64_t)rstep * cbn]; o2 = mask[m0 + 2 * (int64_t)rstep * cbn]; o3 = mask[m0 + 3 * (int64_t)rstep * cbn];
@@ -293,7 +330,7 @@
     for (; r < r1; r += rstep) {
         float v[8], d[8];
         uint32_t o = 0;
-        gn_load8(x + base + (int64_t)r * C, v); gn_load8(dy + base + (int64_t)r * C, d);
+        gn_load8(x + base + (int64_t)r * C, v); gn_dy_load8<T, POOL>(dy, pool, n, r, HW, C, cb * 8, d);
         if (RELU && YMASK) o = mask[((int64_t)n * HW + r) * cbn + cb];
         GN_RED_ROW(v, d, o)
     }
@@ -354,12 +391,12 @@
     return MAED_OK;
 }
 
-template <typename T, bool RES, bool RELU>
+template <typename T, bool RES, bool RELU, bool POOL = false>
 __global__ __launch_bounds__(256) void gn_bwd_apply_kernel(const T* __restrict__ x, const uint8_t* __restrict__ mask, const T* __restrict__ dy,
                                                            const double* __restrict__ sums, const float* __restrict__ ab,
                                                            const float* __restrict__ gamma, const float* __restrict__ beta,
                                                            T* __restrict__ dx, T* __restrict__ dres,
-                                                           int HW, int C, float eps, int rows_per_wg) {
+                                                           int HW, int C, float eps, int rows_per_wg, GnPool pool) {
     __shared__ float lmu[GN_G], lrs[GN_G], lm1[GN_G], lm2[GN_G];
     const int n = blockIdx.y, cpg = C / GN_G;
     if (threadIdx.x < GN_G) {
@@ -385,7 +422,7 @@
     const int64_t base = ((int64_t)n * HW) * C + cb * 8;
     for (int r = r0 + rsub; r < r1; r += rstep) {
         float v[8], d[8], o[8];
-        gn_load8(x + base + (int64_t)r * C, v); gn_load8(dy + base + (int64_t)r * C, d);
+        gn_load8(x + base + (int64_t)r * C, v); gn_dy_load8<T, POOL>(dy, pool, n, r, HW, C, cb * 8, d);
         if (RELU) {
             if (RES) { const uint32_t bits = mask[((int64_t)n * HW + r) * cbn + cb];
 #pragma unroll
@@ -426,12 +463,12 @@
     c.a = make_float4(o[0], o[1], o[2], o[3]); c.b = make_float4(o[4], o[5], o[6], o[7]);
 }
 #define GN1_SYNC_WORDS 80
-template <typename T, bool RELU, bool YMASK, int GPC, int CH, int NT>
+template <typename T, bool RELU, bool YMASK, int GPC, int CH, int NT, bool POOL = false>
 __global__ __launch_bounds__(NT, 4) void gn_bwd_onepass_kernel(const T* __restrict__ x, const uint8_t* __restrict__ mask, const T* __restrict__ dy,
                                                                    const double* __restrict__ sums, const float* __restrict__ gamma, const float* __restrict__ beta,
                                                                    float* ab , T* __restrict__ dx, T* __restrict__ dres,
                                                                    uint32_t* sync , int HW, int C, float eps, int S,
-                                                                   int rows_per_wg, int phase, int skew, uint32_t* fault ) {
+                                                                   int rows_per_wg, int phase, int skew, uint32_t* fault , GnPool pool) {
     MAED_DYN_SHARED(float, lpart);
     __shared__ float lmu[GN_G], lrs[GN_G], lgrp[GN_G * 2], lb[GN_G], lk[GN_G];
     __shared__ int lfail;
@@ -469,7 +506,8 @@
         const int r = r0 + rsub + k * rstep;
         if (r < r1) {
             gn_chunk_ld(x + base + (int64_t)r * C, xr[k]);
-            gn_chunk_ld(dy + base + (int64_t)r * C, dr[k]);
+            if (POOL) { float g8[8]; gn_pool_gather8<T>(pool, n, r, C, cb * 8, g8); gn_chunk_put(dr[k], g8); }
+            else gn_chunk_ld(dy + base + (int64_t)r * C, dr[k]);
             if (RELU && YMASK) mb[k >> 2] |= (uint32_t)mask[((int64_t)n * HW + r) * cbn + cb] << (8 * (k & 3));
         } else { gn_chunk_zero(xr[k]); gn_chunk_zero(dr[k]); }
     }
@@ -599,10 +637,11 @@
     return groupnorm_fwd(x, residual, gamma, beta, y, sums, relu_mask, N, HW, C, eps, relu, MAED_F32, sums_zeroed, twin_x, twin_y, stream);
 }
 
-extern "C" int maed_groupnorm_bwd(const void* x, const uint8_t* relu_mask, const void* dy, const double* sums, const float* gamma, const float* beta,
-                                  void* dx, void* dres, float* dgamma, float* dbeta, float* ab_scratch, int N, int HW, int C, float eps,
-                                  int relu, int dtype, int ab_zeroed, uint32_t* frame_sync, void* aux_stream, void* stream) {
-    MAED_CHECK_ARG(x && dy && sums && gamma && beta && dx && ab_scratch, MAED_ERR_ARG, "groupnorm_bwd: null pointer");
+static int groupnorm_bwd(const void* x, const uint8_t* relu_mask, const void* dy, const double* sums, const float* gamma, const float* beta,
+                         void* dx, void* dres, float* dgamma, float* dbeta, float* ab_scratch, int N, int HW, int C, float eps,
+                         int relu, int dtype, int ab_zeroed, uint32_t* frame_sync, void* aux_stream, void* stream, const GnPool* pool) {
+    MAED_CHECK_ARG(x && (dy || pool) && sums && gamma && beta && dx && ab_scratch, MAED_ERR_ARG, "groupnorm_bwd: null pointer");
+    const GnPool pl = pool ? *pool : GnPool{nullptr, nullptr, 0, 0, 0, 0, 0};
     MAED_CHECK_ARG((dgamma != nullptr) == (dbeta != nullptr), MAED_ERR_ARG, "groupnorm_bwd: dgamma and dbeta go together (both NULL: the caller folds ab_scratch with maed_gn_affine_grad_batch)");
     MAED_CHECK_ARG(!(relu && dres) || relu_mask, MAED_ERR_ARG, "groupnorm_bwd: the forward's relu_mask is needed when a residual was added before the ReLU");
     MAED_PROPAGATE(gn_check(C, HW, "groupnorm_bwd"));
@@ -627,16 +666,17 @@
         rows1 = (((HW + S1 - 1) / S1) + rstep - 1) / rstep * rstep;
         onepass = S1 <= 64;
     }
-#define GN_RED(RELU_, YM_) hipLaunchKernelGGL((gn_bwd_reduce_kernel<T, RELU_, YM_>), rgrid, dim3(256), lds, s, (const T*)x, relu_mask, (const T*)dy, \
-        sums, gamma, beta, ab_scratch, dgamma, dbeta, HW, C, eps, rrows, defer)
-#define GN_APP(RES_, RELU_) hipLaunchKernelGGL((gn_bwd_apply_kernel<T, RES_, RELU_>), grid, dim3(256), 0, s, (const T*)x, relu_mask, (const T*)dy, \
-        sums, ab_scratch, gamma, beta, (T*)dx, (T*)dres, HW, C, eps, rows)
-#define GN_ONE4(RELU_, YM_, GPC_, CH_, PH_, NT_) hipLaunchKernelGGL((gn_bwd_onepass_kernel<T, RELU_, YM_, GPC_, CH_, NT_>), dim3(S1, N), dim3(NT_), lds1, s, (const T*)x, relu_mask, \
-        (const T*)dy, sums, gamma, beta, ab_scratch, (T*)dx, (T*)dres, frame_sync, HW, C, eps, (maed_opt(MAED_OPT_GN_BWD_ONEPASS) == 3 ? 1 : S1), rows1, PH_, skew1, fault1)
-#define GN_ONE3(RELU_, YM_, GPC_, CH_, PH_) do { if (nt1 == 256) GN_ONE4(RELU_, YM_, GPC_, CH_, PH_, 256); else GN_ONE4(RELU_, YM_, GPC_, CH_, PH_, GN1_NT); } while (0)
-#define GN_ONE2(RELU_, YM_, CH_, PH_) do { if (cpg >= 8) GN_ONE3(RELU_, YM_, 1, CH_, PH_); else if (cpg == 4) GN_ONE3(RELU_, YM_, 2, CH_, PH_); else GN_ONE3(RELU_, YM_, 4, CH_, PH_); } while (0)
+#define GN_RED(RELU_, YM_, POOL_) hipLaunchKernelGGL((gn_bwd_reduce_kernel<T, RELU_, YM_, POOL_>), rgrid, dim3(256), lds, s, (const T*)x, relu_mask, (const T*)dy, \
+        sums, gamma, beta, ab_scratch, dgamma, dbeta, HW, C, eps, rrows, defer, pl)
+#define GN_APP(RES_, RELU_, POOL_) hipLaunchKernelGGL((gn_bwd_apply_kernel<T, RES_, RELU_, POOL_>), grid, dim3(256), 0, s, (const T*)x, relu_mask, (const T*)dy, \
+        sums, ab_scratch, gamma, beta, (T*)dx, (T*)dres, HW, C, eps, rows, pl)
+#define GN_ONE4(RELU_, YM_, GPC_, CH_, PH_, NT_, POOL_) hipLaunchKernelGGL((gn_bwd_onepass_kernel<T, RELU_, YM_, GPC_, CH_, NT_, POOL_>), dim3(S1, N), dim3(NT_), lds1, s, (const T*)x, relu_mask, \
+        (const T*)dy, sums, gamma, beta, ab_scratch, (T*)dx, (T*)dres, frame_sync, HW, C, eps, (maed_opt(MAED_OPT_GN_BWD_ONEPASS) == 3 ? 1 : S1), rows1, PH_, skew1, fault1, pl)
+#define GN_ONE3(RELU_, YM_, GPC_, CH_, PH_, POOL_) do { if (nt1 == 256) GN_ONE4(RELU_, YM_, GPC_, CH_, PH_, 256, POOL_); else GN_ONE4(RELU_, YM_, GPC_, CH_, PH_, GN1_NT, POOL_); } while (0)
+#define GN_ONE2(RELU_, YM_, CH_, PH_, POOL_) do { if (cpg >= 8) GN_ONE3(RELU_, YM_, 1, CH_, PH_, POOL_); else if (cpg == 4) GN_ONE3(RELU_, YM_, 2, CH_, PH_, POOL_); else GN_ONE3(RELU_, YM_, 4, CH_, PH_, POOL_); } while (0)
 #define GN_ONE(PH_) do { constexpr int CH_ = sizeof(T) == 2 ? 8 : 4, CHM_ = sizeof(T) == 2 ? 7 : 4; \
-        if (!relu) GN_ONE2(false, false, CH_, PH_); else if (ymask) GN_ONE2(true, true, CH_, PH_); else GN_ONE2(true, false, CHM_, PH_); } while (0)
+        if (!relu) GN_ONE2(false, false, CH_, PH_, false); else if (ymask) GN_ONE2(true, true, CH_, PH_, false); else if (pool) GN_ONE2(true, false, CHM_, PH_, true); \
+        else GN_ONE2(true, false, CHM_, PH_, false); } while (0)
     const size_t lds1 = (size_t)(nt1 / cbn1) * 2 * C * sizeof(float);
     const int opt1 = maed_opt(MAED_OPT_GN_BWD_ONEPASS);
     const int skew1 = (int64_t)S1 * N >= 1536 ? (opt1 >= 10 ? opt1 - 10 : 2) : 0;
@@ -647,7 +687,7 @@
 #else
             GN_ONE(0);
 #endif
-        } else if (!relu) GN_RED(false, false); else if (ymask) GN_RED(true, true); else GN_RED(true, false);
+        } else if (!relu) GN_RED(false, false, false); else if (ymask) GN_RED(true, true, false); else if (pool) GN_RED(true, false, true); else GN_RED(true, false, false);
         if (defer && dgamma) {
             hipStream_t sa = s;
             if (aux_stream) {
@@ -657,7 +697,8 @@
             hipLaunchKernelGGL(gn_affine_grad_kernel, dim3((2 * C + 63) / 64, (N + 63) / 64), dim3(256), 0, sa, ab_scratch, dgamma, dbeta, N, C);
         }
         if (onepass) { }
-        else if (ymask) GN_APP(true, true); else if (dres) GN_APP(true, false); else if (relu) GN_APP(false, true); else GN_APP(false, false);
+        else if (ymask) GN_APP(true, true, false); else if (dres) GN_APP(true, false, false); else if (pool) GN_APP(false, true, true); else if (relu) GN_APP(false, true, false);
+        else GN_APP(false, false, false);
     });
 #undef GN_RED
 #undef GN_APP
@@ -667,6 +708,27 @@
 #undef GN_ONE4
     MAED_CHECK_LAUNCH("groupnorm_bwd");
     return MAED_OK;
+}
+
+extern "C" int maed_groupnorm_bwd(const void* x, const uint8_t* relu_mask, const void* dy, const double* sums, const float* gamma, const float* beta,
+                                  void* dx, void* dres, float* dgamma, float* dbeta, float* ab_scratch, int N, int HW, int C, float eps,
+                                  int relu, int dtype, int ab_zeroed, uint32_t* frame_sync, void* aux_stream, void* stream) {
+    MAED_CHECK_ARG(dy, MAED_ERR_ARG, "groupnorm_bwd: null pointer");
+    return groupnorm_bwd(x, relu_mask, dy, sums, gamma, beta, dx, dres, dgamma, dbeta, ab_scratch, N, HW, C, eps, relu, dtype, ab_zeroed, frame_sync, aux_stream, stream, nullptr);
+}
+
+static void maxpool_geom(int H, int W, int& Ho, int& Wo, int& top, int& left);
+extern "C" int maed_groupnorm_bwd_pooled(const void* x, const void* pooled_dy, const uint8_t* pool_idx, const double* sums, const float* gamma, const float* beta,
+                                         void* dx, float* dgamma, float* dbeta, float* ab_scratch, int N, int H, int W, int C, float eps, int dtype, int ab_zeroed,
+                                         uint32_t* frame_sync, void* aux_stream, void* stream) {
+    MAED_CHECK_ARG(pooled_dy && pool_idx, MAED_ERR_ARG, "groupnorm_bwd_pooled: null pointer");
+    MAED_CHECK_ARG(H > 0 && W > 0 && (int64_t)H * W < (1ll << 31), MAED_ERR_SHAPE, "groupnorm_bwd_pooled: H=%d W=%d", H, W);
+    MAED_CHECK_ARG(is_aligned(pooled_dy, 16) && is_aligned(pool_idx, 8), MAED_ERR_ALIGN, "groupnorm_bwd_pooled: 16-B alignment");
+    GnPool pool{pooled_dy, pool_idx, W, 0, 0, 0, 0};
+    int Ho;
+    maxpool_geom(H, W, Ho, pool.Wo, pool.top, pool.left);
+    pool.Ho = Ho;
+    return groupnorm_bwd(x, nullptr, nullptr, sums, gamma, beta, dx, nullptr, dgamma, dbeta, ab_scratch, N, H * W, C, eps, 1, dtype, ab_zeroed, frame_sync, aux_stream, stream, &pool);
 }
 
 template <typename T>
@@ -704,6 +766,63 @@
 }
 
 template <typename T>
+__global__ __launch_bounds__(256) void maxpool3s2_gn_fwd_kernel(const T* __restrict__ x, const double* __restrict__ sums, const float* __restrict__ gamma,
+                                                                const float* __restrict__ beta, T* __restrict__ y, uint8_t* __restrict__ idx, int H, int W,
+                                                                int C, int Ho, int Wo, int top, int left, float eps) {
+    __shared__ float lmu[GN_G], lrs[GN_G];
+    const int n = blockIdx.y;
+    if (threadIdx.x < GN_G) {
+        const double cnt = (double)H * W * (C / GN_G);
+        const double m = sums[((int64_t)n * GN_G + threadIdx.x) * 2] / cnt;
+        double var = sums[((int64_t)n * GN_G + threadIdx.x) * 2 + 1] / cnt - m * m;
+        if (var < 0.0) var = 0.0;
+        lmu[threadIdx.x] = (float)m; lrs[threadIdx.x] = (float)(1.0 / sqrt(var + (double)eps));
+    }
+    __syncthreads();
+    const int i = blockIdx.x * 256 + threadIdx.x;
+    const int cb = C / 8, cpg = C / GN_G;
+    if (i >= Ho * Wo * cb) return;
+    const int c8 = (i % cb) * 8, pix = i / cb;
+    const int wo = pix % Wo, ho = pix / Wo;
+    float a[8], b[8];
+    {
+        float gg[8], bb[8];
+        ld8(gamma + c8, gg); ld8(beta + c8, bb);
+#pragma unroll
+        for (int j = 0; j < 8; ++j) {
+            const int g = (c8 + j) / cpg;
+            a[j] = lrs[g] * gg[j]; b[j] = bb[j] - lmu[g] * a[j];
+        }
+    }
+    float m[8]; int am[8];
+#pragma unroll
+    for (int j = 0; j < 8; ++j) { m[j] = -INFINITY; am[j] = 0; }
+    bool first = true;
+    for (int kh = 0; kh < 3; ++kh) {
+        const int h = 2 * ho - top + kh;
+        if (h < 0 || h >= H) continue;
+        for (int kw = 0; kw < 3; ++kw) {
+            const int w = 2 * wo - left + kw;
+            if (w < 0 || w >= W) continue;
+            float v[8];
+            ld8(x + (((int64_t)n * H + h) * W + w) * C + c8, v);
+#pragma unroll
+            for (int j = 0; j < 8; ++j) {
+                const float t = round_to<T>(fmaxf(fmaf(v[j], a[j], b[j]), 0.f));
+                if (first || t > m[j] || t != t) { m[j] = t; am[j] = kh * 3 + kw; }
+            }
+            first = false;
+        }
+    }
+    const int64_t o = ((int64_t)n * Ho * Wo * cb + i) * 8;
+    st8(y + o, m);
+    uint32_t lo = 0, hi = 0;
+#pragma unroll
+    for (int j = 0; j < 4; ++j) { lo |= (uint32_t)am[j] << (8 * j); hi |= (uint32_t)am[4 + j] << (8 * j); }
+    *reinterpret_cast<uint2*>(idx + o) = make_uint2(lo, hi);
+}
+
+template <typename T>
 __global__ __launch_bounds__(256) void maxpool3s2_bwd_kernel(const T* __restrict__ dy, const uint8_t* __restrict__ idx, T* __restrict__ dx, int N, int H,
                                                              int W, int C, int Ho, int Wo, int top, int left) {
     const int64_t i = (int64_t)blockIdx.x * 256 + threadIdx.x;
@@ -778,6 +897,21 @@
     MAED_DISPATCH_DTYPE(dtype, T, hipLaunchKernelGGL((maxpool3s2_fwd_kernel<T>), dim3((unsigned)((n + 255) / 256)), dim3(256), 0, (hipStream_t)stream,
                                                       (const T*)x, (T*)y, idx, N, H, W, C, Ho, Wo, top, left));
     MAED_CHECK_LAUNCH("maxpool3s2_same_fwd");
+    return MAED_OK;
+}
+
+extern "C" int maed_maxpool3s2_same_gn_fwd(const void* x, const double* sums, const float* gamma, const float* beta, void* y, uint8_t* idx, int N, int H, int W,
+                                           int C, float eps, int dtype, void* stream) {
+    MAED_CHECK_ARG(x && sums && gamma && beta && y && idx, MAED_ERR_ARG, "maxpool3s2_same_gn_fwd: null pointer");
+    MAED_CHECK_ARG(N >= 0 && H > 0 && W > 0 && C > 0 && C % GN_G == 0 && C % 8 == 0, MAED_ERR_SHAPE, "maxpool3s2_same_gn_fwd: C=%d must be a multiple of 32", C);
+    int Ho, Wo, top, left;
+    maxpool_geom(H, W, Ho, Wo, top, left);
+    const int64_t per_frame = (int64_t)Ho * Wo * (C / 8);
+    MAED_CHECK_ARG(per_frame < (1ll << 31) - 256 && N <= 65535, MAED_ERR_SHAPE, "maxpool3s2_same_gn_fwd: frame or batch too large (N=%d)", N);
+    if (N == 0) return MAED_OK;
+    MAED_DISPATCH_DTYPE(dtype, T, hipLaunchKernelGGL((maxpool3s2_gn_fwd_kernel<T>), dim3((unsigned)((per_frame + 255) / 256), N), dim3(256), 0, (hipStream_t)stream,
+                                                      (const T*)x, sums, gamma, beta, (T*)y, idx, H, W, C, Ho, Wo, top, left, eps));
+    MAED_CHECK_LAUNCH("maxpool3s2_same_gn_fwd");
     return MAED_OK;
 }
 
diff --git a/maed_amd/csrc/options.hip b/maed_amd/csrc/options.hip
--- a/maed_amd/csrc/options.hip
+++ b/maed_amd/csrc/options.hip
@@ -21,6 +21,7 @@
     {0},
     {1},
     {0},
+    {1},
     {1},
 };
 
diff --git a/maed_amd/ops.py b/maed_amd/ops.py
--- a/maed_amd/ops.py
+++ b/maed_amd/ops.py
@@ -1023,6 +1023,62 @@
         dx = torch.empty((N, C_, H, W), dtype=dy.dtype, device=dy.device, memory_format=torch.channels_last)
         check(L.lib().maed_maxpool3s2_same_bwd(_p(dy), _p(idx), _p(dx), N, H, W, C_, dt_code(dy.dtype), _stream()), "maxpool3s2_same_bwd")
         return dx
+
+
+def gn_fuse_apply():
+    return L.get_option(L.OPT_GN_FUSE_APPLY) != 0
+
+
+class StemNormPoolFn(torch.autograd.Function):
+
+    @staticmethod
+    def forward(ctx, x, gamma, beta, eps, direct, sums, ab=None, sync=None):
+        N, C_, H, W = x.shape
+        assert shadow_of(x) is None and x.is_contiguous(memory_format=torch.channels_last) and C_ % 32 == 0, "StemNormPoolFn: channels_last, 32 groups, no shadow"
+        Ho, Wo = (H + 1) // 2, (W + 1) // 2
+        y = torch.empty((N, C_, Ho, Wo), dtype=x.dtype, device=x.device, memory_format=torch.channels_last)
+        idx = torch.empty(N * Ho * Wo * C_, dtype=torch.uint8, device=x.device)
+        check(L.lib().maed_maxpool3s2_same_gn_fwd(_p(x), _p(sums), _p(gamma), _p(beta), _p(y), _p(idx), N, H, W, C_, eps, dt_code(x.dtype), _stream()),
+              "maxpool3s2_same_gn_fwd")
+        ctx.ab = ab
+        ctx.sync = sync if ab is not None else None
+        ctx.save_for_backward(x, idx, sums)
+        ctx.eps, ctx.direct = eps, direct
+        ctx.gamma, ctx.beta = gamma, beta
+        return y
+
+    @staticmethod
+    def backward(ctx, dy):
+        x, idx, sums = ctx.saved_tensors
+        gamma, beta = ctx.gamma, ctx.beta
+        N, C_, H, W = x.shape
+        dy = dy.contiguous(memory_format=torch.channels_last)
+        dx = torch.empty_like(x, memory_format=torch.channels_last)
+        if ctx.direct:
+            if gamma.grad is None:
+                gamma.grad = torch.zeros_like(gamma)
+            if beta.grad is None:
+                beta.grad = torch.zeros_like(beta)
+            dgamma, dbeta = gamma.grad, beta.grad
+        else:
+            dgamma = torch.zeros(C_, dtype=torch.float32, device=x.device)
+            dbeta = torch.zeros(C_, dtype=torch.float32, device=x.device)
+        ab, ab_zeroed, sync = ctx.ab, ctx.ab is not None, ctx.sync
+        ctx.ab = ctx.sync = None
+        if ab is None:
+            ab = torch.empty(N, C_, 2, dtype=torch.float32, device=x.device)
+        if sync is None:
+            sync = torch.zeros(N * GN_SYNC_WORDS, dtype=torch.int32, device=x.device)
+        defer = ctx.direct and ab_zeroed and GN_DEFER_AFFINE
+        aux = side_stream_handle(x.device, ab) if (ctx.direct and not defer) else None
+        check(L.lib().maed_groupnorm_bwd_pooled(_p(x), _p(dy), _p(idx), _p(sums), _p(gamma), _p(beta), _p(dx), None if defer else _p(dgamma),
+                                                None if defer else _p(dbeta), _p(ab), N, H, W, C_, ctx.eps, dt_code(x.dtype), int(ab_zeroed), _p(sync), aux,
+                                                _stream()), "groupnorm_bwd_pooled")
+        if defer:
+            gn_affine_defer(x.device, ab, dgamma, dbeta, N, C_)
+        if ctx.direct:
+            return dx, None, None, None, None, None, None, None
+        return dx, dgamma, dbeta, None, None, None, None, None
 
 
 class Conv1x1Fn(torch.autograd.Function):
diff --git a/maed_amd/resnetv2.py b/maed_amd/resnetv2.py
--- a/maed_amd/resnetv2.py
+++ b/maed_amd/resnetv2.py
@@ -337,17 +337,27 @@
                 _slots(m, _ab_buf=ab[off:off + n].view(N, m.num_channels, 2), _sync_buf=ab[off + n:off + n + N * ops.GN_SYNC_WORDS])
                 off += n + N * ops.GN_SYNC_WORDS
         if ws is not None:
-            return self.stages(self.stem(x))
+            return self.stages(self._stem_library(x))
         for gi, g in enumerate(self._ws_groups):
             wg = self._standardise(g, cdt, twin)
             for k, (ci, w) in enumerate(zip(g.conv_idx, wg)):
                 c = self._convs[ci]
                 _slots(c, _w_std=w, _w_t=g._w_std_t.get(k), _dw=g._dw_slices.get(k), _prec=self.f32_matmul)
-            x = self.stages[0](self.stem(x)) if gi == 0 else self.stages[gi](x)
+            x = self.stages[0](self._stem_library(x)) if gi == 0 else self.stages[gi](x)
         runs = [g for g in self._ws_groups if g._pending_backwards > 0]
         for k, g in enumerate(self._ws_groups):
             g._ws_on_side = bool(runs) and g is not runs[0] and g in runs
         return x
+
+    def _stem_library(self, x):
+        conv, norm, pool = self.stem.conv, self.stem.norm, self.stem.pool
+        y = conv(x)
+        if (ops.gn_fuse_apply() and norm._stats_ready and norm._sums_buf is not None and norm.num_groups == 32 and norm.apply_act and y.dtype == torch.bfloat16
+                and ops.shadow_of(y) is None and pool.kernel_size == 3 and pool.stride == 2 and y.shape[0] <= 65535
+                and y.is_contiguous(memory_format=torch.channels_last)):
+            norm._stats_ready = False
+            return ops.StemNormPoolFn.apply(y, norm.weight, norm.bias, norm.eps, norm._direct_grad, norm._sums_buf, norm._ab_buf, norm._sync_buf)
+        return pool(norm(y))
 
     def _standardise(self, owner, cdt, twin):
         eps = self._convs[0].eps
```

Measured after the change: 418.9, median of 4. About the same (+0.1%).
